# drscotthawley/signaltrain

Measured on AMD Instinct MI355X. Metric: audio-frames/sec (train step) comp_4c 8192-sample windows @ 1/2/4/8 GPUs, higher is better.
Workload: dtype f32; 1 GPU; comp_4c synthetic, 8192-sample windows, batch 256/GPU, fp32 (BASELINE configs[1]); window=8192, frames_per_window=25, global_batch=256, parallelism=dp1

## Files before the change

### include/signaltrain_hip.h

```cpp
#ifndef SIGNALTRAIN_HIP_H
#define SIGNALTRAIN_HIP_H
#include <stddef.h>
#include <stdint.h>
#ifdef __cplusplus
extern "C" {
#endif

#define ST_OK 0
#define ST_ERR_ARG (-1)
#define ST_ERR_LAUNCH (-2)
#define ST_ERR_UNSUPPORTED (-3)

#define ST_PREC_F32 0
#define ST_PREC_BF16 1
#define ST_PREC_BF16_ALL 2
#define ST_PREC_F16 3
#define ST_PREC_F16_ALL 4
#define ST_PREC_F32X3 5

typedef struct st_dims {
    int B;
    int L;
    int N;
    int H;
    int T;
    int OT;
    int F;
    int K;
    int y;
    int prec;
    float loss_scale;
    int clip_all;
} st_dims;

int st_kp(int F);

const char* st_last_error(void);
int st_version(void);

int st_set_tuning(int code);
int st_get_tuning(int* out, int n);
int st_tuning_defaults(int* out, int n);
int st_reset_tuning(void);
int st_effective_prec(const st_dims* d);
int st_set_debug(int v);

int st_profile_enable(int on);
int st_profile_report(char* buf, int buflen);

int st_geometry(double scale_factor, double shrink_factor, int legacy, int K, int B, st_dims* out);

int64_t st_param_offsets(const st_dims* d, int64_t* offs );

size_t st_workspace_bytes(const st_dims* d);
size_t st_workspace_bytes_max(const st_dims* d);

int st_analysis_fwd(const st_dims* d, const float* x, const float* Wr, const float* Wi, float in_scale,
                    float* re, float* im, float* mag, float* phs, void* stream);

int st_ae_fwd(const st_dims* d, const float* mag, const float* phs, const float* knobs,
              const float* ae_m, const float* ae_p, float* mag_hat, float* phs_hat, float* AA,
              float* reg_partial, float* ws, void* stream);
int st_ae_fwd_partials(const st_dims* d);
size_t st_ae_fwd_ws_floats(const st_dims* d);

int st_synth_fold(const st_dims* d, const float* Sr, const float* Si, float* Sfold, void* stream);

int st_synth_slabs(const st_dims* d);
int st_synth_frame_slabs(const st_dims* d);

int st_synthesis_frames(const st_dims* d, const float* AA, const float* Sfold, float* frs, void* stream);

int st_nt128_worklist(const st_dims* d, int which, int ncus, unsigned* out, int cap, int* head6);

int st_fm_div_exact(int R, int B);

int st_ola_loss(const st_dims* d, const float* frs, const float* x, const float* y_true,
                float* y_hat, float* dsyn, float* loss_partial, void* stream);
int st_ola_loss_partials(const st_dims* d);

int st_synthesis_dgrad(const st_dims* d, const float* dsyn, const float* Sfold, float* dAA, void* stream);

int st_synthesis_wgrad(const st_dims* d, const float* AA, const float* dsyn, float* ws,
                       float* gSr, float* gSi, float* norm_partial, void* stream);

int st_ae_bwd(const st_dims* d, const float* mag, const float* phs, const float* knobs,
              const float* ae_m, const float* ae_p, const float* mag_hat, const float* phs_hat,
              const float* dAA, const float* g_mag_hat , float reg_coef,
              float* dmag, float* dphs, float* ws, float* g_m, float* g_p, void* stream);
size_t st_ae_bwd_ws_floats(const st_dims* d);
size_t st_ae_kept_activation_bytes(const st_dims* d);

int st_polar_bwd(const st_dims* d, const float* re, const float* im, const float* dmag, const float* dphs,
                 const float* g_mag , float* dG, void* stream);

int st_analysis_wgrad(const st_dims* d, const float* dG, const float* x, float in_scale, float* ws,
                      float* gWr, float* gWi, float* norm_partial, void* stream);
size_t st_wgrad_ws_floats(const st_dims* d);
int st_norm_partials(const st_dims* d);

int st_finalize_scalars(const st_dims* d, const float* loss_partial, const float* reg_partial,
                        const float* norm_partial_a, const float* norm_partial_s, float inv_world,
                        float* scalars , void* stream);
int st_clip_adam(float* params, float* grads, float* m, float* v, int64_t n_total, int64_t n_stft,
                 const float* scalars, float grad_scale, float lr, float beta1, float beta2, float eps, int step,
                 void* stream);

int st_model_fwd(const st_dims* d, const float* params, const float* x, const float* knobs,
                 float* y_hat, float* mag, float* mag_hat, void* ws, int save_for_backward, void* stream);

int st_model_bwd(const st_dims* d, const float* params, float* grads, const float* x, const float* knobs,
                 const float* g_y_hat, const float* g_mag_hat, const float* g_mag, void* ws, void* stream);

int st_loss_backward(const st_dims* d, const float* params, float* grads, const float* x, const float* knobs,
                     const float* y_true, float* y_hat, float* mag, float* mag_hat, void* ws,
                     float* scalars, void* stream);

int st_eval_step(const st_dims* d, const float* params, const float* x, const float* knobs, const float* y_true,
                 float* y_hat , void* ws, double* acc , double beta, void* stream);

int st_loss_backward_p1(const st_dims* d, const float* params, float* grads, const float* x, const float* knobs,
                        const float* y_true, void* ws, void* stream);
int st_loss_backward_p2(const st_dims* d, float* grads, const float* x, void* ws, float* scalars, void* stream);
int st_loss_backward_p2_staged(const st_dims* d, float* grads, float* stage, const float* x, void* ws, float* scalars, void* stream);
int st_unstage_analysis(const st_dims* d, float* grads, const float* stage, void* stream);

int st_loss_backward_stage(const st_dims* d, const float* params, float* grads, const float* x, const float* knobs,
                           const float* y_true, void* ws, float* scalars, int stage, void* stream);

int st_train_step(const st_dims* d, float* params, float* grads, float* m, float* v, const float* x,
                  const float* knobs, const float* y_true, void* ws, float* scalars,
                  float lr, float beta1, float beta2, float eps, int step, void* stream);

#define ST_GROUP_ANALYSIS  1
#define ST_GROUP_SYNTHESIS 2
#define ST_GROUP_AE_MAG    4
#define ST_GROUP_AE_PHS    8
#define ST_GROUP_ALL      15

#define ST_STAGE_SYN_DGRAD  1
#define ST_STAGE_SYN_WGRAD  2
#define ST_STAGE_AE_BWD     4
#define ST_STAGE_AE_DINPUT  8
#define ST_STAGE_ANA_WGRAD 16

int st_step_groups_stages(int trainable);

int st_train_step_groups(const st_dims* d, float* params, float* grads, float* m, float* v,
                         const float* x, const float* knobs, const float* y_true, void* ws, float* scalars,
                         float lr, float beta1, float beta2, float eps,
                         const int step[4],
                         int trainable, void* stream);

int st_dp_clip_adam(const st_dims* d, float* params, float* grads, float* m, float* v, void* ws,
                    float* scalars, float grad_scale, float lr, float beta1, float beta2, float eps,
                    int step, void* stream);

typedef struct st_dp st_dp;
int st_dp_unique_id(void* id128);
int st_dp_init(const void* id128, int rank, int world, st_dp** out);
int st_dp_destroy(st_dp* p);
int st_dp_rank(const st_dp* p);
int st_dp_world(const st_dp* p);
int st_dp_rccl_version(const st_dp* p);
int st_dp_allreduce(st_dp* p, float* buf, int64_t n, void* stream);
int st_dp_broadcast(st_dp* p, float* buf, int64_t n, int root, void* stream);
int st_dp_sync(st_dp* p, void* stream);
int st_dp_train_step(st_dp* p, const st_dims* d, float* params, float* grads, float* m, float* v, float* stage,
                     const float* x, const float* knobs, const float* y_true, void* ws, float* scalars,
                     float lr, float beta1, float beta2, float eps, int step, int force_exchange, void* stream);

typedef struct st_graph st_graph;
int st_graph_create(const st_dims* d, float* params, float* grads, float* m, float* v, const float* x,
                    const float* knobs, const float* y_true, void* ws, float* scalars,
                    const float* lr_table, int n_lr, float beta1, float beta2, float eps, void* stream, st_graph** out);
int st_graph_launch(st_graph* g, void* stream);
int st_graph_destroy(st_graph* g);

int st_workspace_offsets(const st_dims* d, int64_t* offs8);
size_t st_ae_acts_floats(const st_dims* d);
int st_ae_acts(const st_dims* d, const float* v, const float* knobs, const float* ae, int sf, float* acts, void* stream);

int st_compressor_4c(const float* x, const float* knobs_wc, float sr, int B, int L, int ysz, float* y, void* stream);
int st_compressor(const float* x, const float* knobs_wc, float sr, int B, int L, int ysz, float* y, void* stream);
int st_lowpass(const float* x, const float* knobs_wc, float sr, int B, int L, int ysz, float* y, void* stream);
enum { ST_ECHO_MAX = 8 };
int st_echo(const float* x, const float* knobs_wc, float sr, int B, int L, int ysz, float* y, void* stream);
int st_denoise_input(unsigned seed, unsigned long long first_window, const float* x, const float* knobs_wc, int B, int L, float* x_noisy, void* stream);
size_t st_synth_comp4c_scratch_floats(int B, int L);
int st_synth_comp4c(unsigned seed, unsigned long long first_window, int B, int L, int ysz, int K, float sr,
                    const float* knob_lo, const float* knob_hi, int augment, int chooser, const float* pink_in,
                    float* x, float* y, float* knobs, float* scratch, void* stream);
enum { ST_FX_COMP4C = 0, ST_FX_COMP = 1, ST_FX_LOWPASS = 2, ST_FX_DENOISE = 3, ST_FX_ECHO = 4, ST_FX_DECOMP4C = 5 };
size_t st_synth_effect_scratch_floats(int effect, int B, int L);
int st_synth_effect(int effect, unsigned seed, unsigned long long first_window, int B, int L, int ysz, int K, float sr,
                    const float* knob_lo, const float* knob_hi, int augment, int chooser, const float* pink_in,
                    float* x, float* y, float* knobs, float* scratch, void* stream);
enum { ST_FAMILIES_COMPRESSOR = 0xD7, ST_FAMILIES_ALL = 0xFFF };
int st_synth_effect_families(int effect, unsigned family_mask, unsigned seed, unsigned long long first_window, int B, int L, int ysz, int K, float sr,
                             const float* knob_lo, const float* knob_hi, int augment, int chooser, const float* pink_in,
                             float* x, float* y, float* knobs, float* scratch, void* stream);

enum { ST_PCM_F32 = 0, ST_PCM_S16 = 1 };
int st_file_feed(unsigned seed, unsigned long long first_window, int B, int L, int ysz, int K, int fmt,
                 const void* pool_x, const void* pool_y, const long long* file_off, const long long* file_len, int nfiles,
                 long long min_len, long long pool_samples, const float* file_knobs, int augment,
                 float* x, float* y, float* knobs, long long* meta, void* stream);

size_t st_live_feed_scratch_floats(int effect, int B, int L, float synth_prob);
int st_live_feed(int effect, unsigned family_mask, float synth_prob, unsigned seed, unsigned long long first_window,
                 int B, int L, int ysz, int K, float sr, const float* knob_lo, const float* knob_hi, int augment,
                 int fmt, const void* pool_x, const long long* file_off, const long long* file_len, int nfiles,
                 long long min_len, long long pool_samples,
                 float* x, float* y, float* knobs, long long* meta ,
                 float* scratch, void* stream);

enum { ST_LIVE_PREROLL_MAX = 1 << 22 };
size_t st_live_feed_stream_scratch_floats(int effect, int B, int L, int preroll, float synth_prob);
int st_live_feed_stream(int effect, unsigned family_mask, float synth_prob, int preroll, unsigned seed, unsigned long long first_window,
                        int B, int L, int ysz, int K, float sr, const float* knob_lo, const float* knob_hi, int augment,
                        int fmt, const void* pool_x, const long long* file_off, const long long* file_len, int nfiles,
                        long long min_len, long long pool_samples,
                        float* x, float* y, float* knobs, long long* meta, float* scratch, void* stream);

size_t st_model_input_grad_ws_floats(const st_dims* d);
int st_model_input_grad(const st_dims* d, const float* params, void* ws, float* scratch, float* gxh, void* stream);
// ... 26 lines not shown
```

### signaltrain_amd/_lib.py

```python
import ctypes as C
import os

_HERE = os.path.dirname(os.path.abspath(__file__))
LIB_PATH = os.environ.get("ST_LIB_PATH") or os.path.join(_HERE, "libsignaltrain_hip.so")


class st_dims(C.Structure):
    _fields_ = [(n, C.c_int) for n in ("B", "L", "N", "H", "T", "OT", "F", "K", "y")] + \
               [("prec", C.c_int), ("loss_scale", C.c_float), ("clip_all", C.c_int)]

    def as_dict(self):
        return {n: getattr(self, n) for n, _ in self._fields_}

    def with_arith(self, prec=None, loss_scale=None, clip_all=None):
        d = st_dims(); C.memmove(C.byref(d), C.byref(self), C.sizeof(st_dims))
        if prec is not None: d.prec = int(prec)
        if loss_scale is not None: d.loss_scale = float(loss_scale)
        if clip_all is not None: d.clip_all = int(bool(clip_all))
        return d

    def with_batch(self, B):
        d = st_dims(); C.memmove(C.byref(d), C.byref(self), C.sizeof(st_dims)); d.B = int(B); return d


_p = C.c_void_p
_f = C.c_float
_i = C.c_int
_D = C.POINTER(st_dims)

SIGNATURES = {
    "st_kp": (_i, [_i]),
    "st_last_error": (C.c_char_p, []),
    "st_version": (_i, []),
    "st_set_tuning": (_i, [_i]),
    "st_get_tuning": (_i, [C.POINTER(C.c_int), _i]),
    "st_tuning_defaults": (_i, [C.POINTER(C.c_int), _i]),
    "st_reset_tuning": (_i, []),
    "st_effective_prec": (_i, [_D]),
    "st_set_debug": (_i, [_i]),
    "st_profile_enable": (_i, [_i]),
    "st_profile_report": (_i, [C.c_char_p, _i]),
    "st_geometry": (_i, [C.c_double, C.c_double, _i, _i, _i, _D]),
    "st_param_offsets": (C.c_int64, [_D, C.POINTER(C.c_int64)]),
    "st_workspace_bytes": (C.c_size_t, [_D]),
    "st_workspace_bytes_max": (C.c_size_t, [_D]),
    "st_analysis_fwd": (_i, [_D, _p, _p, _p, _f, _p, _p, _p, _p, _p]),
    "st_ae_fwd": (_i, [_D, _p, _p, _p, _p, _p, _p, _p, _p, _p, _p, _p]),
    "st_ae_fwd_ws_floats": (C.c_size_t, [_D]),
    "st_workspace_offsets": (_i, [_D, C.POINTER(C.c_int64)]),
    "st_ae_acts_floats": (C.c_size_t, [_D]),
    "st_ae_acts": (_i, [_D, _p, _p, _p, _i, _p, _p]),
    "st_compressor_4c": (_i, [_p, _p, C.c_float, C.c_int, C.c_int, C.c_int, _p, _p]),
    "st_compressor": (_i, [_p, _p, C.c_float, C.c_int, C.c_int, C.c_int, _p, _p]),
    "st_lowpass": (_i, [_p, _p, C.c_float, C.c_int, C.c_int, C.c_int, _p, _p]),
    "st_echo": (_i, [_p, _p, C.c_float, C.c_int, C.c_int, C.c_int, _p, _p]),
    "st_denoise_input": (_i, [C.c_uint, C.c_ulonglong, _p, _p, C.c_int, C.c_int, _p, _p]),
    "st_synth_comp4c_scratch_floats": (C.c_size_t, [_i, _i]),
    "st_synth_comp4c": (_i, [C.c_uint, C.c_ulonglong, C.c_int, C.c_int, C.c_int, C.c_int, C.c_float, C.POINTER(C.c_float), C.POINTER(C.c_float),
                             C.c_int, C.c_int, _p, _p, _p, _p, _p, _p]),
    "st_synth_effect_scratch_floats": (C.c_size_t, [_i, _i, _i]),
    "st_synth_effect": (_i, [_i, C.c_uint, C.c_ulonglong, C.c_int, C.c_int, C.c_int, C.c_int, C.c_float, C.POINTER(C.c_float), C.POINTER(C.c_float),
                             C.c_int, C.c_int, _p, _p, _p, _p, _p, _p]),
    "st_synth_effect_families": (_i, [_i, C.c_uint, C.c_uint, C.c_ulonglong, C.c_int, C.c_int, C.c_int, C.c_int, C.c_float, C.POINTER(C.c_float),
                                      C.POINTER(C.c_float), C.c_int, C.c_int, _p, _p, _p, _p, _p, _p]),
    "st_file_feed": (_i, [C.c_uint, C.c_ulonglong, _i, _i, _i, _i, _i, _p, _p, _p, _p, _i, C.c_longlong, C.c_longlong, _p, _i, _p, _p, _p, _p, _p]),
    "st_live_feed_scratch_floats": (C.c_size_t, [_i, _i, _i, C.c_float]),
    "st_live_feed": (_i, [_i, C.c_uint, C.c_float, C.c_uint, C.c_ulonglong, _i, _i, _i, _i, C.c_float, C.POINTER(C.c_float), C.POINTER(C.c_float), _i,
                          _i, _p, _p, _p, _i, C.c_longlong, C.c_longlong, _p, _p, _p, _p, _p, _p]),
    "st_live_feed_stream_scratch_floats": (C.c_size_t, [_i, _i, _i, _i, C.c_float]),
    "st_live_feed_stream": (_i, [_i, C.c_uint, C.c_float, _i, C.c_uint, C.c_ulonglong, _i, _i, _i, _i, C.c_float, C.POINTER(C.c_float), C.POINTER(C.c_float), _i,
                                 _i, _p, _p, _p, _i, C.c_longlong, C.c_longlong, _p, _p, _p, _p, _p, _p]),
    "st_fe_frames": (_i, [C.c_int] * 4),
    "st_fe_ws_floats": (C.c_size_t, [C.c_int] * 6),
    "st_fe_supported": (_i, [C.c_int] * 6),
    "st_fe_analysis_fwd": (_i, [_p, C.c_int, C.c_int, _p, _p, C.c_int, C.c_int, C.c_int, C.c_int, _p, _p]),
    "st_fe_synthesis_fwd": (_i, [_p, C.c_int, C.c_int, _p, C.c_int, C.c_int, C.c_int, C.c_int, _p, _p, _p]),
    "st_model_input_grad_ws_floats": (C.c_size_t, [_D]),
    "st_model_input_grad": (_i, [_D, _p, _p, _p, _p, _p]),
    "st_fe_analysis_bwd": (_i, [_p, C.c_int, C.c_int, _p, C.c_int, C.c_int, C.c_int, C.c_int, _p, _p, _p, _p, _p, _p]),
    "st_fe_synthesis_bwd": (_i, [_p, C.c_int, C.c_int, _p, C.c_int, C.c_int, C.c_int, C.c_int, _p, _p, _p, _p, _p]),
    "st_ae_fwd_partials": (_i, [_D]),
    "st_synth_slabs": (_i, [_D]),
    "st_synth_frame_slabs": (_i, [_D]),
    "st_nt128_worklist": (_i, [_D, _i, _i, C.POINTER(C.c_uint), _i, C.POINTER(C.c_int)]),
    "st_fm_div_exact": (_i, [_i, _i]),
    "st_synth_fold": (_i, [_D, _p, _p, _p, _p]),
    "st_synthesis_frames": (_i, [_D, _p, _p, _p, _p]),
    "st_ola_loss": (_i, [_D, _p, _p, _p, _p, _p, _p, _p]),
    "st_ola_loss_partials": (_i, [_D]),
    "st_synthesis_dgrad": (_i, [_D, _p, _p, _p, _p]),
    "st_synthesis_wgrad": (_i, [_D, _p, _p, _p, _p, _p, _p, _p]),
    "st_ae_bwd": (_i, [_D, _p, _p, _p, _p, _p, _p, _p, _p, _p, _f, _p, _p, _p, _p, _p, _p]),
    "st_ae_bwd_ws_floats": (C.c_size_t, [_D]),
    "st_ae_kept_activation_bytes": (C.c_size_t, [_D]),
    "st_polar_bwd": (_i, [_D, _p, _p, _p, _p, _p, _p, _p]),
    "st_analysis_wgrad": (_i, [_D, _p, _p, _f, _p, _p, _p, _p, _p]),
    "st_wgrad_ws_floats": (C.c_size_t, [_D]),
    "st_norm_partials": (_i, [_D]),
    "st_finalize_scalars": (_i, [_D, _p, _p, _p, _p, _f, _p, _p]),
    "st_clip_adam": (_i, [_p, _p, _p, _p, C.c_int64, C.c_int64, _p, _f, _f, _f, _f, _f, _i, _p]),
    "st_model_fwd": (_i, [_D, _p, _p, _p, _p, _p, _p, _p, _i, _p]),
    "st_model_bwd": (_i, [_D, _p, _p, _p, _p, _p, _p, _p, _p, _p]),
    "st_model_knob_grad": (_i, [_D, _p, _p, _p, _p, _p, _p, _p, _p, _p, _p]),
    "st_knob_grad_fused_supported": (_i, [_D]),
    "st_model_bwd_knobs_ws_floats": (C.c_size_t, [_D]),
    "st_model_bwd_knobs": (_i, [_D, _p, _p, _p, _p, _p, _p, _p, _p, _p, _p, _p]),
    "st_loss_backward": (_i, [_D, _p, _p, _p, _p, _p, _p, _p, _p, _p, _p, _p]),
    "st_eval_step": (_i, [_D, _p, _p, _p, _p, _p, _p, _p, C.c_double, _p]),
    "st_loss_backward_p1": (_i, [_D, _p, _p, _p, _p, _p, _p, _p]),
    "st_loss_backward_p2": (_i, [_D, _p, _p, _p, _p, _p]),
    "st_loss_backward_p2_staged": (_i, [_D, _p, _p, _p, _p, _p, _p]),
    "st_unstage_analysis": (_i, [_D, _p, _p, _p]),
    "st_loss_backward_stage": (_i, [_D, _p, _p, _p, _p, _p, _p, _p, _i, _p]),
    "st_train_step": (_i, [_D, _p, _p, _p, _p, _p, _p, _p, _p, _p, _f, _f, _f, _f, _i, _p]),
    "st_step_groups_stages": (_i, [_i]),
    "st_train_step_groups": (_i, [_D, _p, _p, _p, _p, _p, _p, _p, _p, _p, _f, _f, _f, _f, C.POINTER(C.c_int), _i, _p]),
    "st_dp_clip_adam": (_i, [_D, _p, _p, _p, _p, _p, _p, _f, _f, _f, _f, _f, _i, _p]),
    "st_graph_create": (_i, [_D, _p, _p, _p, _p, _p, _p, _p, _p, _p, _p, _i, _f, _f, _f, _p, C.POINTER(_p)]),
    "st_graph_launch": (_i, [_p, _p]),
    "st_graph_destroy": (_i, [_p]),
    "st_dp_unique_id": (_i, [_p]),
    "st_dp_init": (_i, [_p, _i, _i, C.POINTER(_p)]),
    "st_dp_destroy": (_i, [_p]),
    "st_dp_rank": (_i, [_p]),
    "st_dp_world": (_i, [_p]),
    "st_dp_rccl_version": (_i, [_p]),
    "st_dp_allreduce": (_i, [_p, _p, C.c_int64, _p]),
    "st_dp_broadcast": (_i, [_p, _p, C.c_int64, _i, _p]),
    "st_dp_sync": (_i, [_p, _p]),
    "st_dp_train_step": (_i, [_p, _D, _p, _p, _p, _p, _p, _p, _p, _p, _p, _p, _f, _f, _f, _f, _i, _i, _p]),
}

FX_COMP4C, FX_COMP, FX_LOWPASS, FX_DENOISE, FX_ECHO, FX_DECOMP4C = 0, 1, 2, 3, 4, 5
ECHO_MAX = 8
FAMILIES_COMPRESSOR, FAMILIES_ALL = 0xD7, 0xFFF


def family_mask(choosers):
    if choosers is None:
        return FAMILIES_COMPRESSOR
    fams = sorted({int(c) for c in choosers})
    if not fams or fams[0] < 0 or fams[-1] > 11:
        raise ValueError(f"signaltrain_amd: choosers = {list(choosers)!r}: a non-empty set of signal families out of 0..11 (the superposition, 12 and up, is not built)")
    return sum(1 << f for f in fams)
PCM_F32, PCM_S16 = 0, 1

GROUPS = {"analysis": 1, "synthesis": 2, "aenc": 4, "phs_aenc": 8}
GROUP_SETS = dict(GROUPS, frontend=3)
GROUP_ALL = 15
STAGE_SYN_DGRAD, STAGE_SYN_WGRAD, STAGE_AE_BWD, STAGE_AE_DINPUT, STAGE_ANA_WGRAD = 1, 2, 4, 8, 16

PREC = {"f32": 0, "bf16": 1, "bf16_all": 2, "f16": 3, "f16_all": 4, "f32x3": 5}

_lib = None


def load():
    global _lib
    if _lib is not None:
        return _lib
    if not os.path.isfile(LIB_PATH):
        raise RuntimeError(
            f"signaltrain_amd: {LIB_PATH} is missing. Build it with `python -c 'import __graft_entry__ as g; g.build()'` "
            "or `make -C signaltrain_amd/csrc`. There is no CPU fallback.")
    lib = C.CDLL(LIB_PATH)
    for name, (res, args) in SIGNATURES.items():
        fn = getattr(lib, name)
        fn.restype = res
        fn.argtypes = args
    _lib = lib
    return lib


def check(rc, what=""):
    if rc != 0:
        msg = load().st_last_error().decode("utf-8", "replace")
        raise RuntimeError(f"signaltrain_hip {what} failed (rc={rc}): {msg}")


def ptr(t):
    if t is None:
        return None
    assert t.is_contiguous(), "signaltrain_amd: tensor must be contiguous"
    return C.c_void_p(t.data_ptr())


def on_arg_device(fn):
    import functools
    import torch

    @functools.wraps(fn)
    def wrapped(ctx, first, *rest):
        if torch.is_tensor(first) and first.is_cuda:
            with torch.cuda.device(first.device):
                return fn(ctx, first, *rest)
        return fn(ctx, first, *rest)
    return wrapped


def geometry(scale_factor=1, shrink_factor=4, num_knobs=4, batch=1, scale_scheme="lean"):
    d = st_dims()
    check(load().st_geometry(float(scale_factor), float(shrink_factor), 0 if scale_scheme == "lean" else 1,
                             int(num_knobs), int(batch), C.byref(d)), "st_geometry")
    return d


def param_offsets(d):
    offs = (C.c_int64 * 40)()
    total = load().st_param_offsets(C.byref(d), offs)
    if total < 0:
        check(-1, "st_param_offsets")
    return list(offs), int(total)
```

### signaltrain_amd/csrc/st_api.hip

```cpp
#include <hip/hip_runtime.h>
#include <stdarg.h>
#include <stdio.h>
#include <string.h>
#include <math.h>
#include <mutex>
#include <set>
#include <type_traits>
#include <utility>
#include "st_common.h"
#include "st_gemm.h"
#include "st_gemm_planes.h"
#include "st_gemm_tn.h"
#include "st_gemm16.h"
#include "st_misc.h"
#include "st_ae.h"
#include "st_ae_wide.h"
#include "st_ae_split.h"
#include "st_ae32.h"
#include "st_dp.h"
#include "st_feed.h"
#include "st_feed_files.h"
#include "st_feed_live.h"
#include "st_feed_stream.h"

// ... 22 lines not shown
static hipEvent_t g_prof_ev[ST_PROF_MAX];
static const char* g_prof_name[ST_PROF_MAX];
static bool g_prof_init = false;
static void prof_mark(const char* name, void* stream)
{
    if (!g_prof || g_prof_n >= ST_PROF_MAX) return;
    (void)hipEventRecord(g_prof_ev[g_prof_n], st_stream(stream));
    g_prof_name[g_prof_n++] = name;
}
extern "C" int st_profile_enable(int on)
{
    if (on && !g_prof_init) {
        for (int i = 0; i < ST_PROF_MAX; ++i)
            if (hipEventCreate(&g_prof_ev[i]) != hipSuccess) return st_fail(ST_ERR_LAUNCH, "hipEventCreate");
        g_prof_init = true;
    }
    g_prof = on != 0; g_prof_n = 0;
    return ST_OK;
}
extern "C" int st_profile_report(char* buf, int buflen)
{
    if (!buf || buflen <= 0) return st_fail(ST_ERR_ARG, "st_profile_report: bad buffer");
    const char* names[64]; double tot[64]; int cnt[64]; int nn = 0;
    for (int i = 1; i < g_prof_n; ++i) {
        if (!strcmp(g_prof_name[i], "begin")) continue;
        float ms = 0.f;
        if (hipEventElapsedTime(&ms, g_prof_ev[i - 1], g_prof_ev[i]) != hipSuccess) continue;
        int k = 0; for (; k < nn; ++k) if (!strcmp(names[k], g_prof_name[i])) break;
        if (k == nn) { if (nn == 64) continue; names[nn] = g_prof_name[i]; tot[nn] = 0; cnt[nn] = 0; ++nn; }
        tot[k] += ms; cnt[k]++;
    }
    int off = 0; buf[0] = 0;
    for (int k = 0; k < nn; ++k) off += snprintf(buf + off, off < buflen ? buflen - off : 0, "%s %.6f %d\n", names[k], tot[k], cnt[k]);
    g_prof_n = 0;
    return ST_OK;
}
extern "C" int st_version(void) { return 100; }
extern "C" int st_kp(int F) { return st_kp_of(F); }

extern "C" int st_geometry(double scale_factor, double shrink_factor, int legacy, int K, int B, st_dims* o)
{
    ST_REQ(o && scale_factor > 0 && shrink_factor > 0, "st_geometry: bad arguments");
    const int chunk = (int)(8192 * scale_factor);
    const int out_chunk = (int)(chunk / shrink_factor);
    int ft = 1024, hop = 384;
    if (legacy) { ft = (int)(ft * scale_factor); hop = (int)(hop * scale_factor); }
    o->B = B; o->L = chunk; o->N = ft; o->H = hop; o->K = K;
    o->T = (int)(ceil(chunk / (double)hop) + ceil(ft / (double)hop));
    o->OT = (int)(ceil(out_chunk / (double)hop) + ceil(ft / (double)hop));
    o->y = (o->OT - 1) * hop - ft;
    o->F = ft / 2 + 1;
    return ST_OK;
}

static int check_dims(const st_dims* d)
{
    ST_REQ(d, "null dims");
    ST_REQ(d->B > 0 && d->L > 0 && d->N > 0 && d->H > 0 && d->T > 0 && d->OT > 0 && d->K >= 0, "non-positive dimension");
    ST_REQ(d->F == d->N / 2 + 1, "F must be N/2+1");
    ST_REQ(d->N % 32 == 0 && d->H % 4 == 0 && d->L % 4 == 0 && d->y % 4 == 0, "N%%32, H%%4, L%%4, y%%4 required");
    ST_REQ(d->y == (d->OT - 1) * d->H - d->N && d->y > 0 && d->y <= d->L, "y must equal (OT-1)*H-N");
    ST_REQ(d->OT <= d->T, "OT must be <= T");
    ST_REQ((long long)d->H * d->T >= (long long)d->L + d->N, "T too small: H*T >= L+N required, or a frame overlapping the signal is dropped (T=%d L=%d N=%d H=%d)",
           d->T, d->L, d->N, d->H);
    ST_REQ(d->K <= 16, "at most 16 knobs");
    ST_REQ(d->prec >= ST_PREC_F32 && d->prec <= ST_PREC_F32X3, "st_dims.prec = %d is not an ST_PREC_* level", d->prec);
    ST_REQ(d->loss_scale >= 0.f && d->loss_scale <= 3.0e38f, "st_dims.loss_scale must be 0 (none) or a positive finite scale");
    ST_REQ((size_t)d->B * d->T < ((size_t)1 << 24) && (size_t)d->B * d->T * st_kp_of(d->F) < ((size_t)1 << 30) &&
           (size_t)d->B * ((size_t)d->L + 2 * (size_t)d->N) < ((size_t)1 << 30), "batch too large for 32-bit element offsets (B=%d)", d->B);
    ST_REQ(((unsigned long long)d->B * d->T - 1) * (unsigned long long)d->T < (1ull << 32), "row split inexact: (B*T - 1)*T must stay below 2^32 (B=%d T=%d)", d->B, d->T);
    return ST_OK;
}

static void ae_shapes(const st_dims* d, int* out, int* in)
{
    const sta::AEShape sh{d->T, d->OT, d->K};
    for (int l = 0; l < sta::NL; ++l) { out[l] = sh.out(l); in[l] = sh.in(l); }
}

static int64_t param_offsets(const st_dims* d, int64_t* offs)
{
    int64_t off = 0; int n = 0;
    auto put = [&](int64_t sz) { if (offs) offs[n] = off; ++n; off += (sz + 3) / 4 * 4; };
    for (int s = 0; s < 4; ++s) put((int64_t)d->N * d->N);
    int out[9], in[9]; ae_shapes(d, out, in);
    for (int a = 0; a < 2; ++a)
        for (int l = 0; l < 9; ++l) { put((int64_t)out[l] * in[l]); put(out[l]); }
    return off;
}
extern "C" int64_t st_param_offsets(const st_dims* d, int64_t* offs) { return check_dims(d) != ST_OK ? -1 : param_offsets(d, offs); }

struct Layout {
    int64_t offs[40]; int64_t total; int64_t n_stft; int PG; sta::AEOffsets go; int KP;
};
static int make_layout(const st_dims* d, Layout* L)
{
    ST_TRY(check_dims(d));
    L->total = param_offsets(d, L->offs);
    L->n_stft = L->offs[4];
    L->PG = (int)(L->offs[22] - L->offs[4]);
    for (int l = 0; l < 9; ++l) {
        L->go.w[l] = (int)(L->offs[4 + 2 * l] - L->offs[4]);
        L->go.b[l] = (int)(L->offs[5 + 2 * l] - L->offs[4]);
    }
    L->KP = st_kp_of(d->F);
    return ST_OK;
}

static int num_cus()
{
    static int n = 0;
    if (!n) { int dev = 0; (void)hipGetDevice(&dev); hipDeviceProp_t p; if (hipGetDeviceProperties(&p, dev) == hipSuccess) n = p.multiProcessorCount; if (n <= 0) n = 256; }
    return n;
}
extern "C" int st_set_debug(int v) { return v == 0 ? ST_OK : st_fail(ST_ERR_ARG, "st_set_debug(%d): the product library has no run-time ablations (build with -DST_*_ABLATE=bits)", v); }
static int g_dp_inline = 1;
static int g_ae_save = 1;
static int g_ae_split = -1;
static int g_ae32 = 1;
static int g_pl_bf16 = 0;
static int g_wg_split = 0;
static int g_pl_dgrad = 0;
static int g_pl_shape = 3;
static int g_g16 = 1;
static int g_g16_dma = 0;
static int g_nt128 = 1;
static int g_tn128 = 1;
static int g_tn_fm = 3;
static int g_g16_crop = 15;
static int g_frs_nt = 1;
static int g_xt = 0;
static const int NORM_E_PARTIALS = 32;
static const int NORM_E_MAX = 4096;
static int g_wide_direct = 1;
static int g_an_bk = 32;
static int g_bk = 16;
static int g_wg_mode = 0;
#define ST_TUNING_LIST(X) X(g_ae_split, -1) X(g_ae_save, 1) X(g_dp_inline, 1) X(g_pl_bf16, 0) X(g_wg_split, 0) X(g_pl_dgrad, 0) X(g_pl_shape, 3) X(g_g16, 1) X(g_g16_dma, 0) \
    X(g_nt128, 1) X(g_tn128, 1) X(g_frs_nt, 1) X(g_xt, 0) X(g_an_bk, 32) X(g_bk, 16) X(g_wg_mode, 0) X(g_ae32, 1) X(g_wide_direct, 1) X(g_tn_fm, 3) X(g_g16_crop, 15)
static const struct { int first, count; int* var; int value; int* also; } k_tuning_codes[] = {
    {16, 1, &g_an_bk, 16, &g_bk}, {32, 1, &g_an_bk, 32, &g_bk},
    {100, 1, &g_wg_mode, 0, nullptr}, {102, 1, &g_wg_mode, 2, nullptr},
    {7000, 2, &g_xt, 0, nullptr},
    {8000, 2, &g_ae_split, 0, nullptr}, {8002, 1, &g_ae_split, -1, nullptr},
    {8100, 2, &g_ae32, 0, nullptr},
    {8200, 3, &g_ae_save, 0, nullptr},
    {8300, 2, &g_dp_inline, 0, nullptr},
    {9000, 2, &g_frs_nt, 0, nullptr},
    {9100, 1, &g_pl_shape, 0, nullptr}, {9103, 1, &g_pl_shape, 3, nullptr},
    {9200, 2, &g_pl_dgrad, 0, nullptr},
    {9300, 2, &g_wg_split, 0, nullptr},
    {9400, 2, &g_pl_bf16, 0, nullptr},
    {9500, 2, &g_tn128, 0, nullptr}, {9580, 1, &g_tn128, 2, nullptr}, {9581, 1, &g_tn128, 1, nullptr},
    {9540, 4, &g_tn_fm, 0, nullptr},
    {9560, 16, &g_g16_crop, 0, nullptr},
    {9600, 2, &g_g16, 0, nullptr},
    {9690, 4, &g_g16_dma, 0, nullptr},
    {9950, 2, &g_nt128, 0, nullptr},
    {9970, 2, &g_wide_direct, 0, nullptr},
};
extern "C" int st_set_tuning(int code)
{
    for (const auto& t : k_tuning_codes)
        if (code >= t.first && code < t.first + t.count) { *t.var = t.value + (code - t.first); if (t.also) *t.also = *t.var; return ST_OK; }
    return st_fail(ST_ERR_ARG, "st_set_tuning(%d): no such code", code);
}
extern "C" int st_get_tuning(int* out, int n)
{
    int i = 0;
#define X(v_, d_) if (out && i < n) out[i] = v_; ++i;
    ST_TUNING_LIST(X)
#undef X
    return i;
}
extern "C" int st_tuning_defaults(int* out, int n)
{
    int i = 0;
#define X(v_, d_) if (out && i < n) out[i] = d_; ++i;
    ST_TUNING_LIST(X)
#undef X
    return i;
}
extern "C" int st_reset_tuning(void)
{
#define X(v_, d_) v_ = d_;
    ST_TUNING_LIST(X)
#undef X
    return ST_OK;
}
static inline int gemm_ht(int prec) { return (prec == ST_PREC_BF16 || prec == ST_PREC_BF16_ALL) ? 1 : ((prec == ST_PREC_F16 || prec == ST_PREC_F16_ALL) ? 2 : (prec == ST_PREC_F32X3 ? 3 : 0)); }
static inline int ae_ht(int prec) { return prec == ST_PREC_BF16_ALL ? 1 : (prec == ST_PREC_F16_ALL ? 2 : 0); }
static inline float loss_scale_of(const st_dims* d) { return d->loss_scale > 0.f ? d->loss_scale : 1.0f; }
static inline float reg_scale_of(const st_dims* d) { return (float)(2e-5 / 10.0) / ((float)d->B * (float)d->OT * (float)d->F); }
static inline float reg_coef_of(const st_dims* d) { return loss_scale_of(d) * (float)(2e-5 / 10.0) / ((float)d->B * (float)d->OT * (float)d->F); }
static inline float expfac_of(const st_dims* d) { return (float)(7.0 / d->F); }
#define ST_GEMM_BK(BK_, W_, ...) do { const int ht_ = gemm_ht(d->prec); \
                              if (ht_ == 1) stg::launch_half<W_, 1>(__VA_ARGS__); else if (ht_ == 2) stg::launch_half<W_, 2>(__VA_ARGS__); \
                              else if (ht_ == 3) { ST_TRY((stg::launch_half<W_, 1, 3>(__VA_ARGS__))); } \
                              else if (g_xt) { if ((BK_) == 16) stg::launch<W_, 16, true>(__VA_ARGS__); else stg::launch<W_, 32, true>(__VA_ARGS__); } \
                              else if ((BK_) == 16) stg::launch<W_, 16>(__VA_ARGS__); else stg::launch<W_, 32>(__VA_ARGS__); } while (0)
#define ST_GEMM(W_, ...) ST_GEMM_BK(g_bk, W_, __VA_ARGS__)
#define ST_GEMM_AN(W_, ...) ST_GEMM_BK(g_an_bk, W_, __VA_ARGS__)
#define ST_GEMM_WG(...) do { if (g_wg_mode == 2 && gemm_ht(d->prec) == 0) stg::launch<3, 16, true>(__VA_ARGS__); \
                             else if (gemm_ht(d->prec) == 3 && !g_wg_split) stg::launch<3, 16>(__VA_ARGS__); else ST_GEMM(3, __VA_ARGS__); } while (0)
static int ensure_dyn_lds(const void* fn, const char* name)
{
    static std::mutex mu; static std::set<std::pair<int, const void*>> done;
    int dev = 0; (void)hipGetDevice(&dev);
    std::lock_guard<std::mutex> lk(mu);
    if (done.count({dev, fn})) return ST_OK;
    const hipError_t e = hipFuncSetAttribute(fn, hipFuncAttributeMaxDynamicSharedMemorySize, 160 * 1024);
    if (e != hipSuccess) return st_fail(ST_ERR_LAUNCH, "hipFuncSetAttribute(%s, 160 KB dynamic LDS): %s", name, hipGetErrorString(e));
    done.insert({dev, fn});
    return ST_OK;
}
template <class... P, class... A>
static int launch_lds(const char* name, void (*kernel)(P...), dim3 grid, dim3 block, size_t lds, hipStream_t s, A&&... args)
{
    static_assert(sizeof...(P) == sizeof...(A), "launch_lds: argument count");
    ST_TRY(ensure_dyn_lds(reinterpret_cast<const void*>(kernel), name));
    hipLaunchKernelGGL(kernel, grid, block, lds, s, static_cast<P>(args)...);
    return ST_OK;
}
template <int V> using ic = std::integral_constant<int, V>;
template <class F> static inline auto with_ht(int ht, F&& f) { return ht == 1 ? f(ic<1>{}) : ht == 2 ? f(ic<2>{}) : f(ic<0>{}); }
template <class F> static inline auto with_ht16(int ht, F&& f) { return ht == 2 ? f(ic<2>{}) : f(ic<1>{}); }
template <class F> static inline auto with_bool(bool b, F&& f) { return b ? f(std::true_type{}) : f(std::false_type{}); }
template <class F> static inline auto with_var(int var, F&& f) { return with_ht(var, f); }
template <class F> static inline auto with_slabs(int ns, F&& f) { return ns == 3 ? f(ic<3>{}) : ns == 2 ? f(ic<2>{}) : f(ic<1>{}); }
static const int AE_FWD_NW = 8, AE_BWD_NW = 4;
template <class F> static inline auto with_fwd_nw(int nw, F&& f) { return nw == 11 ? f(ic<11>{}) : f(ic<AE_FWD_NW>{}); }
template <class F> static inline auto with_inner_nw(int nw, F&& f) { return nw == 9 ? f(ic<9>{}) : nw == 12 ? f(ic<12>{}) : f(ic<AE_FWD_NW>{}); }
static int synth_live_rows(const st_dims* d);
static bool ae_is_wide(const st_dims* d);
static int ae_fwd_groups(const st_dims* d) { return d->B * (st_kp_of(d->F) / 32); }
static int ae_fwd_nw(const st_dims* d)
{
    if (ae_is_wide(d) || ae_ht(d->prec) != 0) return AE_FWD_NW;
    const int groups = ae_fwd_groups(d), c = num_cus();
    auto cost = [&](int nw) { int grid = (groups + nw - 1) / nw; if (grid > c) grid = c; const int rounds = (groups + grid * nw - 1) / (grid * nw); return rounds * nw; };
    return cost(11) < cost(AE_FWD_NW) ? 11 : AE_FWD_NW;
}
static int ae_inner_nw(const st_dims* d)
{
    const int groups = ae_fwd_groups(d), c = num_cus();
    int best = AE_FWD_NW, best_cost = 1 << 30;
    for (int nw : {8, 9, 12}) {
        int grid = (groups + nw - 1) / nw; if (grid > c) grid = c;
        const int rounds = (groups + grid * nw - 1) / (grid * nw), cost = rounds * ((nw + 3) / 4);
        if (cost < best_cost) { best_cost = cost; best = nw; }
    }
    return best;
}
static int ae_inner_grid(const st_dims* d) { const int nw = ae_inner_nw(d); int g = (ae_fwd_groups(d) + nw - 1) / nw; int c = num_cus(); return g < c ? g : c; }
static int ae_fwd_grid(const st_dims* d) { const int nw = ae_fwd_nw(d); int g = (ae_fwd_groups(d) + nw - 1) / nw; int c = num_cus(); return g < c ? g : c; }
static int ae_bwd_grid(const st_dims* d) { int groups = d->B * (st_kp_of(d->F) / 32); int g = (groups + AE_BWD_NW - 1) / AE_BWD_NW; int c = num_cus() / 2; if (c < 1) c = 1; return g < c ? g : c; }
static const int WSPLIT_ROWS = 200, WSPLIT_MAX = 16;
static int wgrad_split(int R) { int s = R / WSPLIT_ROWS; if (s < 1) s = 1; if (s > WSPLIT_MAX) s = WSPLIT_MAX; return s; }
static int wgrad_split_tiles(int R, int M, int Nc)
{
    int s = wgrad_split(R);
    const int tiles = ((M + 95) / 96) * ((Nc + 95) / 96), slots = 6 * num_cus();
    int fit = slots / (tiles > 0 ? tiles : 1); if (fit < 1) fit = 1;
    if (fit >= 2) fit &= ~1;
    return s < fit ? s : fit;
}
static int synth_split(int R) { return R >= 4096 ? 1 : 3; }
static int dgrad_slabs(int R) { return synth_split(R); }

static int ae_fwd_partials(const st_dims* d) { return ae_fwd_grid(d) * ae_fwd_nw(d); }
static int ola_loss_partials(const st_dims* d) { return d->B * ((d->y + 255) / 256); }
static int norm_partials(const st_dims* d) { return stm::norm_partial_count(d->F, d->N); }
extern "C" int st_ae_fwd_partials(const st_dims* d) { return check_dims(d) != ST_OK ? 0 : ae_fwd_partials(d); }
extern "C" int st_ola_loss_partials(const st_dims* d) { return check_dims(d) != ST_OK ? 0 : ola_loss_partials(d); }
extern "C" int st_norm_partials(const st_dims* d) { return check_dims(d) != ST_OK ? 0 : norm_partials(d); }
static int tn_split(int R, int N)
{
    const int tiles = (N / 128) * (N / 128);
    int s = num_cus() / (tiles > 0 ? tiles : 1); if (s > 16) s = 16;
    const int cap = R / 64; if (s > cap) s = cap;
    return s < 1 ? 1 : s;
}
static size_t wgrad_ws_floats(const st_dims* d)
{
    int s = wgrad_split_tiles(d->B * d->T, st_kp_of(d->F), d->N);
    const int s2 = tn_split(d->B * d->T, d->N); if (s2 > s) s = s2;
    return (size_t)s * st_kp_of(d->F) * d->N + (size_t)64 * 2 * d->N;
}
extern "C" size_t st_wgrad_ws_floats(const st_dims* d) { return check_dims(d) != ST_OK ? 0 : wgrad_ws_floats(d); }
static size_t synth_wgrad_ws_floats(const st_dims* d) { return wgrad_ws_floats(d); }
static int synth_slabs(const st_dims* d) { return dgrad_slabs(synth_live_rows(d)); }
extern "C" int st_synth_slabs(const st_dims* d) { return check_dims(d) != ST_OK ? 0 : synth_slabs(d); }
static int frames_split(int R) { return R >= 4096 ? 1 : 3; }
static int frame_slabs(const st_dims* d) { return frames_split(synth_live_rows(d)); }
extern "C" int st_synth_frame_slabs(const st_dims* d) { return check_dims(d) != ST_OK ? 0 : frame_slabs(d); }
static bool ae_is_wide(const st_dims* d) { return d->T > 32 || d->OT > 16; }
struct WideWS {
    float *W1p[2], *W5p[2], *V[2], *H[2][8], *E9[2];
    float *DA[2][9], *TL[2], *slabs, *inner_ws;
    size_t fwd_floats, floats; int Tp, nsplit; size_t R, SL; int so[10];
};
static void wide_carve(const st_dims* d, const Layout& L, float* base, WideWS* w)
{
    const int FP = st_kp_of(d->F) / 2;
    const size_t R = (size_t)d->B * FP;
    int out[9], in[9]; ae_shapes(d, out, in);
    w->R = R; w->Tp = st_round_up(d->T, 32);
    { long ns = (long)(R / 128); w->nsplit = (int)(ns < 1 ? 1 : (ns > 256 ? 256 : ns)); }
    w->so[0] = 0;
    for (int l = 0; l < 9; ++l) w->so[l + 1] = w->so[l] + st_round_up(out[l] * (in[l] + 1), 64);
    w->SL = (size_t)w->so[9];
    size_t off = 0;
    auto take = [&](size_t n) { float* p = base ? base + off : nullptr; off += (n + 63) / 64 * 64; return p; };
    for (int a = 0; a < 2; ++a) {
        w->W1p[a] = take((size_t)64 * w->Tp); w->W5p[a] = take(16 * 32);
        w->V[a] = take((size_t)(d->T + 1) * R);
        for (int j = 0; j < 8; ++j) w->H[a][j] = take((size_t)(in[j + 1] + 1) * R);
        w->E9[a] = take((size_t)d->OT * R);
    }
    w->fwd_floats = off;
    for (int a = 0; a < 2; ++a) {
        for (int l = 0; l < 9; ++l) w->DA[a][l] = take((size_t)out[l] * R);
        w->TL[a] = take((size_t)d->OT * R);
    }
    w->slabs = take((size_t)2 * w->nsplit * w->SL);
    w->inner_ws = take((size_t)ae_bwd_grid(d) * 2 * L.PG);
    w->floats = off;
}
static const int AE_SPLIT_NW = 8;
static size_t ae_h4_floats(const st_dims* d) { return (size_t)2 * ae_fwd_groups(d) * 256; }
static int ae_split_grid(const st_dims* d) { int g = (ae_fwd_groups(d) + AE_SPLIT_NW - 1) / AE_SPLIT_NW; int c = num_cus() / 2; if (c < 1) c = 1; return g < c ? g : c; }
static bool ae_use_split(const st_dims* d) { return (g_ae_split < 0 ? ae_ht(d->prec) != 0 : g_ae_split != 0) && !ae_is_wide(d); }
static size_t ae_sv_floats(const st_dims* d) { return (!ae_is_wide(d) && ae_ht(d->prec) == 0) ? (size_t)2 * ae_fwd_groups(d) * sta::AE_SV_TILES * 256 : 0; }
static int ae_parts_max(const st_dims* d) { return ae_split_grid(d) > ae_bwd_grid(d) ? ae_split_grid(d) : ae_bwd_grid(d); }
static bool ae_use_saved(const st_dims* d) { return g_ae_save && !ae_is_wide(d) && ae_ht(d->prec) == 0 && !ae_use_split(d); }
static float* ae_sv_ptr(const st_dims* d, const Layout& L, float* aews) { return aews + 2 * ae_h4_floats(d) + (size_t)ae_parts_max(d) * 2 * L.PG; }
static int ae_img_level(const st_dims* d)
{
    if (g_ae_save == 2 || ae_is_wide(d) || ae_ht(d->prec) != 0 || ae_use_split(d)) return 0;
    const int FP = st_kp_of(d->F) / 2;
    const size_t room = 2 * ae_h4_floats(d);
    if (FP > sta::CL::FWD_TOTAL || room < (size_t)sta::ae_img_fwd_floats(FP)) return 0;
    return room >= (size_t)sta::ae_img_floats(FP) ? 2 : 1;
}
static float* ae_img_ptr(float* aews) { return aews; }
static const char* ae_kg_why(const st_dims* d)
{
    if (ae_is_wide(d)) return nullptr;
    if (ae_use_split(d)) return ae_ht(d->prec) != 0 ? nullptr : "g_ae_split routes fp32 layers to the split kernels";
    if (ae_ht(d->prec) != 0) return "g_ae_split routes 16-bit layers to the single kernel";
    return ae_use_saved(d) ? nullptr : "g_ae_save is off: the recomputing fp32 kernel";
}
static bool ae_kg_route(const st_dims* d) { return ae_kg_why(d) == nullptr; }
extern "C" size_t st_ae_fwd_ws_floats(const st_dims* d)
{
    Layout L; if (make_layout(d, &L) != ST_OK) return 0;
    if (!ae_is_wide(d)) return ae_h4_floats(d);
    WideWS w; wide_carve(d, L, nullptr, &w); return w.fwd_floats;
}
extern "C" size_t st_ae_kept_activation_bytes(const st_dims* d)
{
    if (check_dims(d) != ST_OK || !ae_use_saved(d)) return 0;
    return ae_sv_floats(d) * sizeof(float);
}
static size_t ae_bwd_ws_floats(const st_dims* d, const Layout& L)
{
    if (ae_is_wide(d)) { WideWS w; wide_carve(d, L, nullptr, &w); return w.floats; }
    return 2 * ae_h4_floats(d) + (size_t)ae_parts_max(d) * 2 * L.PG + ae_sv_floats(d);
}
extern "C" size_t st_ae_bwd_ws_floats(const st_dims* d) { Layout L; return make_layout(d, &L) != ST_OK ? 0 : ae_bwd_ws_floats(d, L); }
static int ae_wide_fwd(const st_dims* d, const Layout& L, const float* mag, const float* phs, const float* knobs,
                       const float* ae_m, const float* ae_p, float* mag_hat, float* phs_hat, float* AA, float* reg_partial,
                       WideWS& w, void* stream, unsigned short* AA16 = nullptr, bool in_done = false);

struct PolarWide { float* Vm; float* Vp; int FP; unsigned RV; };
static inline void polar_wide_set(stg::PolarStore& ep, const PolarWide* pw) { if (pw && pw->Vm) { ep.Vm = pw->Vm; ep.Vp = pw->Vp; ep.FP = pw->FP; ep.RV = pw->RV; } }
static int analysis_fwd_impl(const st_dims* d, const float* sig, bool padded, const float* Wr, const float* Wi, float in_scale,
                             float* re, float* im, float* mag, float* phs, void* stream, bool dead_frames_done = false, const PolarWide* pw = nullptr)
{
    const stg::RowMap map = stg::live_frames(d->T, d->H, d->N, d->N, d->L);
    const int R = map.rows(d->B);
    stg::AnalysisW bl{Wr, Wi, d->F, d->N};
    stg::PolarStore ep{re, im, mag, phs, R, d->F, map};
    polar_wide_set(ep, pw);
    if (padded) {
        stg::FramedNT<true> al{sig, d->L, d->H, d->N, R, d->N, 1.0f, map};
        ST_GEMM_AN(4, al, bl, ep, R, 2 * d->F, d->N, 1, st_stream(stream));
    }
    else { stg::FramedNT<false> al{sig, d->L, d->H, d->N, R, d->N, in_scale, map}; ST_GEMM(4, al, bl, ep, R, 2 * d->F, d->N, 1, st_stream(stream)); }
    ST_LAUNCHED("analysis_fwd");
    if (map.Tv < d->T && !dead_frames_done) {
        hipLaunchKernelGGL(stm::zero_dead_frames_kernel, dim3(d->B * (d->T - map.Tv)), dim3(256), 0, st_stream(stream),
                           re, im, mag, phs, d->T, d->F, map.t_lo, map.Tv);
        ST_LAUNCHED("zero_dead_frames");
    }
    return ST_OK;
}
extern "C" int st_analysis_fwd(const st_dims* d, const float* x, const float* Wr, const float* Wi, float in_scale,
                               float* re, float* im, float* mag, float* phs, void* stream)
{
    ST_TRY(check_dims(d)); ST_REQ(x && Wr && Wi, "st_analysis_fwd: null input");
    return analysis_fwd_impl(d, x, false, Wr, Wi, in_scale, re, im, mag, phs, stream);
}
static int pad_scale(const float* in, float* out, int B, int Ls, int pad, float s, void* stream)
{
    hipLaunchKernelGGL(stm::pad_scale_kernel, dim3(((Ls + 2 * pad) / 4 + 255) / 256, B), dim3(256), 0, st_stream(stream), in, out, Ls, pad, s);
    ST_LAUNCHED("pad_scale");
    return ST_OK;
}

static int ae_fwd_body(const st_dims* d, const Layout& L, const float* mag, const float* phs, const float* knobs,
                       const float* ae_m, const float* ae_p, float* mag_hat, float* phs_hat, float* AA,
                       float* reg_partial, float* ws, void* stream, unsigned short* AA16 = nullptr, bool wide_in_done = false, float* sv = nullptr, const float* img = nullptr)
{
    const int aa_ht = AA16 ? gemm_ht(d->prec) : 0;
    ST_REQ(mag && phs && (knobs || d->K == 0) && ae_m && ae_p && ((mag_hat && phs_hat && AA) || (!mag_hat && !phs_hat && !AA && ws)), "st_ae_fwd: null pointer");
    if (!knobs) knobs = ae_m;
    if (ae_is_wide(d)) {
        ST_REQ(mag_hat, "st_ae_fwd: the code-only pass exists for the fused geometries only");
        ST_REQ(ws, "st_ae_fwd: this geometry (T=%d, OT=%d) needs st_ae_fwd_ws_floats() floats of workspace", d->T, d->OT);
        WideWS w; wide_carve(d, L, ws, &w);
        return ae_wide_fwd(d, L, mag, phs, knobs, ae_m, ae_p, mag_hat, phs_hat, AA, reg_partial, w, stream, AA16, wide_in_done);
    }
    ST_REQ((size_t)d->B * d->T * d->F < ((size_t)1 << 30) && (size_t)d->B * d->OT * L.KP < ((size_t)1 << 30),
           "st_ae_fwd: batch too large for the kernel's 32-bit element offsets (B=%d)", d->B);
    const size_t lds = ((size_t)2 * sta::CL::FWD_TOTAL + (size_t)(L.KP / 2)) * sizeof(float);
    const float expfac = expfac_of(d);
    const int ht = ae_ht(d->prec);
    const dim3 grid(ae_fwd_grid(d));
    hipStream_t s = st_stream(stream);
    const bool use32 = g_ae32 && ht != 0 && L.KP / 2 <= 17 * 32 && AE_FWD_NW == 8;
    if (use32)
// ... 31 lines not shown
    ST_LAUNCHED("synth_fold"); return ST_OK;
}

static stg::RowMap synth_live(const st_dims* d) { return stg::live_frames(d->OT, d->H, d->N, d->N, d->y); }
static int synth_live_rows(const st_dims* d) { return synth_live(d).rows(d->B); }

static int synthesis_frames_impl(const st_dims* d, const float* AA, const float* Sfold, const float* SfoldT, float* frs, void* stream);
extern "C" int st_synthesis_frames(const st_dims* d, const float* AA, const float* Sfold, float* frs, void* stream)
{
    ST_TRY(check_dims(d)); ST_REQ(AA && Sfold && frs, "st_synthesis_frames: null pointer");
    return synthesis_frames_impl(d, AA, Sfold, nullptr, frs, stream);
}
static double synth_crop_fraction(const st_dims* d)
{
    const stg::RowMap ms = synth_live(d);
    long live = 0;
    for (int t = ms.t_lo; t < ms.t_lo + ms.Tv; ++t) { int lo, hi; stg::ntw_live_taps(t, t, d->H, d->N, d->N, d->y, lo, hi); live += hi - lo; }
    return 1.0 - (double)live / ((double)ms.Tv * (double)d->N);
}
static inline bool fm_div_exact(int R, int B) { return R >= 0 && B >= 1 && (unsigned long long)(unsigned)R * (unsigned long long)(unsigned)B < (1ull << 32); }
extern "C" int st_fm_div_exact(int R, int B) { return fm_div_exact(R, B) ? 1 : 0; }
static bool use_nt128(const st_dims* d, int M, int Nc, int ncus = 0)
{
    if (!(g_nt128 && gemm_ht(d->prec) == 0 && d->N % 32 == 0 && (M + 127) / 128 <= 255 && fm_div_exact(M, d->B))) return false;
    if (ncus <= 0) ncus = num_cus();
    return ((M + 127) / 128) * ((Nc + 127) / 128) * 2 <= ncus || synth_crop_fraction(d) >= 0.10;
}
static int synthesis_frames_impl(const st_dims* d, const float* AA, const float* Sfold, const float* SfoldT, float* frs, void* stream)
{
    const int KP = st_kp_of(d->F);
    const stg::RowMap ms = synth_live(d);
    const int R = ms.rows(d->B);
    stg::PlainNT al{AA, R, KP, KP, ms};
    stg::PlainTN bl{Sfold, KP, d->N, d->N, stg::all_frames(1)};
    stg::StoreC ep{frs, R, d->N, d->N, (size_t)d->B * d->OT * d->N, ms};
    if (SfoldT && g_frs_nt) {
        stg::PlainNT bt{SfoldT, d->N, KP, KP, stg::all_frames(1)};
        stg::NTWork wk;
        if (use_nt128(d, R, d->N) && stg::ntw_frames(wk, ms, d->B, d->H, d->N, d->N, d->y, KP, frames_split(R), num_cus())) {
            const stg::NTRows ra = stg::ntrows_frame_major(AA, (unsigned)(d->OT * KP), (unsigned)KP, ms, d->B, R), rb{SfoldT, (unsigned)KP, 0u, 0u, 1, 0, d->N};
            const stg::StoreSlab es{frs, R, d->N, d->N, (size_t)d->B * d->OT * d->N, stg::frame_major(ms, d->B)};
            ST_TRY(stg::launch_nt128(ra, rb, es, wk, st_stream(stream)));
        }
        else if (R >= 4096) ST_GEMM(4, al, bt, ep, R, d->N, KP, 1, st_stream(stream));
        else ST_GEMM(2, al, bt, ep, R, d->N, KP, frames_split(R), st_stream(stream));
    }
    else if (R >= 4096) ST_GEMM(4, al, bl, ep, R, d->N, KP, 1, st_stream(stream));
    else ST_GEMM(2, al, bl, ep, R, d->N, KP, frames_split(R), st_stream(stream));
    ST_LAUNCHED("synthesis_frames"); return ST_OK;
}

extern "C" int st_nt128_worklist(const st_dims* d, int which, int ncus, unsigned* out, int cap, int* head6)
{
    if (check_dims(d) != ST_OK || !out || !head6 || cap < 0 || (which != 0 && which != 1)) return -1;
    const int KP = st_kp_of(d->F);
    const stg::RowMap ms = synth_live(d);
    const int R = ms.rows(d->B);
    if (ncus <= 0) ncus = num_cus();
    stg::NTWork wk; wk.n = 0;
    if (!use_nt128(d, R, which ? KP : d->N, ncus)) return 0;
    const bool ok = which ? stg::ntw_dgrad(wk, ms, d->B, d->H, d->N, d->N, d->y, d->F, KP, dgrad_slabs(R), ncus)
                          : stg::ntw_frames(wk, ms, d->B, d->H, d->N, d->N, d->y, KP, frames_split(R), ncus);
    if (!ok) return 0;
    head6[0] = wk.nslabs; head6[1] = wk.col_h; head6[2] = wk.col_stride; head6[3] = d->B; head6[4] = wk.kunit; head6[5] = wk.kt_total;
    for (int i = 0; i < wk.n && i < cap; ++i) out[i] = wk.e[i];
    return wk.n;
}

static int ola_loss_impl(const st_dims* d, const float* frs, const float* x, const float* y_true,
                         float* y_hat, float* dsyn, int dsyn_pad, float* loss_partial, void* stream, unsigned short* dsyn16 = nullptr,
                         bool with_mae = false)
{
    if (with_mae) ST_REQ(y_true && loss_partial && !dsyn, "ola_loss: the MAE partials come with a target and without d syn");
    const float inv = loss_scale_of(d) / ((float)d->B * (float)d->y);
    {
        const int ns = frame_slabs(d), nslot = (d->y + 255) / 256;
        auto al16 = [](const void* p) { return (reinterpret_cast<uintptr_t>(p) & 15) == 0; };
        const bool ok4 = d->H % 4 == 0 && d->N % 4 == 0 && d->y % 4 == 0 && d->L % 4 == 0 && dsyn_pad % 4 == 0 && ns >= 1 && ns <= 3 && (d->N + d->H - 1) / d->H <= 3 &&
                         al16(frs) && al16(x) && al16(y_true) && al16(y_hat) && al16(dsyn) && al16(dsyn16) && ((size_t)d->B * d->OT * d->N) % 4 == 0;
        if (ok4) {
            const dim3 grid((d->y / 4 + 255) / 256, d->B);
            const size_t slab = (size_t)d->B * d->OT * d->N;
            unsigned short* d16 = dsyn ? dsyn16 : nullptr; const int ht = dsyn16 ? gemm_ht(d->prec) : 0;
            with_bool(with_mae, [&](auto MAE) { with_slabs(ns, [&](auto NS) {
                hipLaunchKernelGGL((stm::ola_loss4_kernel<NS(), MAE()>), grid, dim3(256), 0, st_stream(stream), frs, x, y_true, y_hat, dsyn, loss_partial, d->L, d->N, d->H, d->OT, d->y, inv, slab, dsyn_pad, nslot, d16, ht); }); });
            ST_LAUNCHED("ola_loss");
            return ST_OK;
        }
    }
    with_bool(with_mae, [&](auto MAE) {
        hipLaunchKernelGGL(stm::ola_loss_kernel<MAE()>, dim3((d->y + 255) / 256, d->B), dim3(256), 0, st_stream(stream),
                           frs, x, y_true, y_hat, dsyn, loss_partial, d->L, d->N, d->H, d->OT, d->y, inv,
                           frame_slabs(d), (size_t)d->B * d->OT * d->N, dsyn_pad, dsyn ? dsyn16 : nullptr, dsyn16 ? gemm_ht(d->prec) : 0); });
    ST_LAUNCHED("ola_loss");
    return ST_OK;
}
extern "C" int st_ola_loss(const st_dims* d, const float* frs, const float* x, const float* y_true,
                           float* y_hat, float* dsyn, float* loss_partial, void* stream)
{
    ST_TRY(check_dims(d)); ST_REQ(frs, "st_ola_loss: null pointer");
    return ola_loss_impl(d, frs, x, y_true, y_hat, dsyn, 0, loss_partial, stream);
}

static int synthesis_dgrad_impl(const st_dims* d, const float* dsyn, bool padded, const float* Sfold, float* dAA, void* stream)
{
    const int KP = st_kp_of(d->F);
    const stg::RowMap ms = synth_live(d);
    const int R = ms.rows(d->B);
    stg::PlainNT bl{Sfold, KP, d->N, d->N, stg::all_frames(1)};
    stg::StoreC ep{dAA, R, KP, KP, (size_t)d->B * d->OT * KP, ms};
    const int ns = dgrad_slabs(R);
    if (padded) {
        stg::FramedNT<true> al{dsyn, d->y, d->H, d->N, R, d->N, 1.0f, ms};
        stg::NTWork wk;
        if (use_nt128(d, R, KP) && stg::ntw_dgrad(wk, ms, d->B, d->H, d->N, d->N, d->y, d->F, KP, ns, num_cus())) {
            const stg::NTRows ra = stg::ntrows_frame_major(dsyn, (unsigned)(d->y + 2 * d->N), (unsigned)d->H, ms, d->B, R);
            const stg::NTRows rb = wk.col_h ? stg::NTRows{Sfold, (unsigned)((KP / 2) * d->N), (unsigned)d->N, stg::rowmap_magic(d->F - 1), d->F - 1, 0, 2 * (d->F - 1)}
                                            : stg::NTRows{Sfold, (unsigned)d->N, 0u, 0u, 1, 0, KP};
            const stg::StoreSlab es{dAA, R, KP, KP, (size_t)d->B * d->OT * KP, stg::frame_major(ms, d->B)};
            ST_TRY(stg::launch_nt128(ra, rb, es, wk, st_stream(stream)));
        }
        else if (R >= 4096) ST_GEMM(4, al, bl, ep, R, KP, d->N, ns, st_stream(stream));
        else ST_GEMM(2, al, bl, ep, R, KP, d->N, ns, st_stream(stream));
    } else {
        stg::FramedNT<false> al{dsyn, d->y, d->H, d->N, R, d->N, 1.0f, ms};
        if (R >= 4096) ST_GEMM(4, al, bl, ep, R, KP, d->N, ns, st_stream(stream)); else ST_GEMM(2, al, bl, ep, R, KP, d->N, ns, st_stream(stream));
    }
    ST_LAUNCHED("synthesis_dgrad");
    return ST_OK;
}
extern "C" int st_synthesis_dgrad(const st_dims* d, const float* dsyn, const float* Sfold, float* dAA, void* stream)
{
    ST_TRY(check_dims(d)); ST_REQ(dsyn && Sfold && dAA, "st_synthesis_dgrad: null pointer");
    return synthesis_dgrad_impl(d, dsyn, false, Sfold, dAA, stream);
}

static bool use_tn128(const st_dims* d, bool padded)
{
    const int ht = gemm_ht(d->prec);
    return g_tn128 && padded && (ht == 0 || (ht == 3 && !g_wg_split)) && d->N % 256 == 0 && g_wg_mode == 0;
}
struct TNFrameMajor { stg::TNOperand a, b; stg::RowMap map; stg::FrameTrim trim; bool on; };
static TNFrameMajor tn_frame_major(const stg::TNOperand& ta, const stg::TNOperand& tb, const stg::RowMap& live, int B, int H, int Ntaps, int pad, int Ls, bool enable)
{
    TNFrameMajor f; f.on = enable && B >= 2 && fm_div_exact(live.Tv * B, B); f.a = ta; f.b = tb; f.map = live; f.trim = stg::FrameTrim{}; f.trim.on = 0;
    if (!f.on) return f;
    f.a = stg::TNOperand{ta.base + (size_t)live.t_lo * ta.S2, ta.S2, ta.S1};
    f.b = stg::TNOperand{tb.base + (size_t)live.t_lo * tb.S2, tb.S2, tb.S1};
    f.map.Tv = B; f.map.t_lo = 0; f.map.magic = stg::rowmap_magic(B); f.map.fm = 0;
    f.trim = stg::frame_trim(live, B, H, Ntaps, pad, Ls);
    return f;
}
#define ST_TN128(...) do { if (g_tn128 == 2) ST_TRY((stg::launch_tn128<32, false>(__VA_ARGS__))); else ST_TRY((stg::launch_tn128<32, true>(__VA_ARGS__))); } while (0)
static int wgrad_tn128(const st_dims* d, const stg::TNOperand& ta, const stg::TNOperand& tb, const float* zeros, const stg::RowMap& map, int R,
                       float* ws, int ns, stm::NyqJob* nyq, void* stream, const stg::FrameTrim* trim)
{
    const int KP = st_kp_of(d->F);
    const int mh = (d->N / 2) / 128;
    float* part = ws + (size_t)ns * KP * d->N;
    int P = 0;
    const unsigned c0 = (unsigned)(d->F - 1), c1 = (unsigned)(KP / 2 + d->F - 1);
    ST_TN128(ta, tb, zeros, map, R, d->N, mh, (unsigned)(KP / 2), d->N, ws, d->N, (size_t)KP * d->N, ns, st_stream(stream), part, c0, c1, &P, trim);
    nyq->part = part; nyq->P = P; nyq->on = 1;
    return ST_OK;
}
static int synthesis_wgrad_impl(const st_dims* d, const float* AA, const float* dsyn, bool padded, float* ws,
                                float* gSr, float* gSi, float* norm_partial, void* stream, int* defer_slabs = nullptr, stm::NyqJob* defer_nyq = nullptr)
{
    const int KP = st_kp_of(d->F);
    const stg::RowMap ms = synth_live(d);
    const int R = ms.rows(d->B);
    int ns = wgrad_split_tiles(R, KP, d->N);
    stm::NyqJob nyq{}; nyq.on = 0;
    const stg::TNOperand ta{AA, (unsigned)(d->OT * KP), (unsigned)KP}, tb{dsyn, (unsigned)(d->y + 2 * d->N), (unsigned)d->H};
    if (use_tn128(d, padded) && stg::tn128_fits(ta, tb, dsyn, ms, d->N, d->N, (size_t)d->B * d->OT * KP, (size_t)d->B * (d->y + 2 * d->N))) {
        ns = tn_split(R, d->N);
        const TNFrameMajor fm = tn_frame_major(ta, tb, ms, d->B, d->H, d->N, d->N, d->y, (g_tn_fm & 1) != 0);
        ST_TRY(wgrad_tn128(d, fm.a, fm.b, dsyn, fm.map, R, ws, ns, &nyq, stream, &fm.trim));
    } else {
        stg::PlainTN al{AA, R, KP, KP, ms};
        stg::StoreC ep{ws, KP, d->N, d->N, (size_t)KP * d->N, stg::all_frames(1)};
        if (padded) { stg::FramedTN<true> bl{dsyn, d->y, d->H, d->N, R, d->N, 1.0f, ms}; ST_GEMM_WG(al, bl, ep, KP, d->N, R, ns, st_stream(stream)); }
        else { stg::FramedTN<false> bl{dsyn, d->y, d->H, d->N, R, d->N, 1.0f, ms}; ST_GEMM_WG(al, bl, ep, KP, d->N, R, ns, st_stream(stream)); }
    }
    ST_LAUNCHED("synthesis_wgrad");
    if (defer_slabs) { *defer_slabs = ns; if (defer_nyq) *defer_nyq = nyq; return ST_OK; }
    hipLaunchKernelGGL(stm::wgrad_reduce_kernel, dim3(norm_partials(d)), dim3(256), 0, st_stream(stream),
                       ws, ns, gSr, gSi, norm_partial, d->N, d->F, KP, 1, 0, 2 * d->F, (float*)nullptr, nyq);
    ST_LAUNCHED("synthesis_wgrad_reduce");
    return ST_OK;
}
extern "C" int st_synthesis_wgrad(const st_dims* d, const float* AA, const float* dsyn, float* ws,
                                  float* gSr, float* gSi, float* norm_partial, void* stream)
{
    ST_TRY(check_dims(d)); ST_REQ(AA && dsyn && ws && gSr && gSi && norm_partial, "st_synthesis_wgrad: null pointer");
    return synthesis_wgrad_impl(d, AA, dsyn, false, ws, gSr, gSi, norm_partial, stream);
}


extern "C" int st_effective_prec(const st_dims* d)
{
    if (!d) return -1;
    return d->prec;
}
template <class AL, class BL, class EPI>
static void wgemm_pair(int wide_ht, const AL& a0, const BL& b0, const EPI& e0, const AL& a1, const BL& b1, const EPI& e1, int M, int Nc, int K, int ns, hipStream_t s)
{
    if (wide_ht) with_ht16(wide_ht, [&](auto HT) { stg::launch_half_pair<2, HT()>(a0, b0, e0, a1, b1, e1, M, Nc, K, ns, s); });
    else { stg::launch<2, 16>(a0, b0, e0, M, Nc, K, ns, s); stg::launch<2, 16>(a1, b1, e1, M, Nc, K, ns, s); }
}
static int fill_pad_jobs(stw::PadJobs& pj, const st_dims* d, const Layout& L, const float* ae_m, const float* ae_p, const WideWS& w)
{
    int blk = 0;
    for (int a = 0; a < 2; ++a) {
        const float* ae = a ? ae_p : ae_m;
        pj.src[2 * a] = ae + L.go.w[0]; pj.dst[2 * a] = w.W1p[a]; pj.rows[2 * a] = 64; pj.cols[2 * a] = d->T; pj.pitch[2 * a] = w.Tp;
        pj.blk0[2 * a] = blk; blk += (64 * w.Tp + 255) / 256;
        pj.src[2 * a + 1] = ae + L.go.w[4]; pj.dst[2 * a + 1] = w.W5p[a]; pj.rows[2 * a + 1] = 16; pj.cols[2 * a + 1] = 16 + d->K; pj.pitch[2 * a + 1] = 32;
        pj.blk0[2 * a + 1] = blk; blk += 2;
    }
    pj.blk0[4] = blk;
    return blk;
}
static int ae_wide_fwd(const st_dims* d, const Layout& L, const float* mag, const float* phs, const float* knobs,
                       const float* ae_m, const float* ae_p, float* mag_hat, float* phs_hat, float* AA, float* reg_partial,
                       WideWS& w, void* stream, unsigned short* AA16, bool in_done)
{
    hipStream_t s = st_stream(stream);
    const int FP = L.KP / 2, F = d->F, T = d->T, OT = d->OT, R = (int)w.R, Tp = w.Tp;
    const int wide_ht = ae_ht(d->prec);
    ST_REQ(w.R * (size_t)(T > 64 ? T : 64) < ((size_t)1 << 30), "wide autoencoder path: batch too large (B=%d)", d->B);
    const stg::RowMap id = stg::all_frames(1);
    int out[9], in[9]; ae_shapes(d, out, in);
    if (!in_done) {
        stw::PadJobs pj; const int blk = fill_pad_jobs(pj, d, L, ae_m, ae_p, w);
        ST_REQ(FP % 4 == 0 && (size_t)(T + d->K) * d->B * (FP / 4) < ((size_t)1 << 31), "wide autoencoder path: batch too large (B=%d)", d->B);
        const int n_copy = (int)(((size_t)(T + d->K) * d->B * (FP / 4) + 255) / 256);
        hipLaunchKernelGGL(stw::wide_in_kernel, dim3(n_copy + blk), dim3(256), 0, s, mag, phs, knobs, w.V[0], w.V[1], w.H[0][3], w.H[1][3],
                           d->B, T, F, FP, d->K, n_copy, pj);
        ST_LAUNCHED("ae_wide_in");
    }
    {
        stg::PlainNT al0{w.W1p[0], out[0], Tp, Tp, id}, al1{w.W1p[1], out[0], Tp, Tp, id};
        stg::PlainTN bl0{w.V[0], in[0], R, R, id}, bl1{w.V[1], in[0], R, R, id};
        stw::ActStore ep0{w.H[0][0], ae_m + L.go.b[0], out[0], R, FP, F}, ep1{w.H[1][0], ae_p + L.go.b[0], out[0], R, FP, F};
        wgemm_pair(wide_ht, al0, bl0, ep0, al1, bl1, ep1, out[0], R, Tp, 1, s);
    }
    {
        const size_t lds = (size_t)2 * sta::CL::FWD_TOTAL * sizeof(float);
        ST_TRY(with_ht(wide_ht, [&](auto HT) { return with_inner_nw(ae_inner_nw(d), [&](auto NW) {
            return launch_lds("ae_inner_fwd_kernel", sta::ae_inner_fwd_kernel<NW(), HT()>, dim3(ae_inner_grid(d)), dim3(NW() * 64), lds, s,
                              w.H[0][0], w.H[1][0], knobs, ae_m, ae_p, L.go, w.H[0][7], w.H[1][7], d->B, F, d->K, L.KP); }); }));
    }
    {
        stg::PlainNT al0{ae_m + L.go.w[8], OT, 64, 64, id}, al1{ae_p + L.go.w[8], OT, 64, 64, id};
        stg::PlainTN bl0{w.H[0][7], 64, R, R, id}, bl1{w.H[1][7], 64, R, R, id};
        stw::OutStore ep0{w.E9[0], mag_hat, w.V[0] + (size_t)(T - OT) * R, ae_m + L.go.b[8], OT, R, FP, F, 0};
        stw::OutStore ep1{w.E9[1], phs_hat, w.V[1] + (size_t)(T - OT) * R, ae_p + L.go.b[8], OT, R, FP, F, 1};
        wgemm_pair(wide_ht, al0, bl0, ep0, al1, bl1, ep1, OT, R, 64, 1, s);
    }
    ST_LAUNCHED("ae_wide_fwd");
    if (AA) {
        hipLaunchKernelGGL(stw::wide_polar_out_kernel, dim3(ae_fwd_partials(d)), dim3(256), 0, s, mag_hat, phs_hat, AA, reg_partial,
                           d->B, OT, F, FP, L.KP, expfac_of(d), AA16, AA16 ? gemm_ht(d->prec) : 0);
        ST_LAUNCHED("ae_wide_polar_out");
    }
    return ST_OK;
}

static void wide_wgrad_pair(const st_dims* d, WideWS& w, int l, const int* out, const int* in, hipStream_t s, const int wide_ht)
{
    const int R = (int)w.R;
    const stg::RowMap id = stg::all_frames(1);
    stg::PlainNT al0{w.DA[0][l], out[l], R, R, id}, al1{w.DA[1][l], out[l], R, R, id};
    stg::PlainNT bl0{l == 0 ? w.V[0] : w.H[0][l - 1], in[l] + 1, R, R, id}, bl1{l == 0 ? w.V[1] : w.H[1][l - 1], in[l] + 1, R, R, id};
    stg::StoreC ep0{w.slabs + w.so[l], out[l], in[l] + 1, in[l] + 1, w.SL, id};
    stg::StoreC ep1 = ep0;
    if (!wide_ht) ep1.out = w.slabs + (size_t)w.nsplit * w.SL + w.so[l];
    if (wide_ht && R % 32) {
        with_ht16(wide_ht, [&](auto HT) { stg::launch_half_pair<2, HT(), 1, 16>(al0, bl0, ep0, al1, bl1, ep1, out[l], in[l] + 1, R, w.nsplit, s); });
        return;
    }
    wgemm_pair(wide_ht, al0, bl0, ep0, al1, bl1, ep1, out[l], in[l] + 1, R, w.nsplit, s);
}

struct PolarSink { const float* re; const float* im; const float* g_mag; float* dG; unsigned short* dG16; };
static int ae_wide_bwd(const st_dims* d, const Layout& L, const float* mag, const float* phs, const float* knobs,
                       const float* ae_m, const float* ae_p, const float* mag_hat, const float* phs_hat, const float* dAA,
                       const float* g_mag_hat, float reg_coef, float* dmag, float* dphs, WideWS& w, float* g_m, float* g_p,
                       bool have_fwd, void* stream, const PolarSink* sink = nullptr,
                       const stw::SynReduce* syn = nullptr, float* norm_e = nullptr, int* n_norm_e = nullptr, float* kg = nullptr, bool no_dinput = false)
{
    hipStream_t s = st_stream(stream);
    const int FP = L.KP / 2, F = d->F, T = d->T, OT = d->OT, R = (int)w.R;
    const int wide_ht = ae_ht(d->prec);
    const stg::RowMap id = stg::all_frames(1);
    int out[9], in[9]; ae_shapes(d, out, in);
    if (!have_fwd) ST_TRY(ae_wide_fwd(d, L, mag, phs, knobs, ae_m, ae_p, nullptr, nullptr, nullptr, nullptr, w, stream));
    stw::OnesRows rows;
    for (int a = 0; a < 2; ++a) {
        rows.p[9 * a] = w.V[a] + (size_t)in[0] * R;
        for (int j = 0; j < 8; ++j) rows.p[9 * a + 1 + j] = w.H[a][j] + (size_t)in[j + 1] * R;
    }
    const float expfac = expfac_of(d);
    const stg::RowMap ms = synth_live(d);
    {
        const size_t n = (size_t)d->B * OT * FP;
        ST_REQ(n < ((size_t)1 << 30), "wide autoencoder path: batch too large (B=%d)", d->B);
        int grid = (int)((n + 255) / 256); if (grid > 8192) grid = 8192;
        hipLaunchKernelGGL(stw::wide_dout_kernel, dim3(grid + 18 * d->B), dim3(256), 0, s, dAA, synth_slabs(d), (size_t)d->B * OT * L.KP,
                           mag_hat, phs_hat, w.E9[0], w.E9[1], w.V[0] + (size_t)(T - OT) * R, g_mag_hat, reg_coef, expfac,
                           w.DA[0][8], w.DA[1][8], w.TL[0], w.TL[1], d->B, OT, F, FP, L.KP, ms.t_lo, ms.t_lo + ms.Tv - 1, grid, rows);
        ST_LAUNCHED("ae_wide_dout");
    }
    stw::GradTab tab;
    for (int l = 0; l < 9; ++l) { tab.so[l] = w.so[l]; tab.out[l] = out[l]; tab.in[l] = in[l]; tab.gw[l] = L.go.w[l]; tab.gb[l] = L.go.b[l]; }
    tab.so[9] = w.so[9];
    int inner_parts = 0;
    wide_wgrad_pair(d, w, 8, out, in, s, wide_ht);
    {
        stg::PlainTN al0{ae_m + L.go.w[8], out[8], in[8], in[8], id}, al1{ae_p + L.go.w[8], out[8], in[8], in[8], id};
        stg::PlainTN bl0{w.DA[0][8], out[8], R, R, id}, bl1{w.DA[1][8], out[8], R, R, id};
        stg::StoreC ep0{w.DA[0][7], in[8], R, R, 0, id}, ep1{w.DA[1][7], in[8], R, R, 0, id};
        wgemm_pair(wide_ht, al0, bl0, ep0, al1, bl1, ep1, in[8], R, out[8], 1, s);
    }
    {
        const size_t lds = (size_t)sta::ae_bwd_lds_floats(AE_BWD_NW) * sizeof(float);
        const int grid = ae_bwd_grid(d);
        ST_TRY(with_ht(wide_ht, [&](auto HT) { return with_bool(kg != nullptr, [&](auto KG) {
            return launch_lds("ae_bwd_kernel", sta::ae_bwd_kernel<AE_BWD_NW, true, HT(), 0, false, KG()>, dim3(grid, 2), dim3(AE_BWD_NW * 64), lds, s,
                              w.H[0][0], w.H[1][0], knobs, ae_m, ae_p, L.go, L.PG, w.DA[0][7], w.DA[1][7], nullptr, nullptr, 0.f, 0.f,
                              w.DA[0][0], w.DA[1][0], w.inner_ws, d->B, T, OT, F, d->K, L.KP, 0, 0, 1, (size_t)0, nullptr, kg, nullptr); }); }));
        inner_parts = grid;
    }
    for (int l = 1; l < 8; ++l) tab.out[l] = 0;
    wide_wgrad_pair(d, w, 0, out, in, s, wide_ht);
    if (norm_e && 2 * ((w.so[9] + 63) / 64 + (L.PG + 63) / 64) > NORM_E_MAX) norm_e = nullptr;
    hipLaunchKernelGGL(stw::wide_grad_finish_kernel, dim3((w.so[9] + 63) / 64 + (L.PG + 63) / 64 + (syn ? norm_partials(d) : 0), 2), dim3(256), 0, s, w.slabs, w.nsplit, w.SL, tab, g_m, g_p,
                       (w.so[9] + 63) / 64, (const float*)w.inner_ws, inner_parts, L.PG, syn ? *syn : stw::SynReduce{}, norm_e);
    if (norm_e && n_norm_e) *n_norm_e = 2 * ((w.so[9] + 63) / 64 + (L.PG + 63) / 64);
    if (no_dinput) { ST_LAUNCHED("ae_wide_bwd_noin"); return ST_OK; }
    {
        stw::DvPolarArgs q;
        q.DA1m = w.DA[0][0]; q.DA1p = w.DA[1][0]; q.TLm = w.TL[0]; q.TLp = w.TL[1]; q.W1m = ae_m + L.go.w[0]; q.W1p = ae_p + L.go.w[0];
        q.re = sink ? sink->re : nullptr; q.im = sink ? sink->im : nullptr; q.g_mag = sink ? sink->g_mag : nullptr;
        q.dG = sink ? sink->dG : nullptr; q.dG16 = sink ? sink->dG16 : nullptr;
        q.dmag = sink ? nullptr : dmag; q.dphs = sink ? nullptr : dphs;
        q.ht = gemm_ht(d->prec) <= 2 ? gemm_ht(d->prec) : 0; q.sat = gemm_ht(d->prec) == 2 ? 65504.0f : 0.0f;
        q.B = d->B; q.T = T; q.OT = OT; q.F = F; q.FP = FP; q.KP = L.KP;
        const int TP16 = (T + 15) / 16 * 16, groups = d->B * (FP / 16);
        ST_REQ(TP16 <= 192, "wide autoencoder path: T = %d frames exceeds the layer-1 data-gradient kernel's 192", T);
        const size_t lds = (size_t)2 * (wide_ht ? 32 : 64) * TP16 * sizeof(float);
        int grid = ((groups + 7) / 8) * (TP16 / 16); if (grid > num_cus()) grid = num_cus();
        ST_TRY(with_ht(wide_ht, [&](auto HT) { return launch_lds("wide_dv_polar_kernel", stw::wide_dv_polar_kernel<HT()>, dim3(grid), dim3(512), lds, s, q); }));
    }
    ST_LAUNCHED("ae_wide_bwd");
    return ST_OK;
}

static int ae_bwd_body(const st_dims* d, const Layout& L, const float* mag, const float* phs, const float* knobs,
                       const float* ae_m, const float* ae_p, const float* mag_hat, const float* phs_hat,
                       const float* dAA, const float* g_mag_hat, float reg_coef, float* dmag, float* dphs, float* ws,
                       float* g_m, float* g_p, bool have_fwd, void* stream, bool* defer_reduce = nullptr,
                       const PolarSink* sink = nullptr, const stw::SynReduce* syn = nullptr, float* norm_e = nullptr, int* n_norm_e = nullptr,
                       float* kg = nullptr, bool have_img = false, bool no_dinput = false)
{
    ST_REQ(mag && phs && (knobs || d->K == 0) && ae_m && ae_p && mag_hat && phs_hat && dAA && dmag && dphs && ws && g_m && g_p, "st_ae_bwd: null pointer");
    if (!knobs) knobs = ae_m;
    if (ae_is_wide(d)) {
        if (defer_reduce) *defer_reduce = false;
        WideWS w; wide_carve(d, L, ws, &w);
        return ae_wide_bwd(d, L, mag, phs, knobs, ae_m, ae_p, mag_hat, phs_hat, dAA, g_mag_hat, reg_coef, dmag, dphs, w, g_m, g_p, have_fwd, stream, sink, syn, norm_e, n_norm_e, kg, no_dinput);
    }
    ST_REQ(!no_dinput || (!kg && !g_mag_hat), "st_ae_bwd: the form without the input gradient takes neither an upstream d mag_hat nor the knob-gradient output");
    if (kg && !(ae_kg_route(d) && have_fwd)) return st_fail(ST_ERR_UNSUPPORTED, "st_ae_bwd: no per-group d a5 output on this autoencoder backward route (%s)", ae_kg_why(d));
    const size_t lds = (size_t)sta::ae_bwd_lds_floats(AE_BWD_NW) * sizeof(float);
    static_assert((size_t)sta::ae_bwd_lds_floats(AE_BWD_NW) * sizeof(float) <= 160 * 1024, "ae_bwd LDS budget");
    ST_REQ((size_t)synth_slabs(d) * d->B * d->OT * L.KP < ((size_t)1 << 30) && (size_t)d->B * d->T * L.KP < ((size_t)1 << 30),
           "st_ae_bwd: batch too large for the kernel's 32-bit element offsets (B=%d)", d->B);
    const float expfac = expfac_of(d);
    const stg::RowMap live = synth_live(d);
    const int t_hi = live.t_lo + live.Tv - 1, nsl = synth_slabs(d);
    const size_t slab = (size_t)d->B * d->OT * L.KP;
    hipStream_t s = st_stream(stream);
    float* h4x = ws;
    float* da4x = ws + ae_h4_floats(d);
    float* parts = ws + 2 * ae_h4_floats(d);
    int grid = ae_bwd_grid(d);
    const int ht = ae_ht(d->prec);
    if (ae_use_split(d)) {
        if (!have_fwd)
            ST_TRY(ae_fwd_body(d, L, mag, phs, knobs, ae_m, ae_p, nullptr, nullptr, nullptr, nullptr, h4x, stream));
        grid = ae_split_grid(d);
        static_assert((size_t)sta::ae_split_lds_floats<1>(AE_SPLIT_NW) * sizeof(float) <= 160 * 1024 && (size_t)sta::ae_split_lds_floats<2>(AE_SPLIT_NW) * sizeof(float) <= 160 * 1024, "split ae_bwd LDS budget");
        auto part = [&](auto PART, auto HT, auto GM, auto KG) {
            return launch_lds("ae_bwd_part_kernel", sta::ae_bwd_part_kernel<AE_SPLIT_NW, PART(), HT(), GM(), KG()>, dim3(grid, 2), dim3(AE_SPLIT_NW * 64),
                              (size_t)sta::ae_split_lds_floats<PART()>(AE_SPLIT_NW) * sizeof(float), s,
                              mag, phs, knobs, ae_m, ae_p, L.go, L.PG, mag_hat, phs_hat, dAA, g_mag_hat, reg_coef, expfac, dmag, dphs, parts,
                              h4x, da4x, d->B, d->T, d->OT, d->F, d->K, L.KP, live.t_lo, t_hi, nsl, slab, kg); };
        auto halves = [&](auto HT, auto KG) -> int {
            ST_TRY(with_bool(g_mag_hat != nullptr, [&](auto GM) { return part(ic<1>{}, HT, GM, KG); }));
            ST_LAUNCHED("ae_bwd_dec");
            ST_TRY(part(ic<2>{}, HT, std::false_type{}, std::false_type{}));
            ST_LAUNCHED("ae_bwd_enc");
            return ST_OK; };
        if (kg) ST_TRY(with_ht16(ht, [&](auto HT) { return halves(HT, std::true_type{}); }));
        else ST_TRY(with_ht(ht, [&](auto HT) { return halves(HT, std::false_type{}); }));
    } else {
        const int var = g_mag_hat ? 1 : (d->T - d->OT == 16 ? 2 : 0);
        if (no_dinput) {
            if (have_fwd && ae_use_saved(d)) {
                const float* sv = ae_sv_ptr(d, L, ws);
                const float* img = (have_img && ae_img_level(d) == 2) ? ae_img_ptr(ws) : nullptr;
                ST_TRY(with_bool(var == 2, [&](auto T16) { return with_bool(img != nullptr, [&](auto IMG) {
                    return launch_lds("ae_bwd_kernel", sta::ae_bwd_kernel<AE_BWD_NW, false, 0, T16() ? 2 : 0, true, false, IMG(), true>, dim3(grid, 2), dim3(AE_BWD_NW * 64), lds, s,
                                      mag, phs, knobs, ae_m, ae_p, L.go, L.PG, mag_hat, phs_hat, dAA, g_mag_hat, reg_coef, expfac,
                                      dmag, dphs, parts, d->B, d->T, d->OT, d->F, d->K, L.KP, live.t_lo, t_hi, nsl, slab, sv, kg, img); }); }));
            } else
                ST_TRY(with_ht(ht, [&](auto HT) { return with_bool(var == 2, [&](auto T16) {
                    return launch_lds("ae_bwd_kernel", sta::ae_bwd_kernel<AE_BWD_NW, false, HT(), T16() ? 2 : 0, false, false, false, true>, dim3(grid, 2), dim3(AE_BWD_NW * 64), lds, s,
                                      mag, phs, knobs, ae_m, ae_p, L.go, L.PG, mag_hat, phs_hat, dAA, g_mag_hat, reg_coef, expfac,
                                      dmag, dphs, parts, d->B, d->T, d->OT, d->F, d->K, L.KP, live.t_lo, t_hi, nsl, slab, nullptr, nullptr, nullptr); }); }));
        } else
        if (have_fwd && ae_use_saved(d)) {
            const float* sv = ae_sv_ptr(d, L, ws);
            const float* img = (have_img && ae_img_level(d) == 2) ? ae_img_ptr(ws) : nullptr;
            ST_TRY(with_var(var, [&](auto VAR) { return with_bool(kg != nullptr, [&](auto KG) { return with_bool(img != nullptr, [&](auto IMG) {
                return launch_lds("ae_bwd_kernel", sta::ae_bwd_kernel<AE_BWD_NW, false, 0, VAR(), true, KG(), IMG()>, dim3(grid, 2), dim3(AE_BWD_NW * 64), lds, s,
                                  mag, phs, knobs, ae_m, ae_p, L.go, L.PG, mag_hat, phs_hat, dAA, g_mag_hat, reg_coef, expfac,
                                  dmag, dphs, parts, d->B, d->T, d->OT, d->F, d->K, L.KP, live.t_lo, t_hi, nsl, slab, sv, kg, img); }); }); }));
        } else
            ST_TRY(with_ht(ht, [&](auto HT) { return with_var(var, [&](auto VAR) {
                return launch_lds("ae_bwd_kernel", sta::ae_bwd_kernel<AE_BWD_NW, false, HT(), VAR()>, dim3(grid, 2), dim3(AE_BWD_NW * 64), lds, s,
                                  mag, phs, knobs, ae_m, ae_p, L.go, L.PG, mag_hat, phs_hat, dAA, g_mag_hat, reg_coef, expfac,
                                  dmag, dphs, parts, d->B, d->T, d->OT, d->F, d->K, L.KP, live.t_lo, t_hi, nsl, slab, nullptr, nullptr, nullptr); }); }));
        ST_LAUNCHED("ae_bwd");
    }
    if (defer_reduce && *defer_reduce) return ST_OK;
    hipLaunchKernelGGL(stm::ae_grad_reduce_kernel, dim3((L.PG + 63) / 64, 2), dim3(256), 0, s, parts, grid, L.PG, g_m, g_p);
    ST_LAUNCHED("ae_grad_reduce"); return ST_OK;
}
extern "C" int st_ae_bwd(const st_dims* d, const float* mag, const float* phs, const float* knobs,
                         const float* ae_m, const float* ae_p, const float* mag_hat, const float* phs_hat,
                         const float* dAA, const float* g_mag_hat, float reg_coef, float* dmag, float* dphs, float* ws,
                         float* g_m, float* g_p, void* stream)
{
    Layout L; ST_TRY(make_layout(d, &L));
    return ae_bwd_body(d, L, mag, phs, knobs, ae_m, ae_p, mag_hat, phs_hat, dAA, g_mag_hat, reg_coef, dmag, dphs, ws, g_m, g_p, false, stream);
}

extern "C" int st_polar_bwd(const st_dims* d, const float* re, const float* im, const float* dmag, const float* dphs,
                            const float* g_mag, float* dG, void* stream)
{
    ST_TRY(check_dims(d)); ST_REQ(re && im && dmag && dphs && dG, "st_polar_bwd: null pointer");
    const int R = d->B * d->T, KP = st_kp_of(d->F);
    hipLaunchKernelGGL(stm::polar_bwd_kernel, dim3((KP / 2 + 255) / 256, R), dim3(256), 0, st_stream(stream),
                       re, im, dmag, dphs, g_mag, dG, R, d->F, KP, gemm_ht(d->prec) == 2 ? 65504.0f : 0.0f);
    ST_LAUNCHED("polar_bwd"); return ST_OK;
}

static int analysis_wgrad_impl(const st_dims* d, const float* dG, const float* sig, bool padded, float in_scale, float* ws,
                               float* gWr, float* gWi, float* norm_partial, void* stream, int half = -1, float* stage = nullptr, int stage_bf16 = 0)
{
    const int KP = st_kp_of(d->F);
    const stg::RowMap ma = stg::live_frames(d->T, d->H, d->N, d->N, d->L);
    const int R = ma.rows(d->B);
    int ns = wgrad_split_tiles(R, KP, d->N);
    if (half >= 0) {
        const int tiles = ((KP / 2 + 95) / 96) * ((d->N + 95) / 96), cus = num_cus();
        int best = ns; double bf = -1.0;
        for (int c = ns; c >= (ns + 1) / 2 && c >= 1; --c) {
            const int w = tiles * c, rounds = (w + cus - 1) / cus;
            const double f = (double)w / ((double)rounds * cus);
            if (f > bf + 1e-9) { bf = f; best = c; }
        }
        ns = best;
    }
    const int M = half < 0 ? KP : KP / 2, m0 = half > 0 ? KP / 2 : 0;
    stm::NyqJob nyq{}; nyq.on = 0;
    const stg::TNOperand ta{dG, (unsigned)(d->T * KP), (unsigned)KP}, tb{sig, (unsigned)(d->L + 2 * d->N), (unsigned)d->H};
    if (half < 0 && use_tn128(d, padded) && stg::tn128_fits(ta, tb, sig, ma, d->N, d->N, (size_t)d->B * d->T * KP, (size_t)d->B * (d->L + 2 * d->N))) {
        ns = tn_split(R, d->N);
        const TNFrameMajor fm = tn_frame_major(ta, tb, ma, d->B, d->H, d->N, d->N, d->L, (g_tn_fm & 2) != 0);
        ST_TRY(wgrad_tn128(d, fm.a, fm.b, sig, fm.map, R, ws, ns, &nyq, stream, &fm.trim));
    } else {
        stg::PlainTN al{dG + m0, R, KP, M, ma};
        stg::StoreC ep{ws + (size_t)m0 * d->N, M, d->N, d->N, (size_t)KP * d->N, stg::all_frames(1)};
        if (padded) { stg::FramedTN<true> bl{sig, d->L, d->H, d->N, R, d->N, 1.0f, ma}; ST_GEMM_WG(al, bl, ep, M, d->N, R, ns, st_stream(stream)); }
        else { stg::FramedTN<false> bl{sig, d->L, d->H, d->N, R, d->N, in_scale, ma}; ST_GEMM_WG(al, bl, ep, M, d->N, R, ns, st_stream(stream)); }
    }
    ST_LAUNCHED("analysis_wgrad");
    const int nrows = half < 0 ? 2 * d->F : d->F, extra = half == 0 ? 0 : stm::nyq_blocks(d->N);
    hipLaunchKernelGGL(stm::wgrad_reduce_kernel, dim3(nrows + extra), dim3(256), 0, st_stream(stream),
                       ws, ns, gWr, gWi, norm_partial, d->N, d->F, KP, 0, half > 0 ? d->F : 0, nrows, stage, nyq, 0, stage_bf16);
    ST_LAUNCHED("analysis_wgrad_reduce");
    return ST_OK;
}
extern "C" int st_analysis_wgrad(const st_dims* d, const float* dG, const float* x, float in_scale, float* ws,
                                 float* gWr, float* gWi, float* norm_partial, void* stream)
{
    ST_TRY(check_dims(d)); ST_REQ(dG && x && ws && gWr && gWi && norm_partial, "st_analysis_wgrad: null pointer");
    return analysis_wgrad_impl(d, dG, x, false, in_scale, ws, gWr, gWi, norm_partial, stream);
}

static stm::FinArgs fin_args(const st_dims* d, const float* loss_partial, const float* reg_partial, const float* norm_a, const float* norm_s, float norm_scale)
{
    const float inv_y = 1.0f / ((float)d->B * (float)d->y);
    return stm::FinArgs{loss_partial, ola_loss_partials(d), reg_partial, ae_fwd_partials(d),
                        norm_a, norm_partials(d), norm_s, norm_s ? norm_partials(d) : 0, inv_y, reg_scale_of(d), norm_scale, nullptr, 0};
}
static int finalize_scalars(const st_dims* d, const float* loss_partial, const float* reg_partial,
                            const float* norm_a, const float* norm_s, float inv_world, float* scalars, void* stream)
{
    ST_REQ(scalars, "st_finalize_scalars: null pointer");
    stm::FinArgs f = fin_args(d, loss_partial, reg_partial, norm_a, norm_s, inv_world);
    f.n_ns = norm_partials(d);
    hipLaunchKernelGGL(stm::finalize_kernel, dim3(1), dim3(256), 0, st_stream(stream), f, scalars);
    ST_LAUNCHED("finalize_scalars"); return ST_OK;
}
extern "C" int st_finalize_scalars(const st_dims* d, const float* loss_partial, const float* reg_partial,
                                   const float* norm_a, const float* norm_s, float inv_world, float* scalars, void* stream)
{
    ST_TRY(check_dims(d));
    return finalize_scalars(d, loss_partial, reg_partial, norm_a, norm_s, inv_world, scalars, stream);
}

static int clip_adam_impl(float* params, float* grads, float* m, float* v, int64_t n_total, int64_t n_stft ,
                          float* scalars, float grad_scale, float lr, float beta1, float beta2, float eps, int step,
                          const stm::FinArgs* fin, void* stream, bool dev_hyper = false)
{
    ST_REQ(params && grads && m && v && scalars, "st_clip_adam: null pointer");
    ST_REQ(n_total > 0, "st_clip_adam: n_total must be positive (an empty range would be a zero-block launch)");
    ST_REQ(n_stft >= 0, "st_clip_adam: n_stft must not be negative");
    ST_REQ(n_total % 4 == 0 && n_stft % 4 == 0, "st_clip_adam: n_total and n_stft must be multiples of 4");
    ST_REQ(n_stft <= n_total, "st_clip_adam: n_stft exceeds n_total");
    ST_REQ(step >= 1, "st_clip_adam: step must be at least 1");
    const double bc1 = 1.0 - pow((double)beta1, step), bc2 = 1.0 - pow((double)beta2, step);
    const float neg_step = (float)(-(double)lr / bc1);
    const float bc2s = (float)sqrt(bc2);
    const float w1 = (float)(1.0 - (double)beta1), w2 = (float)(1.0 - (double)beta2);
    int grid = (int)((n_total / 4 + 255) / 256); if (grid > 2048) grid = 2048;
    if (dev_hyper) {
        ST_REQ(fin, "device-side hyper-parameters need the fused finalize");
        hipLaunchKernelGGL((stm::clip_adam_kernel<true, true>), dim3(grid), dim3(256), 0, st_stream(stream),
                           params, grads, m, v, n_total / 4, n_stft / 4, scalars, grad_scale, 0.f, w1, beta2, w2, 1.f, eps, *fin, beta1);
    } else if (fin)
        hipLaunchKernelGGL(stm::clip_adam_kernel<true>, dim3(grid), dim3(256), 0, st_stream(stream),
                           params, grads, m, v, n_total / 4, n_stft / 4, scalars, grad_scale, neg_step, w1, beta2, w2, bc2s, eps, *fin);
    else
        hipLaunchKernelGGL(stm::clip_adam_kernel<false>, dim3(grid), dim3(256), 0, st_stream(stream),
                           params, grads, m, v, n_total / 4, n_stft / 4, scalars, grad_scale, neg_step, w1, beta2, w2, bc2s, eps, stm::FinArgs{});
    ST_LAUNCHED("clip_adam"); return ST_OK;
}
extern "C" int st_clip_adam(float* params, float* grads, float* m, float* v, int64_t n_total, int64_t n_stft,
                            const float* scalars, float grad_scale, float lr, float beta1, float beta2, float eps, int step,
                            void* stream)
{
    return clip_adam_impl(params, grads, m, v, n_total, n_stft, const_cast<float*>(scalars), grad_scale, lr, beta1, beta2, eps, step, nullptr, stream);
}

struct WS {
    float *re, *im, *mag, *phs, *mag_hat, *phs_hat, *AA, *dAA, *Sfold, *SfoldT, *frs, *y_hat, *dsyn, *dmag, *dphs, *dG, *xp;
    float *wg, *wg2, *aews, *loss_p, *reg_p, *norm_a, *norm_s, *norm_e;
    unsigned short *pl_W, *pl_Sfold, *pl_SfoldT;
    unsigned short *xp16, *W16, *Sfold16, *SfoldT16, *AA16, *dsyn16, *dG16;
    int n_norm_e;
    bool g16;
    size_t bytes;
};
static void carve(const st_dims* d, const Layout& L, void* base, WS* w)
{
    const size_t RT = (size_t)d->B * d->T, RO = (size_t)d->B * d->OT, F = d->F, KP = st_kp_of(d->F), N = d->N;
    size_t off = 0;
    auto take = [&](size_t n) { float* p = base ? reinterpret_cast<float*>(base) + off : nullptr; off += (n + 63) / 64 * 64; return p; };
    w->re = take(RT * F); w->im = take(RT * F); w->mag = take(RT * F); w->phs = take(RT * F);
    w->mag_hat = take(RO * F); w->phs_hat = take(RO * F);
    const size_t nsl = synth_slabs(d), nfs = frame_slabs(d);
    w->AA = take(RO * KP); w->dAA = take(nsl * RO * KP);
    w->Sfold = take(KP * N); w->SfoldT = take(KP * N); w->frs = take(nfs * RO * N);
    w->y_hat = take((size_t)d->B * d->y); w->dsyn = take((size_t)d->B * (d->y + 2 * d->N));
    w->xp = take((size_t)d->B * (d->L + 2 * d->N));
    w->dmag = take(RT * F); w->dphs = take(RT * F); w->dG = take(RT * KP);
    w->wg = take(wgrad_ws_floats(d)); w->aews = take(ae_bwd_ws_floats(d, L));
    w->loss_p = take(ola_loss_partials(d)); w->reg_p = take(ae_fwd_partials(d));
    w->norm_a = take(norm_partials(d)); w->norm_s = take(norm_partials(d)); w->norm_e = take(NORM_E_MAX); w->n_norm_e = 0;
    auto take16 = [&](size_t n) { return reinterpret_cast<unsigned short*>(take((n + 1) / 2)); };
    w->pl_W = take16((size_t)3 * 2 * F * N); w->pl_Sfold = take16((size_t)3 * KP * N); w->pl_SfoldT = take16((size_t)3 * KP * N);
    w->xp16 = take16((size_t)d->B * (d->L + 2 * d->N) + 256); w->W16 = take16((size_t)2 * F * N); w->Sfold16 = take16(KP * N); w->SfoldT16 = take16(KP * N);
    w->AA16 = take16(RO * KP + 256); w->dsyn16 = take16((size_t)d->B * (d->y + 2 * d->N) + 256); w->dG16 = take16(RT * KP + 256);
    w->wg2 = take(synth_wgrad_ws_floats(d));
    w->g16 = false;
    w->bytes = off * sizeof(float);
}
extern "C" int st_workspace_offsets(const st_dims* d, int64_t* offs8)
{
    Layout L; ST_TRY(make_layout(d, &L)); ST_REQ(offs8, "st_workspace_offsets: null pointer");
    WS w; carve(d, L, reinterpret_cast<void*>(sizeof(float)), &w);
    float* base = reinterpret_cast<float*>(sizeof(float));
    float* p[8] = {w.re, w.im, w.mag, w.phs, w.mag_hat, w.phs_hat, w.AA, w.y_hat};
    for (int i = 0; i < 8; ++i) offs8[i] = (int64_t)(p[i] - base);
    return ST_OK;
}
extern "C" size_t st_ae_acts_floats(const st_dims* d)
{
    if (check_dims(d) != ST_OK) return 0;
    return (size_t)d->B * d->F * (64 + 32 + 16 + 16 + 16 + d->K + 16 + 16 + 32 + 64 + d->OT);
}
extern "C" int st_ae_acts(const st_dims* d, const float* v, const float* knobs, const float* ae, int sf, float* acts, void* stream)
{
    Layout L; ST_TRY(make_layout(d, &L));
    ST_REQ(v && (knobs || d->K == 0) && ae && acts, "st_ae_acts: null pointer");
    if (!knobs) knobs = ae;
    stm::AeActsArgs a;
    a.v = v; a.knobs = knobs; a.ae = ae; a.B = d->B; a.T = d->T; a.OT = d->OT; a.F = d->F; a.K = d->K; a.sf = sf;
    for (int l = 0; l < 9; ++l) { a.w_off[l] = L.go.w[l]; a.b_off[l] = L.go.b[l]; }
    int out[9], in[9], widths[10]; ae_shapes(d, out, in);
    for (int i = 0; i < 10; ++i) widths[i] = i < 4 ? out[i] : i == 4 ? in[4] : out[i - 1];
    size_t off = 0;
    for (int i = 0; i < 10; ++i) { a.out[i] = acts + off; off += (size_t)d->B * d->F * widths[i]; }
    hipLaunchKernelGGL(stm::ae_acts_kernel, dim3((d->B * d->F + 63) / 64), dim3(64), 0, st_stream(stream), a);
    ST_LAUNCHED("ae_acts"); return ST_OK;
}
extern "C" size_t st_workspace_bytes(const st_dims* d)
{
    Layout L; if (make_layout(d, &L) != ST_OK) return 0;
    WS w; carve(d, L, nullptr, &w); return w.bytes;
}
extern "C" size_t st_workspace_bytes_max(const st_dims* d)
{
    Layout L; if (make_layout(d, &L) != ST_OK) return 0;
    size_t best = 0;
    st_dims q = *d;
    for (int b = 1; b <= d->B; ++b)
        for (int prec = ST_PREC_F32; prec <= ST_PREC_F32X3; ++prec)
            for (int ca = 0; ca < 2; ++ca) {
                q.B = b; q.prec = prec; q.clip_all = ca;
                WS w; carve(&q, L, nullptr, &w);
// ... 198 lines not shown
    const bool planes = use_planes(d) && !w.g16;
    const bool polar_rows = !(wide_direct && y_true && !mag);
    float* const pmag = polar_rows ? w.mag : nullptr; float* const pphs = polar_rows ? w.phs : nullptr;
    if (w.g16) ST_TRY(analysis_fwd16(d, w, save ? w.re : nullptr, save ? w.im : nullptr, pmag, pphs, stream, &pwide));
    else if (planes) {
        ST_TRY(planes_prepare(d, Wr, Wi, w, stream));
        ST_TRY(analysis_fwd_planes(d, w, save ? w.re : nullptr, save ? w.im : nullptr, pmag, pphs, stream, &pwide));
    } else
    ST_TRY(analysis_fwd_impl(d, w.xp, true, Wr, Wi, 1.0f, save ? w.re : nullptr, save ? w.im : nullptr, pmag, pphs, stream, true, &pwide));
    float* const sv = (save && ae_use_saved(d)) ? ae_sv_ptr(d, L, w.aews) : nullptr;
    ST_TRY(ae_fwd_body(d, L, w.mag, w.phs, knobs, ae_m, ae_p, w.mag_hat, w.phs_hat, w.AA, w.reg_p,
                       (ae_is_wide(d) || (save && ae_use_split(d))) ? w.aews : nullptr, stream, w.g16 ? w.AA16 : nullptr, wide_direct, sv,
                       ae_img_level(d) ? ae_img_ptr(w.aews) : nullptr));
    if (w.g16) ST_TRY(synthesis_frames16(d, w, stream)); else
    if (planes) ST_TRY(synthesis_frames_planes(d, w, stream)); else
    ST_TRY(synthesis_frames_impl(d, w.AA, w.Sfold, w.SfoldT, w.frs, stream));
    ST_TRY(ola_loss_impl(d, w.frs, x, y_true, y_hat ? y_hat : w.y_hat, (save && y_true) ? w.dsyn : nullptr, d->N,
                         eval_p ? eval_p : y_true ? w.loss_p : nullptr, stream, w.g16 ? w.dsyn16 : nullptr, eval_p != nullptr));
    const size_t nm = (size_t)d->B * d->T * d->F * sizeof(float), nh = (size_t)d->B * d->OT * d->F * sizeof(float);
    if (mag && hipMemcpyAsync(mag, w.mag, nm, hipMemcpyDeviceToDevice, st_stream(stream)) != hipSuccess) return st_fail(ST_ERR_LAUNCH, "copy mag");
    if (mag_hat && hipMemcpyAsync(mag_hat, w.mag_hat, nh, hipMemcpyDeviceToDevice, st_stream(stream)) != hipSuccess) return st_fail(ST_ERR_LAUNCH, "copy mag_hat");
    return ST_OK;
}

static int wgrad16_and_reduce(Call& c, float* grads, bool synth, int half, float* stage, int stage_bf16, int* defer_slabs = nullptr)
{
    const st_dims* d = c.d; const Layout& L = c.L; WS& w = c.w; void* stream = c.stream;
    const int KP = L.KP, F = d->F, N = d->N;
    const stg::RowMap map = synth ? synth_live(d) : stg::live_frames(d->T, d->H, d->N, d->N, d->L);
    const int R = map.rows(d->B);
    int ns = g16_wsplit(d, R);
    if (half >= 0) {
        const int room = (int)((wgrad_ws_floats(d) - (size_t)64 * 2 * N) / ((size_t)KP * N));
        const int tiles = ((KP / 2 + 127) / 128) * (N / 128);
        ns = (2 * num_cus()) / (tiles > 0 ? tiles : 1);
        if (ns > R / 128) ns = R / 128; if (ns > room) ns = room; if (ns < 1) ns = 1;
    }
    if (synth) ST_TRY(wgrad16(d, w.AA16, (unsigned)(d->OT * KP), w.dsyn16, (unsigned)(d->y + 2 * N), map, R, w.wg, ns, stream, 0, -1, (g_g16_crop & 4) ? d->y : 0));
    else ST_TRY(wgrad16(d, w.dG16, (unsigned)(d->T * KP), w.xp16, (unsigned)(d->L + 2 * N), map, R, w.wg, ns, stream, half > 0 ? KP / 2 : 0, half < 0 ? -1 : KP / 2, (g_g16_crop & 8) ? d->L : 0));
    ST_LAUNCHED(synth ? "synthesis_wgrad" : "analysis_wgrad");
    if (defer_slabs) { *defer_slabs = ns; return ST_OK; }
    stm::NyqJob nq{}; nq.on = 0;
    float* const g0 = grads + L.offs[synth ? 2 : 0]; float* const g1 = grads + L.offs[synth ? 3 : 1];
    const int per = stm::nyq_blocks(N) / 2;
    if (half < 0) hipLaunchKernelGGL(stm::wgrad_reduce_kernel, dim3(norm_partials(d)), dim3(256), 0, st_stream(stream),
                                     w.wg, ns, g0, g1, synth ? w.norm_s : w.norm_a, N, F, KP, synth ? 1 : 0, 0, 2 * F, stage, nq, 0, stage_bf16);
    else hipLaunchKernelGGL(stm::wgrad_reduce_kernel, dim3(F + per), dim3(256), 0, st_stream(stream),
                            w.wg, ns, g0, g1, w.norm_a, N, F, KP, 0, half * F, F, stage, nq, half * per, stage_bf16);
    ST_LAUNCHED(synth ? "synthesis_wgrad_reduce" : "analysis_wgrad_reduce");
    return ST_OK;
}
static const int ST_STAGE_EVERY = ST_STAGE_SYN_DGRAD | ST_STAGE_SYN_WGRAD | ST_STAGE_AE_BWD | ST_STAGE_AE_DINPUT | ST_STAGE_ANA_WGRAD;
static int backward_syn(Call& c, float* grads, int* defer_slabs = nullptr, stm::NyqJob* defer_nyq = nullptr, int stages = ST_STAGE_EVERY)
{
    const st_dims* d = c.d; const Layout& L = c.L; WS& w = c.w; void* stream = c.stream;
    const bool dgrad = (stages & ST_STAGE_SYN_DGRAD) != 0, wgrad = (stages & ST_STAGE_SYN_WGRAD) != 0;
    if (w.g16) {
        if (dgrad) ST_TRY(synthesis_dgrad16(d, w, stream));
        if (defer_slabs && defer_nyq) { *defer_nyq = stm::NyqJob{}; defer_nyq->on = 0; }
        return wgrad ? wgrad16_and_reduce(c, grads, true, -1, nullptr, 0, defer_slabs) : ST_OK;
    }
    if (dgrad) {
    if (use_planes(d) && g_pl_dgrad) ST_TRY(synthesis_dgrad_planes(d, w, stream)); else
    ST_TRY(synthesis_dgrad_impl(d, w.dsyn, true, w.Sfold, w.dAA, stream));
    }
    if (!wgrad) return ST_OK;
    return synthesis_wgrad_impl(d, w.AA, w.dsyn, true, w.wg, grads + L.offs[2], grads + L.offs[3], w.norm_s, stream, defer_slabs, defer_nyq);
}
static int backward_ae(Call& c, const float* params, float* grads, const float* g_mag_hat, const float* g_mag, float reg_coef, int syn_slabs = 0,
                       const stm::NyqJob* syn_nyq = nullptr, float* kg = nullptr, int stages = ST_STAGE_EVERY)
{
    const st_dims* d = c.d; const Layout& L = c.L; WS& w = c.w; void* stream = c.stream;
    const float* ae_m = params + L.offs[4]; const float* ae_p = params + L.offs[22];
    bool deferred = true;
    const PolarSink sink{w.re, w.im, g_mag, w.g16 ? nullptr : w.dG, w.g16 ? w.dG16 : nullptr};
    stw::SynReduce syn{};
    if (syn_slabs > 0 && ae_is_wide(d)) {
        syn.wg = w.wg; syn.nz = syn_slabs; syn.gSr = grads + L.offs[2]; syn.gSi = grads + L.offs[3]; syn.norm_s = w.norm_s; syn.N = d->N; syn.F = d->F; syn.KP = L.KP;
        syn.nyq = stm::NyqJob{}; syn.nyq.on = 0; if (syn_nyq) syn.nyq = *syn_nyq;
    }
    ST_TRY(ae_bwd_body(d, L, w.mag, w.phs, c.knobs, ae_m, ae_p, w.mag_hat, w.phs_hat, w.dAA, g_mag_hat, reg_coef, w.dmag, w.dphs,
                       w.aews, grads + L.offs[4], grads + L.offs[22], true, stream, &deferred, &sink, syn.wg ? &syn : nullptr,
                       (d->clip_all && ae_is_wide(d)) ? w.norm_e : nullptr, &w.n_norm_e, kg, true, !(stages & ST_STAGE_AE_DINPUT)));
    if (!deferred) return ST_OK;
    stm::PostAeArgs a;
    a.ws = w.aews + 2 * ae_h4_floats(d); a.nparts = ae_use_split(d) ? ae_split_grid(d) : ae_bwd_grid(d); a.PG = L.PG; a.g_m = grads + L.offs[4]; a.g_p = grads + L.offs[22];
    a.n_red_x = (L.PG + 63) / 64; a.n_red = 2 * a.n_red_x;
    a.re = w.re; a.im = w.im; a.dmag = w.dmag; a.dphs = w.dphs; a.g_mag = g_mag; a.dG = w.dG; a.F = d->F; a.KP = L.KP;
    a.gx = (L.KP / 2 + 255) / 256; a.sat = gemm_ht(d->prec) == 2 ? 65504.0f : 0.0f;
    a.n_polar = a.gx * d->B * d->T;
    a.polar_total = 0; a.polar_magic = 0;
    if (stm::polar_flat_ok((long long)d->B * d->T, L.KP / 2)) {
        a.polar_total = (unsigned)((long long)d->B * d->T * (L.KP / 2)); a.polar_magic = stm::polar_magic(L.KP / 2);
        a.n_polar = (int)((a.polar_total + 256 * stm::POLAR_EPT - 1) / (256 * stm::POLAR_EPT));
    }
    a.wg = w.wg; a.wg_nz = syn_slabs; a.gSr = grads + L.offs[2]; a.gSi = grads + L.offs[3]; a.norm_s = w.norm_s; a.N = d->N;
    a.nyq = stm::NyqJob{}; a.nyq.on = 0; if (syn_nyq) a.nyq = *syn_nyq;
    a.dG16 = nullptr; a.ht = 0;
    if (w.g16) { a.dG16 = w.dG16; a.ht = gemm_ht(d->prec); a.dG = nullptr; }
    a.norm_e = nullptr;
    if (d->clip_all && a.n_red <= NORM_E_MAX) { a.norm_e = w.norm_e; w.n_norm_e = a.n_red; }
    if (!(stages & ST_STAGE_AE_DINPUT)) a.n_polar = 0;
    hipLaunchKernelGGL(stm::post_ae_kernel, dim3(a.n_red + a.n_polar + (syn_slabs > 0 ? norm_partials(d) : 0)), dim3(256), 0, st_stream(stream), a);
    if (!(stages & ST_STAGE_AE_DINPUT)) { ST_LAUNCHED("post_ae_reduce"); return ST_OK; }
    ST_LAUNCHED("post_ae");
    return ST_OK;
}
static int backward_p1(Call& c, const float* params, float* grads, const float* g_mag_hat, const float* g_mag, float reg_coef, float* kg = nullptr, int stages = ST_STAGE_EVERY)
{
    if (!(stages & ST_STAGE_AE_BWD)) return backward_syn(c, grads, nullptr, nullptr, stages);
    int syn_slabs = 0; stm::NyqJob syn_nyq{}; syn_nyq.on = 0;
    ST_TRY(backward_syn(c, grads, &syn_slabs, &syn_nyq, stages));
    return backward_ae(c, params, grads, g_mag_hat, g_mag, reg_coef, syn_slabs, &syn_nyq, kg, stages);
}
static int backward_p2(Call& c, float* grads, float* stage = nullptr, int stage_bf16 = 0)
{
    if (c.w.g16) return wgrad16_and_reduce(c, grads, false, -1, stage, stage_bf16);
    return analysis_wgrad_impl(c.d, c.w.dG, c.w.xp, true, 1.0f, c.w.wg, grads + c.L.offs[0], grads + c.L.offs[1], c.w.norm_a, c.stream, -1, stage, stage_bf16);
}
static int analysis_wgrad_half(Call& c, float* grads, int half, float* stage, int stage_bf16, stm::NyqJob* nyq_io)
{
    const st_dims* d = c.d; const Layout& L = c.L; WS& w = c.w; void* stream = c.stream;
    const int KP = st_kp_of(d->F), F = d->F, N = d->N, m0 = half ? KP / 2 : 0;
    const stg::RowMap ma = stg::live_frames(d->T, d->H, d->N, d->N, d->L);
    const int R = ma.rows(d->B);
    const int room = (int)((wgrad_ws_floats(d) - (size_t)64 * 2 * N) / ((size_t)KP * N));
    const int per = stm::nyq_blocks(N) / 2;
    int ns;
    const stg::TNOperand ta{w.dG + m0, (unsigned)(d->T * KP), (unsigned)KP}, tb{w.xp, (unsigned)(d->L + 2 * d->N), (unsigned)d->H};
    if (w.g16) {
        if (!half) { *nyq_io = stm::NyqJob{}; nyq_io->on = 0; }
        return wgrad16_and_reduce(c, grads, false, half, stage, stage_bf16);
    }
    if (use_tn128(d, true) && stg::tn128_fits(ta, tb, w.xp, ma, N / 2, N, (size_t)d->B * d->T * KP, (size_t)d->B * (d->L + 2 * d->N))) {
        const int mh = (N / 2) / 128, tiles = mh * (N / 128);
        ns = num_cus() / (tiles > 0 ? tiles : 1); if (ns > 16) ns = 16; if (ns > R / 64) ns = R / 64; if (ns > room) ns = room; if (ns < 1) ns = 1;
        float* part = w.wg + (size_t)room * KP * N;
        int P = 0;
        const TNFrameMajor fm = tn_frame_major(ta, tb, ma, d->B, d->H, N, N, d->L, (g_tn_fm & 2) != 0);
        ST_TN128(fm.a, fm.b, w.xp, fm.map, R, N / 2, mh, (unsigned)(KP / 2), N, w.wg + (size_t)m0 * N, N, (size_t)KP * N, ns, st_stream(stream),
                 half ? nullptr : part, (unsigned)(F - 1), (unsigned)(KP / 2 + F - 1), &P, &fm.trim);
        if (!half) { nyq_io->part = part; nyq_io->P = P; nyq_io->on = 1; }
    } else {
        ST_LAUNCHED("analysis_wgrad");
        if (!half) { *nyq_io = stm::NyqJob{}; nyq_io->on = 0; }
        return analysis_wgrad_impl(d, w.dG, w.xp, true, 1.0f, w.wg, grads + L.offs[0], grads + L.offs[1], w.norm_a, stream, half, stage, stage_bf16);
    }
    ST_LAUNCHED("analysis_wgrad");
    hipLaunchKernelGGL(stm::wgrad_reduce_kernel, dim3(F + per), dim3(256), 0, st_stream(stream),
                       w.wg, ns, grads + L.offs[0], grads + L.offs[1], w.norm_a, N, F, KP, 0, half * F, F, stage, *nyq_io, half * per, stage_bf16);
    ST_LAUNCHED("analysis_wgrad_reduce");
    return ST_OK;
}
static int backward_impl(Call& c, const float* params, float* grads, const float* g_mag_hat, const float* g_mag, float reg_coef, float* kg = nullptr)
{
    ST_TRY(backward_p1(c, params, grads, g_mag_hat, g_mag, reg_coef, kg));
    return backward_p2(c, grads);
}

extern "C" int st_model_fwd(const st_dims* d, const float* params, const float* x, const float* knobs,
                            float* y_hat, float* mag, float* mag_hat, void* ws, int save_for_backward, void* stream)
{
    Call c; ST_TRY(call_begin(&c, d, params, knobs, ws, stream, FP32_OPERANDS));
    ST_REQ(params && x && (knobs || d->K == 0) && ws, "st_model_fwd: null pointer");
    return forward_impl(c, params, x, nullptr, y_hat, mag, mag_hat, save_for_backward != 0);
}

extern "C" int st_model_bwd(const st_dims* d, const float* params, float* grads, const float* x, const float* knobs,
                            const float* g_y_hat, const float* g_mag_hat, const float* g_mag, void* ws, void* stream)
{
    Call c; ST_TRY(call_begin(&c, d, params, knobs, ws, stream, FP32_OPERANDS));
    ST_REQ(params && grads && x && (knobs || d->K == 0) && g_y_hat && ws, "st_model_bwd: null pointer");
    ST_TRY(pad_scale(g_y_hat, c.w.dsyn, d->B, d->y, d->N, 2.0f, stream));
    return backward_impl(c, params, grads, g_mag_hat, g_mag, 0.0f);
}

__global__ void knob_grad_kernel(const float* __restrict__ Wm, const float* __restrict__ gbm, const float* __restrict__ Wp, const float* __restrict__ gbp,
                                 const int K, float* __restrict__ out, const int ng)
{
    __shared__ float gb[32];
    const int k = threadIdx.x;
    if (k < 32) {
        const float* p = (k < 16 ? gbm : gbp) + (size_t)blockIdx.x * ng * 16 + (k & 15);
        float a = p[0];
        for (int j = 1; j < ng; ++j) a += p[j * 16];
        gb[k] = a;
    }
    __syncthreads();
    if (k >= K) return;
    float s = 0.f, t = 0.f;
    for (int o = 0; o < 16; ++o) { s += Wm[o * (16 + K) + 16 + k] * gb[o]; t += Wp[o * (16 + K) + 16 + k] * gb[16 + o]; }
    out[(size_t)blockIdx.x * K + k] = s + t;
}
extern "C" int st_model_knob_grad(const st_dims* d, const float* params, float* grads_scratch, const float* x, const float* knobs,
                                  const float* g_y_hat, const float* g_mag_hat, const float* g_mag, void* ws, float* g_knobs, void* stream)
{
    Layout L; ST_TRY(make_layout(d, &L));
    ST_REQ(params && grads_scratch && x && knobs && g_y_hat && ws && g_knobs, "st_model_knob_grad: null pointer");
    ST_REQ(d->K >= 1 && d->K <= 64, "st_model_knob_grad: K = %d", d->K);
    st_dims d1 = *d; d1.B = 1;
    Layout L1; ST_TRY(make_layout(&d1, &L1));
    const size_t w5 = (size_t)L1.offs[4] + (size_t)L1.go.w[4], b5 = (size_t)L1.offs[4] + (size_t)L1.go.b[4];
    for (int b = 0; b < d->B; ++b) {
        const float* xb = x + (size_t)b * d->L; const float* kb = knobs + (size_t)b * d->K;
        ST_TRY(st_model_fwd(&d1, params, xb, kb, nullptr, nullptr, nullptr, ws, 1, stream));
        ST_TRY(st_model_bwd(&d1, params, grads_scratch, xb, kb, g_y_hat + (size_t)b * d->y, g_mag_hat ? g_mag_hat + (size_t)b * d->OT * d->F : nullptr,
                            g_mag ? g_mag + (size_t)b * d->T * d->F : nullptr, ws, stream));
        hipLaunchKernelGGL(knob_grad_kernel, dim3(1), dim3(64), 0, st_stream(stream), params + w5, grads_scratch + b5, params + w5 + L1.PG, grads_scratch + b5 + L1.PG,
                           d->K, g_knobs + (size_t)b * d->K, 1);
    }
    ST_LAUNCHED("knob_grad");
    return ST_OK;
}

extern "C" int st_knob_grad_fused_supported(const st_dims* d)
{
    if (check_dims(d) != ST_OK) return 0;
    if (d->K < 1) { (void)st_fail(ST_ERR_ARG, "st_model_bwd_knobs: K = %d (a model without knobs has no knob gradient)", d->K); return 0; }
    if (!ae_kg_route(d)) { (void)st_fail(ST_ERR_UNSUPPORTED, "st_model_bwd_knobs: no per-group d a5 output on this autoencoder backward route (%s)", ae_kg_why(d)); return 0; }
    return 1;
}
extern "C" size_t st_model_bwd_knobs_ws_floats(const st_dims* d)
{
    if (check_dims(d) != ST_OK) return 0;
    return (size_t)2 * ae_fwd_groups(d) * 16;
}
extern "C" int st_model_bwd_knobs(const st_dims* d, const float* params, float* grads, const float* x, const float* knobs,
                                  const float* g_y_hat, const float* g_mag_hat, const float* g_mag, void* ws, float* scratch, float* g_knobs, void* stream)
{
    Call c; ST_TRY(call_begin(&c, d, params, knobs, ws, stream, FP32_OPERANDS));
    const Layout& L = c.L;
    ST_REQ(params && grads && x && knobs && g_y_hat && ws && scratch && g_knobs, "st_model_bwd_knobs: null pointer");
    ST_REQ(d->K >= 1, "st_model_bwd_knobs: K = %d (a model without knobs has no knob gradient)", d->K);
    if (!ae_kg_route(d)) return st_fail(ST_ERR_UNSUPPORTED, "st_model_bwd_knobs: no per-group d a5 output on this autoencoder backward route (%s)", ae_kg_why(d));
    ST_TRY(pad_scale(g_y_hat, c.w.dsyn, d->B, d->y, d->N, 2.0f, stream));
    ST_TRY(backward_impl(c, params, grads, g_mag_hat, g_mag, 0.0f, scratch));
    const size_t w5 = (size_t)L.offs[4] + (size_t)L.go.w[4];
    const int gpw = L.KP / 32;
    hipLaunchKernelGGL(knob_grad_kernel, dim3(d->B), dim3(64), 0, st_stream(stream), params + w5, (const float*)scratch, params + w5 + L.PG,
                       (const float*)scratch + (size_t)ae_fwd_groups(d) * 16, d->K, g_knobs, gpw);
    ST_LAUNCHED("knob_grad");
    return ST_OK;
}

extern "C" int st_loss_backward(const st_dims* d, const float* params, float* grads, const float* x, const float* knobs,
                                const float* y_true, float* y_hat, float* mag, float* mag_hat, void* ws,
                                float* scalars, void* stream)
{
    Call c; ST_TRY(call_begin(&c, d, params, knobs, ws, stream, G16_PIPELINE));
    ST_REQ(params && grads && x && (knobs || d->K == 0) && y_true && ws && scalars, "st_loss_backward: null pointer");
    prof_mark("begin", stream);
    ST_TRY(forward_impl(c, params, x, y_true, y_hat, mag, mag_hat, true));
    ST_TRY(backward_impl(c, params, grads, nullptr, nullptr, reg_coef_of(d)));
    return finalize_scalars(d, c.w.loss_p, c.w.reg_p, c.w.norm_a, c.w.norm_s, 1.0f / loss_scale_of(d), scalars, stream);
}

extern "C" int st_eval_step(const st_dims* d, const float* params, const float* x, const float* knobs, const float* y_true,
                            float* y_hat, void* ws, double* acc, double beta, void* stream)
{
    Call c; ST_TRY(call_begin(&c, d, params, knobs, ws, stream, G16_PIPELINE));
    ST_REQ(params, "st_eval_step: null pointer (params)"); ST_REQ(x, "st_eval_step: null pointer (x)");
    ST_REQ(knobs || d->K == 0, "st_eval_step: null pointer (knobs, K = %d)", d->K);
    ST_REQ(y_true, "st_eval_step: null pointer (y_true)"); ST_REQ(ws, "st_eval_step: null pointer (ws)"); ST_REQ(acc, "st_eval_step: null pointer (acc)");
    prof_mark("begin", stream);
    float* const eval_p = c.w.dsyn;
    ST_TRY(forward_impl(c, params, x, y_true, y_hat, nullptr, nullptr, false, eval_p));
    const stm::FinArgs f = fin_args(d, eval_p, c.w.reg_p, nullptr, nullptr, 1.0f);
    hipLaunchKernelGGL(stm::eval_finalize_kernel, dim3(1), dim3(256), 0, st_stream(stream), f, beta, acc);
    ST_LAUNCHED("eval_finalize"); return ST_OK;
}

extern "C" int st_loss_backward_p1(const st_dims* d, const float* params, float* grads, const float* x, const float* knobs,
                                   const float* y_true, void* ws, void* stream)
{
    Call c; ST_TRY(call_begin(&c, d, params, knobs, ws, stream, G16_PIPELINE));
    ST_REQ(params && grads && x && (knobs || d->K == 0) && y_true && ws, "st_loss_backward_p1: null pointer");
    prof_mark("begin", stream);
    ST_TRY(forward_impl(c, params, x, y_true, nullptr, nullptr, nullptr, true));
    return backward_p1(c, params, grads, nullptr, nullptr, reg_coef_of(d));
}
extern "C" int st_loss_backward_p2(const st_dims* d, float* grads, const float* x, void* ws, float* scalars, void* stream)
{
    Call c; ST_TRY(call_begin(&c, d, nullptr, nullptr, ws, stream, G16_PIPELINE));
    ST_REQ(grads && x && ws && scalars, "st_loss_backward_p2: null pointer");
    ST_TRY(backward_p2(c, grads));
    return finalize_scalars(d, c.w.loss_p, c.w.reg_p, c.w.norm_a, c.w.norm_s, 1.0f / loss_scale_of(d), scalars, stream);
}

extern "C" int st_loss_backward_p2_staged(const st_dims* d, float* grads, float* stage, const float* x, void* ws, float* scalars, void* stream)
{
    Call c; ST_TRY(call_begin(&c, d, nullptr, nullptr, ws, stream, G16_PIPELINE));
    ST_REQ(grads && stage && x && ws && scalars, "st_loss_backward_p2_staged: null pointer");
    (void)scalars;
    return backward_p2(c, grads, stage);
}
extern "C" int st_unstage_analysis(const st_dims* d, float* grads, const float* stage, void* stream)
{
    Layout L; ST_TRY(make_layout(d, &L));
    ST_REQ(grads && stage, "st_unstage_analysis: null pointer");
    const size_t live = (size_t)d->F * d->N * sizeof(float);
    if (hipMemcpyAsync(grads + L.offs[0], stage, live, hipMemcpyDeviceToDevice, st_stream(stream)) != hipSuccess ||
        hipMemcpyAsync(grads + L.offs[1], stage + (size_t)d->F * d->N, live, hipMemcpyDeviceToDevice, st_stream(stream)) != hipSuccess)
        return st_fail(ST_ERR_LAUNCH, "st_unstage_analysis: copy failed");
    return ST_OK;
}

extern "C" int st_loss_backward_stage(const st_dims* d, const float* params, float* grads, const float* x, const float* knobs,
                                      const float* y_true, void* ws, float* scalars, int stage, void* stream)
// ... 894 lines not shown
```

### signaltrain_amd/csrc/st_gemm_tn.h

```cpp
#pragma once
#include "st_gemm.h"

#ifndef ST_G128_ABLATE
#define ST_G128_ABLATE 0
#endif
#define ST_G128_KEEP4(v_) asm volatile("" :: "v"((v_)[0]), "v"((v_)[1]), "v"((v_)[2]), "v"((v_)[3]))

namespace stg {

struct TNJob {
    const float* base;
    unsigned a0, b0;
    unsigned SA1, SA2, SB1, SB2;
    unsigned magic; int Tv, t_lo;
    int K;
    unsigned zero;
    int mh; unsigned mstride;
    float* nyq_out; unsigned nyq_c0, nyq_c1; int nyq_P, Nc, nsplit;
    int trim, fB; unsigned char fa[64], fb[64];
};
struct FrameTrim { int on, B; unsigned char fa[64], fb[64]; };
static inline FrameTrim frame_trim(const RowMap& live, int B, int H, int Ntaps, int pad, int Ls)
{
    FrameTrim f; f.on = (Ntaps % 128 == 0 && Ntaps / 128 <= 64 && live.Tv <= 255) ? 1 : 0; f.B = B;
    for (int j = 0; j < 64; ++j) { f.fa[j] = 0; f.fb[j] = (unsigned char)(live.Tv <= 255 ? live.Tv : 255); }
    if (!f.on) return f;
    for (int j = 0; j < Ntaps / 128; ++j) {
        const int n0 = 128 * j;
        int a = 0, b = live.Tv;
        while (a < b && H * (live.t_lo + a) + n0 + 127 < pad) ++a;
        while (b > a && H * (live.t_lo + b - 1) + n0 >= pad + Ls) --b;
        f.fa[j] = (unsigned char)a; f.fb[j] = (unsigned char)b;
    }
    return f;
}

__device__ __forceinline__ void nyq_partial(const TNJob& j, const int p)
{
    if (p >= j.nyq_P) return;
    const int per = (j.K + j.nyq_P - 1) / j.nyq_P, k0 = p * per, k1 = (k0 + per < j.K) ? k0 + per : j.K;
    for (int n4 = threadIdx.x; n4 < j.Nc / 4; n4 += 256) {
        float4 s0 = make_float4(0.f, 0.f, 0.f, 0.f), s1 = s0;
        for (int kb = k0; kb < k1; kb += 8) {
            float a0[8], a1[8]; float4 x[8];
#pragma unroll
            for (int u = 0; u < 8; ++u) {
                const int k = kb + u < k1 ? kb + u : k1 - 1;
                const unsigned w = __umulhi((unsigned)k, j.magic), t = (unsigned)j.t_lo + ((unsigned)k - w * (unsigned)j.Tv);
                const float* arow = j.base + j.a0 + (size_t)w * j.SA1 + (size_t)t * j.SA2;
                a0[u] = kb + u < k1 ? arow[j.nyq_c0] : 0.f; a1[u] = kb + u < k1 ? arow[j.nyq_c1] : 0.f;
                x[u] = *reinterpret_cast<const float4*>(j.base + j.b0 + (size_t)w * j.SB1 + (size_t)t * j.SB2 + 4 * n4);
            }
#pragma unroll
            for (int u = 0; u < 8; ++u) {
                s0.x = __builtin_fmaf(a0[u], x[u].x, s0.x); s0.y = __builtin_fmaf(a0[u], x[u].y, s0.y); s0.z = __builtin_fmaf(a0[u], x[u].z, s0.z); s0.w = __builtin_fmaf(a0[u], x[u].w, s0.w);
                s1.x = __builtin_fmaf(a1[u], x[u].x, s1.x); s1.y = __builtin_fmaf(a1[u], x[u].y, s1.y); s1.z = __builtin_fmaf(a1[u], x[u].z, s1.z); s1.w = __builtin_fmaf(a1[u], x[u].w, s1.w);
            }
        }
        float* o = j.nyq_out + (size_t)p * 2 * j.Nc + 4 * n4;
        *reinterpret_cast<float4*>(o) = s0;
        *reinterpret_cast<float4*>(o + j.Nc) = s1;
    }
}

template <int BKT, bool PIPE = false, bool UNI = false>
__global__ void __launch_bounds__(256) __attribute__((amdgpu_waves_per_eu(1, 2)))
gemm_tn128_kernel(const TNJob j, float* __restrict__ out, const int ldo, const size_t slab, const int ksplit)
{
    constexpr int TS = BKT * 128;
    constexpr int NP = BKT / 8;
    constexpr int KS = BKT / 2;
    extern __shared__ __attribute__((aligned(16))) float tn_lds[];
    float* const As = tn_lds;
    float* const Bs = tn_lds + 2 * TS;

    const int tid = threadIdx.x, lane = tid & 63, wave = tid >> 6, wm = wave >> 1, wn = wave & 1;
    if ((int)blockIdx.z >= j.nsplit) { nyq_partial(j, (int)(blockIdx.y * gridDim.x + blockIdx.x)); return; }
    int tbx, tby, tbz; xcd_tile(tbx, tby, tbz, j.nsplit);
    const unsigned rowA = (unsigned)(tby % j.mh) * 128u + (unsigned)(tby / j.mh) * j.mstride;
    const unsigned colB = (unsigned)tbx * 128u;
    int k_begin = tbz * ksplit;
    int k_end = (k_begin + ksplit < j.K) ? k_begin + ksplit : j.K;
    if (j.trim) {
        const int lo = (int)j.fa[tbx] * j.fB, hi = (int)j.fb[tbx] * j.fB;
        const int per = ((hi - lo + j.nsplit - 1) / j.nsplit + BKT - 1) / BKT * BKT;
        k_begin = lo + tbz * per;
        k_end = (k_begin + per < hi) ? k_begin + per : hi;
    }

    const int c4 = tid & 31, kr = tid >> 5;
    const unsigned la = 4u * (j.a0 + rowA + 4u * (unsigned)c4), lb = 4u * (j.b0 + colB + 4u * (unsigned)c4), lz = 4u * (j.zero + 4u * (unsigned)c4);
    const unsigned sa1 = 4u * j.SA1, sa2 = 4u * j.SA2, sb1 = 4u * j.SB1, sb2 = 4u * j.SB2;
    float4 ra[NP], rb[NP];
    auto ld = [&](const unsigned byte_off) { return *reinterpret_cast<const float4*>(reinterpret_cast<const char*>(j.base) + byte_off); };
    auto gload_pass = [&](const int kt, const int p) {
        const int k = kt + kr + 8 * p;
        const unsigned kc = (unsigned)(k < j.K ? k : j.K - 1);
        const unsigned b = __umulhi(kc, j.magic);
        const unsigned t = (unsigned)j.t_lo + kc - __umul24(b, (unsigned)j.Tv);
        const unsigned oa = __umul24(b, sa1) + __umul24(t, sa2) + la;
        const unsigned ob = __umul24(b, sb1) + __umul24(t, sb2) + lb;
        const unsigned live = (unsigned)((k - j.K) >> 31);
        ra[p] = ld((oa & live) | (lz & ~live));
        rb[p] = ld(ob);
    };
    auto gload = [&](const int kt) {
#pragma unroll
        for (int p = 0; p < NP; ++p) gload_pass(kt, p);
    };
    auto lstore_pass = [&](const int buf, const int p) {
        float* as = As + buf * TS + kr * 128 + 4 * c4;
        float* bs = Bs + buf * TS + kr * 128 + 4 * c4;
        *reinterpret_cast<float4*>(as + p * 8 * 128) = ra[p];
        *reinterpret_cast<float4*>(bs + p * 8 * 128) = rb[p];
    };
    auto lstore = [&](const int buf) {
#pragma unroll
        for (int p = 0; p < NP; ++p) lstore_pass(buf, p);
    };

    f32x16 acc[2][2];
#pragma unroll
    for (int mi = 0; mi < 2; ++mi)
#pragma unroll
        for (int nj = 0; nj < 2; ++nj)
#pragma unroll
            for (int i = 0; i < 16; ++i) acc[mi][nj][i] = 0.f;

    const int h = lane >> 5, l31 = lane & 31;
    if constexpr (PIPE) {
        constexpr int PAIRS = KS / 2;
        static_assert(PAIRS % 2 == 0 && NP + 1 <= PAIRS - 1, "fragment buffers alternate by pair; stores and loads sit before the barrier");
        const int ntiles = (k_end - k_begin + BKT - 1) / BKT;
        if (ntiles > 0) {
            const int k_last = k_begin + (ntiles - 1) * BKT;
            unsigned ua[UNI ? NP : 1], ub[UNI ? NP : 1];
            if constexpr (UNI) {
#pragma unroll
                for (int p = 0; p < NP; ++p) { ua[p] = la + (unsigned)(kr + 8 * p) * sa2; ub[p] = lb + (unsigned)(kr + 8 * p) * sb2; }
            }
            auto gl = [&](const int kt, const int p) {
                if constexpr (UNI) {
                    const unsigned b = __umulhi((unsigned)kt, j.magic), t0 = (unsigned)j.t_lo + (unsigned)kt - b * (unsigned)j.Tv;
                    ra[p] = ld(b * sa1 + t0 * sa2 + ua[p]);
                    rb[p] = ld(b * sb1 + t0 * sb2 + ub[p]);
                } else gload_pass(kt, p);
            };
            const int a_off = h * 128 + wm * 64 + 2 * l31;
            const int b_off = h * 128 + wn * 64 + 2 * l31;
            float2 fa[2][2], fb[2][2];
            auto frag = [&](const int stage, const int pr, const int buf) {
                const float* as = As + stage * TS + a_off;
                const float* bs = Bs + stage * TS + b_off;
#pragma unroll
                for (int u = 0; u < 2; ++u) {
                    fa[buf][u] = *reinterpret_cast<const float2*>(as + (2 * pr + u) * 256);
                    fb[buf][u] = *reinterpret_cast<const float2*>(bs + (2 * pr + u) * 256);
                }
            };
            auto mfma8 = [&](const int buf) {
#pragma unroll
                for (int u = 0; u < 2; ++u) {
                    const float2 a = fa[buf][u], b = fb[buf][u];
                    acc[0][0] = __builtin_amdgcn_mfma_f32_32x32x2f32(a.x, b.x, acc[0][0], 0, 0, 0);
                    acc[0][1] = __builtin_amdgcn_mfma_f32_32x32x2f32(a.x, b.y, acc[0][1], 0, 0, 0);
                    acc[1][0] = __builtin_amdgcn_mfma_f32_32x32x2f32(a.y, b.x, acc[1][0], 0, 0, 0);
                    acc[1][1] = __builtin_amdgcn_mfma_f32_32x32x2f32(a.y, b.y, acc[1][1], 0, 0, 0);
                }
            };
#pragma unroll
            for (int p = 0; p < NP; ++p) gl(k_begin, p);
            lstore(0);
#pragma unroll
            for (int p = 0; p < NP; ++p) gl(ntiles > 1 ? k_begin + BKT : k_begin, p);
            __syncthreads();
            frag(0, 0, 0);
            int cur = 0;
            for (int i = 0; i < ntiles; ++i) {
                const int k2 = k_begin + (i + 2) * BKT, kn = k2 < k_last ? k2 : k_last;
                __builtin_amdgcn_sched_barrier(0);
#pragma unroll
                for (int pr = 0; pr < PAIRS - 1; ++pr) {
                    frag(cur, pr + 1, (pr + 1) & 1);
                    if (pr < NP) lstore_pass(cur ^ 1, pr);
                    if (pr >= 1 && pr <= NP) gl(kn, pr - 1);
                    mfma8(pr & 1);
                    __builtin_amdgcn_sched_barrier(0);
                }
                __syncthreads();
                frag(cur ^ 1, 0, 0);
                mfma8(1);
                __builtin_amdgcn_sched_barrier(0);
                cur ^= 1;
            }
        }
    } else if (k_begin < k_end) {
        gload(k_begin);
        lstore(0);
        __syncthreads();
        int cur = 0;
        const int a_off = h * 128 + wm * 64 + 2 * l31;
        const int b_off = h * 128 + wn * 64 + 2 * l31;
        float2 abl_f[4];
#pragma unroll
        for (int u = 0; u < 4; ++u) abl_f[u] = (ST_G128_ABLATE & 2) ? *reinterpret_cast<const float2*>(As + a_off + u * 256) : make_float2(0.f, 0.f);
        for (int kt = k_begin; kt < k_end; kt += BKT) {
            const bool more = kt + BKT < k_end;
            if (!(ST_G128_ABLATE & 8)) gload(more ? kt + BKT : kt);
            __builtin_amdgcn_sched_barrier(0);
            const float* as = As + cur * TS + a_off;
            const float* bs = Bs + cur * TS + b_off;
            float2 fa[2][2], fb[2][2];
            auto frag = [&](const int pr, const int buf) {
#pragma unroll
                for (int u = 0; u < 2; ++u) {
                    if (ST_G128_ABLATE & 2) { fa[buf][u] = abl_f[(2 * buf + u) & 3]; fb[buf][u] = abl_f[(2 * buf + u + 1) & 3]; continue; }
                    fa[buf][u] = *reinterpret_cast<const float2*>(as + (2 * pr + u) * 256);
                    fb[buf][u] = *reinterpret_cast<const float2*>(bs + (2 * pr + u) * 256);
                }
            };
            frag(0, 0);
#pragma unroll
            for (int pr = 0; pr < KS / 2; ++pr) {
                if (pr + 1 < KS / 2) frag(pr + 1, (pr + 1) & 1);
#pragma unroll
                for (int u = 0; u < 2; ++u) {
                    const float2 a = fa[pr & 1][u], b = fb[pr & 1][u];
                    acc[0][0] = __builtin_amdgcn_mfma_f32_32x32x2f32(a.x, b.x, acc[0][0], 0, 0, 0);
                    acc[0][1] = __builtin_amdgcn_mfma_f32_32x32x2f32(a.x, b.y, acc[0][1], 0, 0, 0);
                    acc[1][0] = __builtin_amdgcn_mfma_f32_32x32x2f32(a.y, b.x, acc[1][0], 0, 0, 0);
                    acc[1][1] = __builtin_amdgcn_mfma_f32_32x32x2f32(a.y, b.y, acc[1][1], 0, 0, 0);
                }
            }
            __builtin_amdgcn_sched_group_barrier(0x100, 2, 0);
#pragma unroll
            for (int pr = 0; pr < KS / 2; ++pr) {
                if (pr + 1 < KS / 2) __builtin_amdgcn_sched_group_barrier(0x100, 2, 0);
                __builtin_amdgcn_sched_group_barrier(0x008, 8, 0);
            }
            __builtin_amdgcn_sched_barrier(0);
            if (!(ST_G128_ABLATE & 4)) lstore(cur ^ 1);
            else {
#pragma unroll
                for (int p = 0; p < NP; ++p) { asm volatile("" :: "v"(ra[p].x), "v"(ra[p].y), "v"(ra[p].z), "v"(ra[p].w)); asm volatile("" :: "v"(rb[p].x), "v"(rb[p].y), "v"(rb[p].z), "v"(rb[p].w)); }
            }
            if (!(ST_G128_ABLATE & 1)) __syncthreads();
            cur ^= 1;
        }
    }
    float* o = out + (size_t)tbz * slab + (size_t)(rowA + wm * 64) * ldo + colB + wn * 64 + 2 * l31;
#pragma unroll
    for (int i = 0; i < 16; ++i) {
        const int r = 2 * d_row(i, lane);
#pragma unroll
        for (int mi = 0; mi < 2; ++mi)
            *reinterpret_cast<float2*>(o + (size_t)(r + mi) * ldo) = make_float2(acc[mi][0][i], acc[mi][1][i]);
    }
}

struct TNOperand { const float* base; unsigned S1, S2; };
static inline bool tn128_fits(const TNOperand& A, const TNOperand& B, const float* zeros, const RowMap& map, int M, int Nc, size_t extentA, size_t extentB)
{
    if (M % 128 || Nc % 128 || map.Tv < 2) return false;
    const unsigned lim24 = 1u << 22;
    if (A.S1 >= lim24 || A.S2 >= lim24 || B.S1 >= lim24 || B.S2 >= lim24) return false;
    const float* lo = A.base < B.base ? A.base : B.base; if (zeros < lo) lo = zeros;
    const size_t lim = (size_t)1 << 30;
    return (size_t)(A.base - lo) + extentA < lim && (size_t)(B.base - lo) + extentB < lim && (size_t)(zeros - lo) + 128 < lim;
}
static inline bool tn128_uniform(const RowMap& map, int K, int bkt, const FrameTrim* trim)
{
    if (map.Tv % bkt || K % bkt) return false;
    return !(trim && trim->on) || trim->B % bkt == 0;
}
template <int BKT, bool PIPE = false>
static inline int launch_tn128(const TNOperand& A, const TNOperand& B, const float* zeros, const RowMap& map, int K,
                               int M, int mh, unsigned mstride, int Nc, float* out, int ldo, size_t slab, int nsplit, hipStream_t s,
                               float* nyq_out = nullptr, unsigned nyq_c0 = 0, unsigned nyq_c1 = 0, int* nyq_P = nullptr, const FrameTrim* trim = nullptr)
{
    const float* lo = A.base < B.base ? A.base : B.base; if (zeros < lo) lo = zeros;
    TNJob j;
    j.base = lo; j.a0 = (unsigned)(A.base - lo); j.b0 = (unsigned)(B.base - lo); j.zero = (unsigned)(zeros - lo);
    j.SA1 = A.S1; j.SA2 = A.S2; j.SB1 = B.S1; j.SB2 = B.S2;
    j.magic = map.magic; j.Tv = map.Tv; j.t_lo = map.t_lo; j.K = K; j.mh = mh; j.mstride = mstride;
    j.trim = (trim && trim->on) ? 1 : 0; j.fB = trim ? trim->B : 0;
    for (int i = 0; i < 64; ++i) { j.fa[i] = trim ? trim->fa[i] : 0; j.fb[i] = trim ? trim->fb[i] : 0; }
    int ksplit = K;
    if (nsplit > 1) ksplit = st_round_up((K + nsplit - 1) / nsplit, BKT);
    constexpr size_t lds = (size_t)4 * BKT * 128 * sizeof(float);
    static_assert(lds <= 65536, "the Nyquist side workgroups share a CU with a GEMM workgroup: 2 x 64 KB of the 160");
    const int nz = nsplit > 1 ? nsplit : 1, tiles = (Nc / 128) * (M / 128);
    j.nsplit = nz; j.Nc = Nc; j.nyq_out = nyq_out; j.nyq_c0 = nyq_c0; j.nyq_c1 = nyq_c1;
    j.nyq_P = tiles < 64 ? tiles : 64; { const int W = K / 8 > 0 ? K / 8 : 1; if (j.nyq_P > W) j.nyq_P = W; }
    if (nyq_P) *nyq_P = j.nyq_P;
    const dim3 grid(Nc / 128, M / 128, nz + (nyq_out ? 1 : 0));
    if (!PIPE) hipLaunchKernelGGL((gemm_tn128_kernel<BKT>), grid, dim3(256), lds, s, j, out, ldo, slab, ksplit);
    else if (tn128_uniform(map, K, BKT, trim)) hipLaunchKernelGGL((gemm_tn128_kernel<BKT, PIPE, PIPE>), grid, dim3(256), lds, s, j, out, ldo, slab, ksplit);
    else hipLaunchKernelGGL((gemm_tn128_kernel<BKT, PIPE, false>), grid, dim3(256), lds, s, j, out, ldo, slab, ksplit);
    return 0;
}

}

namespace stg {

struct NTRows { const float* base; unsigned S1, S2, magic; int Tv, t_lo, R; };
__device__ __forceinline__ unsigned ntrows_off(const NTRows& o, const int r)
{
    const unsigned rc = (unsigned)(r < o.R ? r : o.R - 1);
    const unsigned b = o.magic ? __umulhi(rc, o.magic) : rc;
    const unsigned t = o.magic ? (unsigned)o.t_lo + (rc - b * (unsigned)o.Tv) : 0u;
    return b * o.S1 + t * o.S2;
}
static inline NTRows ntrows_frame_major(const float* base, unsigned s_window, unsigned s_frame, const RowMap& live, int B, int R)
{
    return NTRows{base + (size_t)live.t_lo * s_frame, s_frame, s_window, B > 1 ? rowmap_magic(B) : 0u, B, 0, R};
}

constexpr int NTW_MAX = 768;
struct NTWork {
    int n, nslabs;
    int col_h, col_stride;
    int kunit, kt_total;
    unsigned nyq_b[2], nyq_col[2];
    unsigned e[NTW_MAX];
};
static inline unsigned ntw_pack(int mt, int nt, int z, int zf, int kind, int k0, int kl)
{
    return (unsigned)mt | (unsigned)nt << 8 | (unsigned)z << 14 | (unsigned)zf << 16 | (unsigned)kind << 18 | (unsigned)k0 << 19 | (unsigned)kl << 25;
}

struct StoreSlab {
    float* out; int M, Nc, ld; size_t slab; RowMap map;
    __device__ void operator()(const int z, const int m0, const int n0, const f32x16 (&acc)[2]) const {
        const int lane = threadIdx.x & 63;
        float* o = out + (size_t)z * slab;
#pragma unroll
        for (int i = 0; i < 16; ++i) {
            const int row = m0 + d_row(i, lane);
            if (row < M) {
                float* orow = o + (size_t)map.full(row) * ld;
#pragma unroll
                for (int j = 0; j < 2; ++j) {
                    const int col = n0 + 32 * j + (lane & 31);
                    if (col < Nc) orow[col] = acc[j][i];
                }
            }
        }
    }
};

__device__ __forceinline__ void nt128_nyquist(const NTRows& ra, const NTRows& rb, const StoreSlab& epi, const NTWork& wk, const int m_blk, const int k_begin, const int k_end)
{
    const int lane = threadIdx.x & 63, wave = threadIdx.x >> 6;
    const float* b0 = rb.base + wk.nyq_b[0];
    const float* b1 = rb.base + wk.nyq_b[1];
    for (int r0 = wave; r0 < 128; r0 += 16) {
        float s0[4], s1[4];
        const float* a[4];
#pragma unroll
        for (int u = 0; u < 4; ++u) { s0[u] = 0.f; s1[u] = 0.f; a[u] = ra.base + ntrows_off(ra, m_blk + r0 + 4 * u); }
        for (int k = k_begin + 4 * lane; k < k_end; k += 256) {
            const f32x4 vb0 = *reinterpret_cast<const f32x4*>(b0 + k), vb1 = *reinterpret_cast<const f32x4*>(b1 + k);
            f32x4 va[4];
#pragma unroll
            for (int u = 0; u < 4; ++u) va[u] = *reinterpret_cast<const f32x4*>(a[u] + k);
#pragma unroll
            for (int u = 0; u < 4; ++u) {
                s0[u] += (va[u][0] * vb0[0] + va[u][1] * vb0[1]) + (va[u][2] * vb0[2] + va[u][3] * vb0[3]);
                s1[u] += (va[u][0] * vb1[0] + va[u][1] * vb1[1]) + (va[u][2] * vb1[2] + va[u][3] * vb1[3]);
            }
        }
#pragma unroll
        for (int u = 0; u < 4; ++u) {
#pragma unroll
            for (int m = 32; m >= 1; m >>= 1) { s0[u] += __shfl_xor(s0[u], m); s1[u] += __shfl_xor(s1[u], m); }
            const int row = m_blk + r0 + 4 * u;
            if (lane < 2 && row < epi.M) {
                float* o = epi.out + (size_t)epi.map.full(row) * epi.ld + wk.nyq_col[lane];
                o[0] = lane ? s1[u] : s0[u];
                for (int z = 1; z < wk.nslabs; ++z) o[(size_t)z * epi.slab] = 0.f;
            }
        }
    }
}

__global__ void __launch_bounds__(256)
gemm_nt128_kernel(const NTRows ra, const NTRows rb, const StoreSlab epi, const NTWork wk)
{
    constexpr int BKT = 32, LD = BKT + 4, TS = 128 * LD;
    constexpr int NP = 4;
    extern __shared__ __attribute__((aligned(16))) float nt_lds[];
    float* const As = nt_lds;
    float* const Bs = nt_lds + 2 * TS;
    const int tid = threadIdx.x, lane = tid & 63, wave = tid >> 6, wm = wave >> 1, wn = wave & 1;
    const unsigned ent = wk.e[blockIdx.x];
    const int m_blk = (int)(ent & 255u) * 128, n_blk = (int)((ent >> 8) & 63u) * 128, tbz = (int)((ent >> 14) & 3u), zf = (int)((ent >> 16) & 3u);
    const int k_begin = (int)((ent >> 19) & 63u) * wk.kunit * BKT;
    int k_end = k_begin + (int)(ent >> 25) * wk.kunit * BKT;
    if (k_end > wk.kt_total * BKT) k_end = wk.kt_total * BKT;
    if ((ent >> 18) & 1u) { nt128_nyquist(ra, rb, epi, wk, m_blk, k_begin, k_end); return; }

    const int lr = tid >> 3, lk = (tid & 7) * 4;
    unsigned ao[NP], bo[NP];
#pragma unroll
    for (int p = 0; p < NP; ++p) {
        ao[p] = 4u * (ntrows_off(ra, m_blk + lr + 32 * p) + (unsigned)lk);
        bo[p] = 4u * (ntrows_off(rb, n_blk + lr + 32 * p) + (unsigned)lk);
    }
    f32x4 va[NP], vb[NP];
    auto gload = [&](const int kt) {
        const char* pa = reinterpret_cast<const char*>(ra.base) + 4 * (size_t)kt;
        const char* pb = reinterpret_cast<const char*>(rb.base) + 4 * (size_t)kt;
#pragma unroll
        for (int p = 0; p < NP; ++p) {
            va[p] = *reinterpret_cast<const f32x4*>(pa + ao[p]);
            vb[p] = *reinterpret_cast<const f32x4*>(pb + bo[p]);
        }
    };
    auto lstore = [&](const int buf) {
        float* as = As + buf * TS + lr * LD + lk;
        float* bs = Bs + buf * TS + lr * LD + lk;
#pragma unroll
        for (int p = 0; p < NP; ++p) {
            *reinterpret_cast<f32x4*>(as + p * 32 * LD) = va[p];
            *reinterpret_cast<f32x4*>(bs + p * 32 * LD) = vb[p];
        }
    };
    f32x16 acc[2][2];
#pragma unroll
    for (int mi = 0; mi < 2; ++mi)
#pragma unroll
        for (int nj = 0; nj < 2; ++nj)
#pragma unroll
            for (int i = 0; i < 16; ++i) acc[mi][nj][i] = 0.f;

    if (k_begin < k_end) {
        gload(k_begin);
        lstore(0);
        __syncthreads();
        int cur = 0;
        const int h = lane >> 5, l31 = lane & 31;
        const int a_off = (wm * 64 + l31) * LD + 16 * h, b_off = (wn * 64 + l31) * LD + 16 * h;
        f32x4 abl_f[4];
#pragma unroll
        for (int u = 0; u < 4; ++u) abl_f[u] = (ST_G128_ABLATE & 2) ? *reinterpret_cast<const f32x4*>(As + a_off + 4 * u) : f32x4{0.f, 0.f, 0.f, 0.f};
        for (int kt = k_begin; kt < k_end; kt += BKT) {
            const bool more = kt + BKT < k_end;
            if (!(ST_G128_ABLATE & 8)) gload(more ? kt + BKT : kt);
            __builtin_amdgcn_sched_barrier(0);
            const float* as = As + cur * TS + a_off;
// ... 165 lines not shown
```

### signaltrain_amd/csrc/st_misc.h

```cpp
#pragma once
#include "st_common.h"
#include "st_ae.h"

namespace stm {

__device__ __forceinline__ void fold_row(const float* __restrict__ Sr, const float* __restrict__ Si, float* __restrict__ Sfold,
                                         const int N, const int F, const int KP, const int row)
{
    const int half = KP / 2;
    const bool is_im = row >= half;
    const int k = is_im ? row - half : row;
    const float* S = is_im ? Si : Sr;
    const bool valid = k < F;
    const bool paired = valid && k >= 1 && k <= F - 2;
    const float sgn = is_im ? -1.f : 1.f;
    for (int n4 = threadIdx.x; n4 < N / 4; n4 += blockDim.x) {
        float4 v = make_float4(0.f, 0.f, 0.f, 0.f);
        if (valid) {
            v = reinterpret_cast<const float4*>(S + (size_t)k * N)[n4];
            if (paired) {
                const float4 u = reinterpret_cast<const float4*>(S + (size_t)(N - k) * N)[n4];
                v.x += sgn * u.x; v.y += sgn * u.y; v.z += sgn * u.z; v.w += sgn * u.w;
            }
        }
// ... 337 lines not shown
        gim = dm * bb * inv + dp * rp / den;
        if (sat > 0.f) { gre = __builtin_amdgcn_fmed3f(gre, -sat, sat); gim = __builtin_amdgcn_fmed3f(gim, -sat, sat); }
    }
    if (dG16) { dG16[(size_t)r * KP + c] = st_to_h16(gre, ht); dG16[(size_t)r * KP + half + c] = st_to_h16(gim, ht); }
    if (dG) { dG[(size_t)r * KP + c] = gre; dG[(size_t)r * KP + half + c] = gim; }
}
constexpr int POLAR_EPT = 4;
__host__ __device__ static inline unsigned polar_magic(int half) { return (unsigned)((0x100000000ull + (unsigned)half - 1) / (unsigned)half); }
__host__ static inline bool polar_flat_ok(long long R, int half)
{
    const unsigned long long M = polar_magic(half), slack = M * (unsigned)half - 0x100000000ull;
    const unsigned long long total = (unsigned long long)R * (unsigned)half;
    return total < 0x7fffffffull && (slack == 0 || total < 0x100000000ull / slack);
}
__device__ __forceinline__ void polar_bwd_flat(const float* __restrict__ re, const float* __restrict__ im, const float* __restrict__ dmag,
                 const float* __restrict__ dphs, const float* __restrict__ g_mag, float* __restrict__ dG, const int F, const int KP, const float sat,
                 const unsigned bx, const unsigned total, const unsigned magic, unsigned short* __restrict__ dG16, const int ht)
{
    const unsigned half = (unsigned)KP / 2;
    unsigned r[POLAR_EPT], c[POLAR_EPT]; bool on[POLAR_EPT], live[POLAR_EPT];
    float a[POLAR_EPT], bb[POLAR_EPT], dm[POLAR_EPT], dp[POLAR_EPT];
#pragma unroll
    for (int u = 0; u < POLAR_EPT; ++u) {
        const unsigned e = (bx * POLAR_EPT + u) * 256 + threadIdx.x;
        on[u] = e < total;
        r[u] = __umulhi(on[u] ? e : 0u, magic); c[u] = (on[u] ? e : 0u) - r[u] * half;
        live[u] = on[u] && c[u] < (unsigned)F;
        const size_t i = live[u] ? (size_t)r[u] * F + c[u] : 0;
        a[u] = re[i]; bb[u] = im[i]; dm[u] = dmag[i] + (g_mag ? g_mag[i] : 0.f); dp[u] = dphs[i];
    }
#pragma unroll
    for (int u = 0; u < POLAR_EPT; ++u) {
        float gre = 0.f, gim = 0.f;
        if (live[u]) {
            const float mg = sqrtf(a[u] * a[u] + bb[u] * bb[u]);
            const float inv = mg > 0.f ? 1.0f / mg : 0.f;
            const float rp = a[u] + 1e-7f;
            const float den = rp * rp + bb[u] * bb[u];
            gre = dm[u] * a[u] * inv - dp[u] * bb[u] / den;
            gim = dm[u] * bb[u] * inv + dp[u] * rp / den;
            if (sat > 0.f) { gre = __builtin_amdgcn_fmed3f(gre, -sat, sat); gim = __builtin_amdgcn_fmed3f(gim, -sat, sat); }
        }
        if (on[u]) {
            const size_t o = (size_t)r[u] * KP + c[u];
            if (dG16) { dG16[o] = st_to_h16(gre, ht); dG16[o + half] = st_to_h16(gim, ht); }
            if (dG) { dG[o] = gre; dG[o + half] = gim; }
        }
    }
}
__global__ void __launch_bounds__(256)
polar_bwd_kernel(const float* __restrict__ re, const float* __restrict__ im, const float* __restrict__ dmag,
                 const float* __restrict__ dphs, const float* __restrict__ g_mag, float* __restrict__ dG, int R, int F, int KP, const float sat,
                 unsigned short* __restrict__ dG16 = nullptr, const int ht = 0)
{
    polar_bwd_block(re, im, dmag, dphs, g_mag, dG, F, KP, sat, blockIdx.x, blockIdx.y, dG16, ht);
}

struct NyqJob {
    const float* part; int P;
    int on;
};
__device__ __forceinline__ void stage_store4(float* __restrict__ stage, const size_t elem, const float4 v, const int bf16)
{
    if (bf16) {
        typedef __bf16 bf16x2_t __attribute__((ext_vector_type(2)));
        typedef float f32x2_t __attribute__((ext_vector_type(2)));
        union { bf16x2_t h; unsigned u; } lo, hi;
        lo.h = __builtin_convertvector((f32x2_t){v.x, v.y}, bf16x2_t); hi.h = __builtin_convertvector((f32x2_t){v.z, v.w}, bf16x2_t);
        *reinterpret_cast<uint2*>(reinterpret_cast<unsigned short*>(stage) + elem) = make_uint2(lo.u, hi.u);
    } else *reinterpret_cast<float4*>(stage + elem) = v;
}
constexpr int NYQ_CW = 256;
__host__ __device__ static inline int nyq_blocks(int N) { return 2 * ((N + NYQ_CW - 1) / NYQ_CW); }
__host__ __device__ static inline int norm_partial_count(int F, int N) { return 2 * F + nyq_blocks(N); }
__device__ __forceinline__ void
nyquist_chunk(const NyqJob& q, float* __restrict__ gRe, float* __restrict__ gIm, float* __restrict__ norm_partial,
              const int N, const int F, const int blk, const int slot, float* __restrict__ stage, const int stage_bf16 = 0)
{
    __shared__ float4 part[4][64];
    __shared__ float red[4];
    const int per = (N + NYQ_CW - 1) / NYQ_CW;
    const bool is_im = blk >= per;
    const int n4 = (is_im ? blk - per : blk) * (NYQ_CW / 4) + (threadIdx.x & 63), grp = threadIdx.x >> 6;
    float4 v = make_float4(0.f, 0.f, 0.f, 0.f);
    if (4 * n4 < N)
        for (int p0 = grp; p0 < q.P; p0 += 32) {
            float4 u[8];
#pragma unroll
            for (int j = 0; j < 8; ++j) { const int p = p0 + 4 * j < q.P ? p0 + 4 * j : grp; u[j] = *reinterpret_cast<const float4*>(q.part + ((size_t)p * 2 + (is_im ? 1 : 0)) * N + 4 * n4); }
#pragma unroll
            for (int j = 0; j < 8; ++j) if (p0 + 4 * j < q.P) { v.x += u[j].x; v.y += u[j].y; v.z += u[j].z; v.w += u[j].w; }
        }
    part[grp][threadIdx.x & 63] = v;
    __syncthreads();
    float na = 0.f;
    if (threadIdx.x < 64 && 4 * n4 < N) {
        const float4 a = part[0][threadIdx.x], b = part[1][threadIdx.x], c = part[2][threadIdx.x], d = part[3][threadIdx.x];
        v = make_float4((a.x + b.x) + (c.x + d.x), (a.y + b.y) + (c.y + d.y), (a.z + b.z) + (c.z + d.z), (a.w + b.w) + (c.w + d.w));
        *reinterpret_cast<float4*>((is_im ? gIm : gRe) + (size_t)(F - 1) * N + 4 * n4) = v;
        if (stage) stage_store4(stage, (size_t)((is_im ? F : 0) + F - 1) * N + 4 * n4, v, stage_bf16);
        na = fabsf(v.x) + fabsf(v.y) + fabsf(v.z) + fabsf(v.w);
    }
    const float tot = block_sum<4>(na, red);
    if (threadIdx.x == 0) norm_partial[slot] = tot;
}
__device__ __forceinline__ void
wgrad_reduce_block(const float* __restrict__ ws, int nz, float* __restrict__ gRe, float* __restrict__ gIm,
                   float* __restrict__ norm_partial, int N, int F, int KP, int mode, const int row, float* __restrict__ stage, const NyqJob& nyq,
                   const int stage_bf16 = 0)
{
    __shared__ float red[4];
    if (row >= 2 * F) {
        if (nyq.on) nyquist_chunk(nyq, gRe, gIm, norm_partial, N, F, row - 2 * F, row, stage, stage_bf16);
        else if (threadIdx.x == 0) norm_partial[row] = 0.f;
        return;
    }
    const bool is_im = row >= F;
    const int k = is_im ? row - F : row;
    if (nyq.on && k == F - 1) { if (threadIdx.x == 0) norm_partial[row] = 0.f; return; }
    const int src = is_im ? KP / 2 + k : k;
    float* g = is_im ? gIm : gRe;
    const bool mirror = mode == 1 && k >= 1 && k <= F - 2;
    const float sgn = is_im ? -1.f : 1.f;
    const size_t slab = (size_t)KP * N;
    float na = 0.f;
    for (int n4 = threadIdx.x; n4 < N / 4; n4 += blockDim.x) {
        float4 v = make_float4(0.f, 0.f, 0.f, 0.f);
        for (int z0 = 0; z0 < nz; z0 += 8) {
            float4 u[8];
#pragma unroll
            for (int j = 0; j < 8; ++j) { const int z = z0 + j < nz ? z0 + j : nz - 1; u[j] = reinterpret_cast<const float4*>(ws + z * slab + (size_t)src * N)[n4]; }
#pragma unroll
            for (int j = 0; j < 8; ++j) if (z0 + j < nz) { v.x += u[j].x; v.y += u[j].y; v.z += u[j].z; v.w += u[j].w; }
        }
        reinterpret_cast<float4*>(g + (size_t)k * N)[n4] = v;
        if (stage) stage_store4(stage, (size_t)row * N + 4 * n4, v, stage_bf16);
        float a = fabsf(v.x) + fabsf(v.y) + fabsf(v.z) + fabsf(v.w);
        if (mirror) {
            reinterpret_cast<float4*>(g + (size_t)(N - k) * N)[n4] = make_float4(sgn * v.x, sgn * v.y, sgn * v.z, sgn * v.w);
            a *= 2.f;
        }
        na += a;
    }
    const float tot = block_sum<4>(na, red);
    if (threadIdx.x == 0) norm_partial[row] = tot;
}
__global__ void __launch_bounds__(256)
wgrad_reduce_kernel(const float* __restrict__ ws, int nz, float* __restrict__ gRe, float* __restrict__ gIm,
                    float* __restrict__ norm_partial, int N, int F, int KP, int mode, int row0, int nrows, float* __restrict__ stage, const NyqJob nyq,
                    const int extra0 = 0, const int stage_bf16 = 0)
{
    const int row = (int)blockIdx.x < nrows ? (int)blockIdx.x + row0 : 2 * F + extra0 + ((int)blockIdx.x - nrows);
    wgrad_reduce_block(ws, nz, gRe, gIm, norm_partial, N, F, KP, mode, row, stage, nyq, stage_bf16);
}

__global__ void __launch_bounds__(256)
l1_partial_kernel(const float* __restrict__ g, int64_t n, float scale, float* __restrict__ partial)
{
    __shared__ float red[4];
    float a = 0.f;
    const int64_t n4 = n / 4;
    for (int64_t i = (int64_t)blockIdx.x * 256 + threadIdx.x; i < n4; i += (int64_t)gridDim.x * 256) {
        const float4 v = reinterpret_cast<const float4*>(g)[i];
        a += fabsf(v.x * scale) + fabsf(v.y * scale) + fabsf(v.z * scale) + fabsf(v.w * scale);
    }
    const float tot = block_sum<4>(a, red);
    if (threadIdx.x == 0) partial[blockIdx.x] = tot;
}

__global__ void __launch_bounds__(256)
unstage_l1_kernel(const float* __restrict__ stage, float* __restrict__ gRe, float* __restrict__ gIm, const int F, const int N, const float scale,
                  float* __restrict__ partial, const int n_partial, const int stage_bf16 = 0)
{
    __shared__ float red[4];
    const int row = blockIdx.x;
    const bool is_im = row >= F;
    float* dst = (is_im ? gIm : gRe) + (size_t)(is_im ? row - F : row) * N;
    const float* src = stage + (size_t)row * N;
    float a = 0.f;
    for (int i = threadIdx.x; i < N / 4; i += 256) {
        float4 v;
        if (stage_bf16) {
            const uint2 u = *reinterpret_cast<const uint2*>(reinterpret_cast<const unsigned short*>(stage) + (size_t)row * N + 4 * i);
            v = make_float4(__uint_as_float(u.x << 16), __uint_as_float(u.x & 0xffff0000u), __uint_as_float(u.y << 16), __uint_as_float(u.y & 0xffff0000u));
        } else v = reinterpret_cast<const float4*>(src)[i];
        reinterpret_cast<float4*>(dst)[i] = v;
        a += fabsf(v.x * scale) + fabsf(v.y * scale) + fabsf(v.z * scale) + fabsf(v.w * scale);
    }
    const float tot = block_sum<4>(a, red);
    if (threadIdx.x == 0) partial[row] = tot;
    if (row == 2 * F - 1) for (int j = 2 * F + threadIdx.x; j < n_partial; j += 256) partial[j] = 0.f;
}

__device__ __forceinline__ void ae_grad_reduce_block(const float* __restrict__ ws, const int nparts, const int PG,
                                                     float* __restrict__ g_m, float* __restrict__ g_p, const int bx, const int ae,
                                                     float* __restrict__ norm_out = nullptr, const int slot = 0)
{
    __shared__ float red[4][64];
    const int col = threadIdx.x & 63, pl = threadIdx.x >> 6;
    const int i = bx * 64 + col;
    float s = 0.f;
    if (i < PG) {
        const float* base = ws + (size_t)ae * PG + i;
        const size_t stride = (size_t)2 * PG;
        for (int p0 = pl; p0 < nparts; p0 += 32) {
            float v[8];
#pragma unroll
            for (int u = 0; u < 8; ++u) { const int p = p0 + 4 * u; v[u] = p < nparts ? base[(size_t)p * stride] : 0.f; }
#pragma unroll
            for (int u = 0; u < 8; ++u) s += v[u];
        }
    }
    red[pl][col] = s;
    __syncthreads();
    if (pl != 0) return;
    const float r = i < PG ? (red[0][col] + red[1][col]) + (red[2][col] + red[3][col]) : 0.f;
    if (i < PG) (ae ? g_p : g_m)[i] = r;
    if (norm_out) { const float t = wave_sum(fabsf(r)); if (col == 0) norm_out[slot] = t; }
}
__global__ void __launch_bounds__(256)
ae_grad_reduce_kernel(const float* __restrict__ ws, int nparts, int PG, float* __restrict__ g_m, float* __restrict__ g_p)
{
    ae_grad_reduce_block(ws, nparts, PG, g_m, g_p, blockIdx.x, blockIdx.y);
}
struct PostAeArgs {
    const float* ws; int nparts, PG; float* g_m; float* g_p; int n_red_x, n_red;
    const float* re; const float* im; const float* dmag; const float* dphs; const float* g_mag; float* dG; int F, KP, gx; float sat;
    int n_polar; const float* wg; int wg_nz; float* gSr; float* gSi; float* norm_s; int N; NyqJob nyq;
    unsigned short* dG16; int ht;
    unsigned polar_total, polar_magic;
    float* norm_e;
};
__global__ void __launch_bounds__(256)
post_ae_kernel(const PostAeArgs a)
{
    const int blk = blockIdx.x;
    if (blk < a.n_red) { const int ae = blk / a.n_red_x; ae_grad_reduce_block(a.ws, a.nparts, a.PG, a.g_m, a.g_p, blk - ae * a.n_red_x, ae, a.norm_e, blk); }
    else if (blk < a.n_red + a.n_polar && a.polar_total) polar_bwd_flat(a.re, a.im, a.dmag, a.dphs, a.g_mag, a.dG, a.F, a.KP, a.sat, (unsigned)(blk - a.n_red), a.polar_total, a.polar_magic, a.dG16, a.ht);
    else if (blk < a.n_red + a.n_polar) { const int q = blk - a.n_red, r = q / a.gx; polar_bwd_block(a.re, a.im, a.dmag, a.dphs, a.g_mag, a.dG, a.F, a.KP, a.sat, q - r * a.gx, r, a.dG16, a.ht); }
    else wgrad_reduce_block(a.wg, a.wg_nz, a.gSr, a.gSi, a.norm_s, a.N, a.F, a.KP, 1, blk - a.n_red - a.n_polar, nullptr, a.nyq);
}

struct FinArgs {
    const float* loss_partial; int n_loss; const float* reg_partial; int n_reg;
    const float* norm_a; int n_na; const float* norm_s; int n_ns;
    float inv_ycount, reg_scale, norm_scale;
    const float* norm_e; int n_ne;
};
__device__ __forceinline__ float finalize_block(const FinArgs& f, const bool want_loss, float* red, float& lc, float& rg, float& nrm)
{
    auto psum = [](const float* __restrict__ p, const int n) {
        float s0 = 0.f, s1 = 0.f, s2 = 0.f, s3 = 0.f;
        if ((reinterpret_cast<uintptr_t>(p) & 15) == 0) {
            const int n4 = n >> 2;
            const float4* p4 = reinterpret_cast<const float4*>(p);
            int i = threadIdx.x;
            for (; i + 768 < n4; i += 1024) {
                const float4 u0 = p4[i], u1 = p4[i + 256], u2 = p4[i + 512], u3 = p4[i + 768];
                s0 += (u0.x + u0.y) + (u0.z + u0.w); s1 += (u1.x + u1.y) + (u1.z + u1.w);
                s2 += (u2.x + u2.y) + (u2.z + u2.w); s3 += (u3.x + u3.y) + (u3.z + u3.w);
            }
            for (; i < n4; i += 256) { const float4 u = p4[i]; s0 += (u.x + u.y) + (u.z + u.w); }
            for (int j = 4 * n4 + threadIdx.x; j < n; j += 256) s1 += p[j];
        } else for (int j = threadIdx.x; j < n; j += 256) s0 += p[j];
        return (s0 + s1) + (s2 + s3);
    };
    float a = 0.f, b = 0.f, c = 0.f;
    if (want_loss && f.loss_partial) a = psum(f.loss_partial, f.n_loss);
    if (want_loss && f.reg_partial) b = psum(f.reg_partial, f.n_reg);
    if (f.norm_a) c += psum(f.norm_a, f.n_na);
    if (f.norm_s) c += psum(f.norm_s, f.n_ns);
    if (f.norm_e) c += psum(f.norm_e, f.n_ne);
    if (want_loss) { a = block_sum<4>(a, red); b = block_sum<4>(b, red); }
    c = block_sum<4>(c, red);
    __shared__ float bc;
    if (threadIdx.x == 0) bc = c;
    __syncthreads();
    lc = a * f.inv_ycount; rg = b * f.reg_scale; nrm = bc * f.norm_scale;
    const float coef = 1.0f / (nrm + 1e-6f);
    return coef < 1.0f ? coef : 1.0f;
}
__global__ void __launch_bounds__(256)
finalize_kernel(const FinArgs f, float* __restrict__ scalars)
{
    __shared__ float red[4];
    float lc, rg, nrm;
    const float coef = finalize_block(f, true, red, lc, rg, nrm);
    if (threadIdx.x == 0) {
        if (f.loss_partial) { scalars[1] = lc; scalars[2] = rg; scalars[0] = lc + rg; }
        if (f.norm_a || f.norm_s || f.norm_e) { scalars[3] = nrm; scalars[4] = coef; }
    }
}

__global__ void __launch_bounds__(256)
eval_finalize_kernel(const FinArgs f, const double beta, double* __restrict__ acc)
{
    __shared__ float red[4];
    float lc, rg, nrm, ma, t0, t1;
    finalize_block(f, true, red, lc, rg, nrm);
    FinArgs g = f; g.loss_partial = f.loss_partial + mae_partial_offset(f.n_loss); g.reg_partial = nullptr;
    finalize_block(g, true, red, ma, t0, t1);
    if (threadIdx.x == 0) {
#pragma clang fp contract(off)
        const double loss = (double)(lc + rg), mae = (double)ma;
        acc[0] = beta * acc[0] + (1.0 - beta) * loss;
        acc[1] = loss; acc[2] = (double)lc; acc[3] = (double)rg; acc[4] = mae;
// ... 395 lines not shown
```

Before: 11.21 million frames/s.

## Fuse analysis and synthesis weight-gradient GEMMs into one paired TN128 launch

Adds a paired TN128 kernel that computes the analysis and synthesis weight-gradient GEMMs in one launch. Each workgroup processes one tile from each problem, with column permutations chosen so a heavy K-range from one is paired with a light one from the other. The second job's prologue loads are issued before the first job's results are stored. A single fused reduce kernel then replaces the two separate reduce launches, removing launch overhead and tail imbalance between the two stages. The cost is more code complexity and a larger per-workgroup workload, which may reduce parallelism.

```diff
diff --git a/include/signaltrain_hip.h b/include/signaltrain_hip.h
--- a/include/signaltrain_hip.h
+++ b/include/signaltrain_hip.h
@@ -72,6 +72,8 @@
 int st_synthesis_frames(const st_dims* d, const float* AA, const float* Sfold, float* frs, void* stream);
 
 int st_nt128_worklist(const st_dims* d, int which, int ncus, unsigned* out, int cap, int* head6);
+
+int st_wgrad_pair_plan(const st_dims* d, int ncus, int* out, int cap);
 
 int st_fm_div_exact(int R, int B);
 
diff --git a/signaltrain_amd/_lib.py b/signaltrain_amd/_lib.py
--- a/signaltrain_amd/_lib.py
+++ b/signaltrain_amd/_lib.py
@@ -83,6 +83,7 @@
     "st_synth_slabs": (_i, [_D]),
     "st_synth_frame_slabs": (_i, [_D]),
     "st_nt128_worklist": (_i, [_D, _i, _i, C.POINTER(C.c_uint), _i, C.POINTER(C.c_int)]),
+    "st_wgrad_pair_plan": (_i, [_D, _i, C.POINTER(C.c_int), _i]),
     "st_fm_div_exact": (_i, [_i, _i]),
     "st_synth_fold": (_i, [_D, _p, _p, _p, _p]),
     "st_synthesis_frames": (_i, [_D, _p, _p, _p, _p]),
diff --git a/signaltrain_amd/csrc/st_api.hip b/signaltrain_amd/csrc/st_api.hip
--- a/signaltrain_amd/csrc/st_api.hip
+++ b/signaltrain_amd/csrc/st_api.hip
@@ -198,6 +198,7 @@
     {9300, 2, &g_wg_split, 0, nullptr},
     {9400, 2, &g_pl_bf16, 0, nullptr},
     {9500, 2, &g_tn128, 0, nullptr}, {9580, 1, &g_tn128, 2, nullptr}, {9581, 1, &g_tn128, 1, nullptr},
+    {9582, 1, &g_tn128, 3, nullptr},
     {9540, 4, &g_tn_fm, 0, nullptr},
     {9560, 16, &g_g16_crop, 0, nullptr},
     {9600, 2, &g_g16, 0, nullptr},
@@ -320,10 +321,10 @@
 extern "C" int st_ae_fwd_partials(const st_dims* d) { return check_dims(d) != ST_OK ? 0 : ae_fwd_partials(d); }
 extern "C" int st_ola_loss_partials(const st_dims* d) { return check_dims(d) != ST_OK ? 0 : ola_loss_partials(d); }
 extern "C" int st_norm_partials(const st_dims* d) { return check_dims(d) != ST_OK ? 0 : norm_partials(d); }
-static int tn_split(int R, int N)
+static int tn_split(int R, int N, int ncus = 0)
 {
     const int tiles = (N / 128) * (N / 128);
-    int s = num_cus() / (tiles > 0 ? tiles : 1); if (s > 16) s = 16;
+    int s = (ncus > 0 ? ncus : num_cus()) / (tiles > 0 ? tiles : 1); if (s > 16) s = 16;
     const int cap = R / 64; if (s > cap) s = cap;
     return s < 1 ? 1 : s;
 }
@@ -661,6 +662,28 @@
     return f;
 }
 #define ST_TN128(...) do { if (g_tn128 == 2) ST_TRY((stg::launch_tn128<32, false>(__VA_ARGS__))); else ST_TRY((stg::launch_tn128<32, true>(__VA_ARGS__))); } while (0)
+struct TNProblem { stg::TNOperand a, b; const float* zeros; stg::RowMap map; stg::FrameTrim trim; int R, ns; bool fits; };
+static TNProblem tn_problem(const st_dims* d, const stg::TNOperand& ta, const stg::TNOperand& tb, const stg::RowMap& live, size_t extentA, int Ls, int fm_bit, bool padded, int ncus)
+{
+    TNProblem p; p.zeros = tb.base; p.R = live.rows(d->B);
+    p.fits = use_tn128(d, padded) && stg::tn128_fits(ta, tb, tb.base, live, d->N, d->N, extentA, (size_t)d->B * (Ls + 2 * d->N));
+    p.ns = tn_split(p.R, d->N, ncus);
+    const TNFrameMajor fm = tn_frame_major(ta, tb, live, d->B, d->H, d->N, d->N, Ls, (g_tn_fm & fm_bit) != 0);
+    p.a = fm.a; p.b = fm.b; p.map = fm.map; p.trim = fm.trim;
+    return p;
+}
+static TNProblem synthesis_tn_problem(const st_dims* d, const float* AA, const float* dsyn, bool padded, int ncus = 0)
+{
+    const int KP = st_kp_of(d->F);
+    const stg::TNOperand ta{AA, (unsigned)(d->OT * KP), (unsigned)KP}, tb{dsyn, (unsigned)(d->y + 2 * d->N), (unsigned)d->H};
+    return tn_problem(d, ta, tb, synth_live(d), (size_t)d->B * d->OT * KP, d->y, 1, padded, ncus);
+}
+static TNProblem analysis_tn_problem(const st_dims* d, const float* dG, const float* sig, bool padded, int ncus = 0)
+{
+    const int KP = st_kp_of(d->F);
+    const stg::TNOperand ta{dG, (unsigned)(d->T * KP), (unsigned)KP}, tb{sig, (unsigned)(d->L + 2 * d->N), (unsigned)d->H};
+    return tn_problem(d, ta, tb, stg::live_frames(d->T, d->H, d->N, d->N, d->L), (size_t)d->B * d->T * KP, d->L, 2, padded, ncus);
+}
 static int wgrad_tn128(const st_dims* d, const stg::TNOperand& ta, const stg::TNOperand& tb, const float* zeros, const stg::RowMap& map, int R,
                        float* ws, int ns, stm::NyqJob* nyq, void* stream, const stg::FrameTrim* trim)
 {
@@ -681,11 +704,10 @@
     const int R = ms.rows(d->B);
     int ns = wgrad_split_tiles(R, KP, d->N);
     stm::NyqJob nyq{}; nyq.on = 0;
-    const stg::TNOperand ta{AA, (unsigned)(d->OT * KP), (unsigned)KP}, tb{dsyn, (unsigned)(d->y + 2 * d->N), (unsigned)d->H};
-    if (use_tn128(d, padded) && stg::tn128_fits(ta, tb, dsyn, ms, d->N, d->N, (size_t)d->B * d->OT * KP, (size_t)d->B * (d->y + 2 * d->N))) {
-        ns = tn_split(R, d->N);
-        const TNFrameMajor fm = tn_frame_major(ta, tb, ms, d->B, d->H, d->N, d->N, d->y, (g_tn_fm & 1) != 0);
-        ST_TRY(wgrad_tn128(d, fm.a, fm.b, dsyn, fm.map, R, ws, ns, &nyq, stream, &fm.trim));
+    const TNProblem tp = synthesis_tn_problem(d, AA, dsyn, padded);
+    if (tp.fits) {
+        ns = tp.ns;
+        ST_TRY(wgrad_tn128(d, tp.a, tp.b, tp.zeros, tp.map, R, ws, ns, &nyq, stream, &tp.trim));
     } else {
         stg::PlainTN al{AA, R, KP, KP, ms};
         stg::StoreC ep{ws, KP, d->N, d->N, (size_t)KP * d->N, stg::all_frames(1)};
@@ -987,11 +1009,10 @@
     }
     const int M = half < 0 ? KP : KP / 2, m0 = half > 0 ? KP / 2 : 0;
     stm::NyqJob nyq{}; nyq.on = 0;
-    const stg::TNOperand ta{dG, (unsigned)(d->T * KP), (unsigned)KP}, tb{sig, (unsigned)(d->L + 2 * d->N), (unsigned)d->H};
-    if (half < 0 && use_tn128(d, padded) && stg::tn128_fits(ta, tb, sig, ma, d->N, d->N, (size_t)d->B * d->T * KP, (size_t)d->B * (d->L + 2 * d->N))) {
-        ns = tn_split(R, d->N);
-        const TNFrameMajor fm = tn_frame_major(ta, tb, ma, d->B, d->H, d->N, d->N, d->L, (g_tn_fm & 2) != 0);
-        ST_TRY(wgrad_tn128(d, fm.a, fm.b, sig, fm.map, R, ws, ns, &nyq, stream, &fm.trim));
+    const TNProblem tp = analysis_tn_problem(d, dG, sig, padded);
+    if (half < 0 && tp.fits) {
+        ns = tp.ns;
+        ST_TRY(wgrad_tn128(d, tp.a, tp.b, tp.zeros, tp.map, R, ws, ns, &nyq, stream, &tp.trim));
     } else {
         stg::PlainTN al{dG + m0, R, KP, M, ma};
         stg::StoreC ep{ws + (size_t)m0 * d->N, M, d->N, d->N, (size_t)KP * d->N, stg::all_frames(1)};
@@ -1496,8 +1517,52 @@
     ST_LAUNCHED("analysis_wgrad_reduce");
     return ST_OK;
 }
+struct WgradPair { TNProblem pa, ps; stg::TNLaunch la, ls; stg::TNPair pair; bool on; };
+static void wgrad_pair_make(WgradPair& q, const st_dims* d, const WS& w, int ncus = 0)
+{
+    const int KP = st_kp_of(d->F), N = d->N, mh = (N / 2) / 128;
+    q.on = false;
+    if (g_tn128 != 1 || w.g16 || gemm_ht(d->prec) != 0 || ae_is_wide(d)) return;
+    q.pa = analysis_tn_problem(d, w.dG, w.xp, true, ncus); q.ps = synthesis_tn_problem(d, w.AA, w.dsyn, true, ncus);
+    if (!q.pa.fits || !q.ps.fits) return;
+    const unsigned c0 = (unsigned)(d->F - 1), c1 = (unsigned)(KP / 2 + d->F - 1);
+    const size_t slab = (size_t)KP * N;
+    q.la = stg::tn128_job(32, q.pa.a, q.pa.b, q.pa.zeros, q.pa.map, q.pa.R, N, mh, (unsigned)(KP / 2), N, w.wg, N, slab, q.pa.ns, w.wg + (size_t)q.pa.ns * slab, c0, c1, nullptr, &q.pa.trim);
+    q.ls = stg::tn128_job(32, q.ps.a, q.ps.b, q.ps.zeros, q.ps.map, q.ps.R, N, mh, (unsigned)(KP / 2), N, w.wg2, N, slab, q.ps.ns, w.wg2 + (size_t)q.ps.ns * slab, c0, c1, nullptr, &q.ps.trim);
+    q.on = stg::tn128_pair_make(q.pair, q.la, q.ls, 32);
+}
+static int wgrad_pair(Call& c, const WgradPair& q, float* grads)
+{
+    const st_dims* d = c.d; const Layout& L = c.L; void* stream = c.stream;
+    ST_TRY(stg::launch_tn128_pair<32>(q.pair, q.la, q.ls, st_stream(stream)));
+    ST_LAUNCHED("wgrad_pair");
+    stm::WgradPairArgs a;
+    const stg::TNLaunch* l[2] = {&q.la, &q.ls};
+    for (int i = 0; i < 2; ++i) {
+        a.ws[i] = l[i]->out; a.nz[i] = l[i]->j.nsplit; a.gRe[i] = grads + L.offs[2 * i]; a.gIm[i] = grads + L.offs[2 * i + 1]; a.norm[i] = i ? c.w.norm_s : c.w.norm_a;
+        a.nyq[i].part = l[i]->j.nyq_out; a.nyq[i].P = l[i]->j.nyq_P; a.nyq[i].on = 1;
+    }
+    a.N = d->N; a.F = d->F; a.KP = L.KP;
+    hipLaunchKernelGGL(stm::wgrad_pair_reduce_kernel, dim3(2 * norm_partials(d)), dim3(256), 0, st_stream(stream), a);
+    ST_LAUNCHED("wgrad_pair_reduce");
+    return ST_OK;
+}
+extern "C" int st_wgrad_pair_plan(const st_dims* d, int ncus, int* out, int cap)
+{
+    Layout L;
+    if (make_layout(d, &L) != ST_OK || cap < 0 || (cap > 0 && !out)) return -1;
+    WS w; carve(d, L, reinterpret_cast<void*>(sizeof(float)), &w);
+    WgradPair q; wgrad_pair_make(q, d, w, ncus);
+    if (!q.on) return 0;
+    return stg::tn128_pair_describe(q.pair, d->N / 128, d->N / 128, 32, out, cap);
+}
 static int backward_impl(Call& c, const float* params, float* grads, const float* g_mag_hat, const float* g_mag, float reg_coef, float* kg = nullptr)
 {
+    WgradPair q; wgrad_pair_make(q, c.d, c.w);
+    if (q.on) {
+        ST_TRY(backward_p1(c, params, grads, g_mag_hat, g_mag, reg_coef, kg, ST_STAGE_EVERY & ~ST_STAGE_SYN_WGRAD));
+        return wgrad_pair(c, q, grads);
+    }
     ST_TRY(backward_p1(c, params, grads, g_mag_hat, g_mag, reg_coef, kg));
     return backward_p2(c, grads);
 }
diff --git a/signaltrain_amd/csrc/st_gemm_tn.h b/signaltrain_amd/csrc/st_gemm_tn.h
--- a/signaltrain_amd/csrc/st_gemm_tn.h
+++ b/signaltrain_amd/csrc/st_gemm_tn.h
@@ -35,6 +35,18 @@
     return f;
 }
 
+__host__ __device__ static inline void tn128_krange(const TNJob& j, const int tx, const int z, const int ksplit, const int bkt, int& k_begin, int& k_end)
+{
+    k_begin = z * ksplit;
+    k_end = (k_begin + ksplit < j.K) ? k_begin + ksplit : j.K;
+    if (j.trim) {
+        const int lo = (int)j.fa[tx] * j.fB, hi = (int)j.fb[tx] * j.fB;
+        const int per = ((hi - lo + j.nsplit - 1) / j.nsplit + bkt - 1) / bkt * bkt;
+        k_begin = lo + z * per;
+        k_end = (k_begin + per < hi) ? k_begin + per : hi;
+    }
+}
+
 __device__ __forceinline__ void nyq_partial(const TNJob& j, const int p)
 {
     if (p >= j.nyq_P) return;
@@ -63,62 +75,161 @@
     }
 }
 
+template <int BKT, bool UNI> struct TNTile {
+    static constexpr int TS = BKT * 128;
+    static constexpr int NP = BKT / 8;
+    static constexpr int KS = BKT / 2;
+    static constexpr int PAIRS = KS / 2;
+    static_assert(PAIRS % 2 == 0 && NP + 1 <= PAIRS - 1, "fragment buffers alternate by pair; stores and loads sit before the barrier");
+    float* As; float* Bs;
+    int c4, kr, a_off, b_off;
+    const char* base; unsigned la, lb, lz, sa1, sa2, sb1, sb2, magic; int Tv, t_lo, K;
+    unsigned ua[UNI ? NP : 1], ub[UNI ? NP : 1];
+    int k_begin, ntiles, k_last;
+    float4 ra[NP], rb[NP];
+    float2 fa[2][2], fb[2][2];
+
+    __device__ __forceinline__ void init(float* lds)
+    {
+        const int tid = threadIdx.x, lane = tid & 63, wave = tid >> 6, wm = wave >> 1, wn = wave & 1, h = lane >> 5, l31 = lane & 31;
+        As = lds; Bs = lds + 2 * TS;
+        c4 = tid & 31; kr = tid >> 5;
+        a_off = h * 128 + wm * 64 + 2 * l31;
+        b_off = h * 128 + wn * 64 + 2 * l31;
+    }
+    __device__ __forceinline__ void job(const TNJob& j, const unsigned rowA, const unsigned colB)
+    {
+        base = reinterpret_cast<const char*>(j.base);
+        la = 4u * (j.a0 + rowA + 4u * (unsigned)c4); lb = 4u * (j.b0 + colB + 4u * (unsigned)c4); lz = 4u * (j.zero + 4u * (unsigned)c4);
+        sa1 = 4u * j.SA1; sa2 = 4u * j.SA2; sb1 = 4u * j.SB1; sb2 = 4u * j.SB2;
+        magic = j.magic; Tv = j.Tv; t_lo = j.t_lo; K = j.K;
+        if constexpr (UNI) {
+#pragma unroll
+            for (int p = 0; p < NP; ++p) { ua[p] = la + (unsigned)(kr + 8 * p) * sa2; ub[p] = lb + (unsigned)(kr + 8 * p) * sb2; }
+        }
+    }
+    __device__ __forceinline__ float4 ld(const unsigned byte_off) const { return *reinterpret_cast<const float4*>(base + byte_off); }
+    __device__ __forceinline__ void gl(const int kt, const int p)
+    {
+        if constexpr (UNI) {
+            const unsigned b = __umulhi((unsigned)kt, magic), t0 = (unsigned)t_lo + (unsigned)kt - b * (unsigned)Tv;
+            ra[p] = ld(b * sa1 + t0 * sa2 + ua[p]);
+            rb[p] = ld(b * sb1 + t0 * sb2 + ub[p]);
+        } else {
+            const int k = kt + kr + 8 * p;
+            const unsigned kc = (unsigned)(k < K ? k : K - 1);
+            const unsigned b = __umulhi(kc, magic);
+            const unsigned t = (unsigned)t_lo + kc - __umul24(b, (unsigned)Tv);
+            const unsigned oa = __umul24(b, sa1) + __umul24(t, sa2) + la;
+            const unsigned ob = __umul24(b, sb1) + __umul24(t, sb2) + lb;
+            const unsigned live = (unsigned)((k - K) >> 31);
+            ra[p] = ld((oa & live) | (lz & ~live));
+            rb[p] = ld(ob);
+        }
+    }
+    __device__ __forceinline__ void gload(const int kt)
+    {
+#pragma unroll
+        for (int p = 0; p < NP; ++p) gl(kt, p);
+    }
+    __device__ __forceinline__ void lstore_pass(const int buf, const int p)
+    {
+        float* as = As + buf * TS + kr * 128 + 4 * c4;
+        float* bs = Bs + buf * TS + kr * 128 + 4 * c4;
+        *reinterpret_cast<float4*>(as + p * 8 * 128) = ra[p];
+        *reinterpret_cast<float4*>(bs + p * 8 * 128) = rb[p];
+    }
+    __device__ __forceinline__ void lstore(const int buf)
+    {
+#pragma unroll
+        for (int p = 0; p < NP; ++p) lstore_pass(buf, p);
+    }
+    __device__ __forceinline__ void frag(const int stage, const int pr, const int buf)
+    {
+        const float* as = As + stage * TS + a_off;
+        const float* bs = Bs + stage * TS + b_off;
+#pragma unroll
+        for (int u = 0; u < 2; ++u) {
+            fa[buf][u] = *reinterpret_cast<const float2*>(as + (2 * pr + u) * 256);
+            fb[buf][u] = *reinterpret_cast<const float2*>(bs + (2 * pr + u) * 256);
+        }
+    }
+    __device__ __forceinline__ void mfma8(f32x16 (&acc)[2][2], const int buf) const
+    {
+#pragma unroll
+        for (int u = 0; u < 2; ++u) {
+            const float2 a = fa[buf][u], b = fb[buf][u];
+            acc[0][0] = __builtin_amdgcn_mfma_f32_32x32x2f32(a.x, b.x, acc[0][0], 0, 0, 0);
+            acc[0][1] = __builtin_amdgcn_mfma_f32_32x32x2f32(a.x, b.y, acc[0][1], 0, 0, 0);
+            acc[1][0] = __builtin_amdgcn_mfma_f32_32x32x2f32(a.y, b.x, acc[1][0], 0, 0, 0);
+            acc[1][1] = __builtin_amdgcn_mfma_f32_32x32x2f32(a.y, b.y, acc[1][1], 0, 0, 0);
+        }
+    }
+    __device__ __forceinline__ void prologue(const int kb, const int ke)
+    {
+        k_begin = kb; ntiles = (ke - kb + BKT - 1) / BKT;
+        if (ntiles > 0) {
+            k_last = k_begin + (ntiles - 1) * BKT;
+            gload(k_begin);
+            lstore(0);
+            gload(ntiles > 1 ? k_begin + BKT : k_begin);
+        }
+    }
+    __device__ __forceinline__ void tile(f32x16 (&acc)[2][2], const int i, int& cur)
+    {
+        const int k2 = k_begin + (i + 2) * BKT, kn = k2 < k_last ? k2 : k_last;
+        __builtin_amdgcn_sched_barrier(0);
+#pragma unroll
+        for (int pr = 0; pr < PAIRS - 1; ++pr) {
+            frag(cur, pr + 1, (pr + 1) & 1);
+            if (pr < NP) lstore_pass(cur ^ 1, pr);
+            if (pr >= 1 && pr <= NP) gl(kn, pr - 1);
+            mfma8(acc, pr & 1);
+            __builtin_amdgcn_sched_barrier(0);
+        }
+        __syncthreads();
+        frag(cur ^ 1, 0, 0);
+        mfma8(acc, 1);
+        __builtin_amdgcn_sched_barrier(0);
+        cur ^= 1;
+    }
+    template <bool PEEL> __device__ __forceinline__ void loop(f32x16 (&acc)[2][2])
+    {
+        if (ntiles > 0) {
+            __syncthreads();
+            frag(0, 0, 0);
+            int cur = 0, i = 0;
+            if constexpr (PEEL) { tile(acc, 0, cur); i = 1; }
+            for (; i < ntiles; ++i) tile(acc, i, cur);
+        }
+    }
+};
+__device__ __forceinline__ void tn128_store(const f32x16 (&acc)[2][2], float* __restrict__ o, const int ldo, const int lane)
+{
+#pragma unroll
+    for (int i = 0; i < 16; ++i) {
+        const int r = 2 * d_row(i, lane);
+#pragma unroll
+        for (int mi = 0; mi < 2; ++mi)
+            *reinterpret_cast<float2*>(o + (size_t)(r + mi) * ldo) = make_float2(acc[mi][0][i], acc[mi][1][i]);
+    }
+}
+
 template <int BKT, bool PIPE = false, bool UNI = false>
 __global__ void __launch_bounds__(256) __attribute__((amdgpu_waves_per_eu(1, 2)))
 gemm_tn128_kernel(const TNJob j, float* __restrict__ out, const int ldo, const size_t slab, const int ksplit)
 {
-    constexpr int TS = BKT * 128;
-    constexpr int NP = BKT / 8;
-    constexpr int KS = BKT / 2;
+    constexpr int TS = BKT * 128, NP = BKT / 8, KS = BKT / 2;
     extern __shared__ __attribute__((aligned(16))) float tn_lds[];
-    float* const As = tn_lds;
-    float* const Bs = tn_lds + 2 * TS;
 
     const int tid = threadIdx.x, lane = tid & 63, wave = tid >> 6, wm = wave >> 1, wn = wave & 1;
     if ((int)blockIdx.z >= j.nsplit) { nyq_partial(j, (int)(blockIdx.y * gridDim.x + blockIdx.x)); return; }
     int tbx, tby, tbz; xcd_tile(tbx, tby, tbz, j.nsplit);
     const unsigned rowA = (unsigned)(tby % j.mh) * 128u + (unsigned)(tby / j.mh) * j.mstride;
     const unsigned colB = (unsigned)tbx * 128u;
-    int k_begin = tbz * ksplit;
-    int k_end = (k_begin + ksplit < j.K) ? k_begin + ksplit : j.K;
-    if (j.trim) {
-        const int lo = (int)j.fa[tbx] * j.fB, hi = (int)j.fb[tbx] * j.fB;
-        const int per = ((hi - lo + j.nsplit - 1) / j.nsplit + BKT - 1) / BKT * BKT;
-        k_begin = lo + tbz * per;
-        k_end = (k_begin + per < hi) ? k_begin + per : hi;
-    }
-
-    const int c4 = tid & 31, kr = tid >> 5;
-    const unsigned la = 4u * (j.a0 + rowA + 4u * (unsigned)c4), lb = 4u * (j.b0 + colB + 4u * (unsigned)c4), lz = 4u * (j.zero + 4u * (unsigned)c4);
-    const unsigned sa1 = 4u * j.SA1, sa2 = 4u * j.SA2, sb1 = 4u * j.SB1, sb2 = 4u * j.SB2;
-    float4 ra[NP], rb[NP];
-    auto ld = [&](const unsigned byte_off) { return *reinterpret_cast<const float4*>(reinterpret_cast<const char*>(j.base) + byte_off); };
-    auto gload_pass = [&](const int kt, const int p) {
-        const int k = kt + kr + 8 * p;
-        const unsigned kc = (unsigned)(k < j.K ? k : j.K - 1);
-        const unsigned b = __umulhi(kc, j.magic);
-        const unsigned t = (unsigned)j.t_lo + kc - __umul24(b, (unsigned)j.Tv);
-        const unsigned oa = __umul24(b, sa1) + __umul24(t, sa2) + la;
-        const unsigned ob = __umul24(b, sb1) + __umul24(t, sb2) + lb;
-        const unsigned live = (unsigned)((k - j.K) >> 31);
-        ra[p] = ld((oa & live) | (lz & ~live));
-        rb[p] = ld(ob);
-    };
-    auto gload = [&](const int kt) {
-#pragma unroll
-        for (int p = 0; p < NP; ++p) gload_pass(kt, p);
-    };
-    auto lstore_pass = [&](const int buf, const int p) {
-        float* as = As + buf * TS + kr * 128 + 4 * c4;
-        float* bs = Bs + buf * TS + kr * 128 + 4 * c4;
-        *reinterpret_cast<float4*>(as + p * 8 * 128) = ra[p];
-        *reinterpret_cast<float4*>(bs + p * 8 * 128) = rb[p];
-    };
-    auto lstore = [&](const int buf) {
-#pragma unroll
-        for (int p = 0; p < NP; ++p) lstore_pass(buf, p);
-    };
-
+    int k_begin, k_end; tn128_krange(j, tbx, tbz, ksplit, BKT, k_begin, k_end);
+
+    TNTile<BKT, UNI> t; t.init(tn_lds); t.job(j, rowA, colB);
     f32x16 acc[2][2];
 #pragma unroll
     for (int mi = 0; mi < 2; ++mi)
@@ -127,86 +238,23 @@
 #pragma unroll
             for (int i = 0; i < 16; ++i) acc[mi][nj][i] = 0.f;
 
-    const int h = lane >> 5, l31 = lane & 31;
+    const int l31 = lane & 31;
     if constexpr (PIPE) {
-        constexpr int PAIRS = KS / 2;
-        static_assert(PAIRS % 2 == 0 && NP + 1 <= PAIRS - 1, "fragment buffers alternate by pair; stores and loads sit before the barrier");
-        const int ntiles = (k_end - k_begin + BKT - 1) / BKT;
-        if (ntiles > 0) {
-            const int k_last = k_begin + (ntiles - 1) * BKT;
-            unsigned ua[UNI ? NP : 1], ub[UNI ? NP : 1];
-            if constexpr (UNI) {
-#pragma unroll
-                for (int p = 0; p < NP; ++p) { ua[p] = la + (unsigned)(kr + 8 * p) * sa2; ub[p] = lb + (unsigned)(kr + 8 * p) * sb2; }
-            }
-            auto gl = [&](const int kt, const int p) {
-                if constexpr (UNI) {
-                    const unsigned b = __umulhi((unsigned)kt, j.magic), t0 = (unsigned)j.t_lo + (unsigned)kt - b * (unsigned)j.Tv;
-                    ra[p] = ld(b * sa1 + t0 * sa2 + ua[p]);
-                    rb[p] = ld(b * sb1 + t0 * sb2 + ub[p]);
-                } else gload_pass(kt, p);
-            };
-            const int a_off = h * 128 + wm * 64 + 2 * l31;
-            const int b_off = h * 128 + wn * 64 + 2 * l31;
-            float2 fa[2][2], fb[2][2];
-            auto frag = [&](const int stage, const int pr, const int buf) {
-                const float* as = As + stage * TS + a_off;
-                const float* bs = Bs + stage * TS + b_off;
-#pragma unroll
-                for (int u = 0; u < 2; ++u) {
-                    fa[buf][u] = *reinterpret_cast<const float2*>(as + (2 * pr + u) * 256);
-                    fb[buf][u] = *reinterpret_cast<const float2*>(bs + (2 * pr + u) * 256);
-                }
-            };
-            auto mfma8 = [&](const int buf) {
-#pragma unroll
-                for (int u = 0; u < 2; ++u) {
-                    const float2 a = fa[buf][u], b = fb[buf][u];
-                    acc[0][0] = __builtin_amdgcn_mfma_f32_32x32x2f32(a.x, b.x, acc[0][0], 0, 0, 0);
-                    acc[0][1] = __builtin_amdgcn_mfma_f32_32x32x2f32(a.x, b.y, acc[0][1], 0, 0, 0);
-                    acc[1][0] = __builtin_amdgcn_mfma_f32_32x32x2f32(a.y, b.x, acc[1][0], 0, 0, 0);
-                    acc[1][1] = __builtin_amdgcn_mfma_f32_32x32x2f32(a.y, b.y, acc[1][1], 0, 0, 0);
-                }
-            };
-#pragma unroll
-            for (int p = 0; p < NP; ++p) gl(k_begin, p);
-            lstore(0);
-#pragma unroll
-            for (int p = 0; p < NP; ++p) gl(ntiles > 1 ? k_begin + BKT : k_begin, p);
-            __syncthreads();
-            frag(0, 0, 0);
-            int cur = 0;
-            for (int i = 0; i < ntiles; ++i) {
-                const int k2 = k_begin + (i + 2) * BKT, kn = k2 < k_last ? k2 : k_last;
-                __builtin_amdgcn_sched_barrier(0);
-#pragma unroll
-                for (int pr = 0; pr < PAIRS - 1; ++pr) {
-                    frag(cur, pr + 1, (pr + 1) & 1);
-                    if (pr < NP) lstore_pass(cur ^ 1, pr);
-                    if (pr >= 1 && pr <= NP) gl(kn, pr - 1);
-                    mfma8(pr & 1);
-                    __builtin_amdgcn_sched_barrier(0);
-                }
-                __syncthreads();
-                frag(cur ^ 1, 0, 0);
-                mfma8(1);
-                __builtin_amdgcn_sched_barrier(0);
-                cur ^= 1;
-            }
-        }
+        t.prologue(k_begin, k_end);
+        t.template loop<false>(acc);
     } else if (k_begin < k_end) {
-        gload(k_begin);
-        lstore(0);
+        float* const As = t.As; float* const Bs = t.Bs;
+        t.gload(k_begin);
+        t.lstore(0);
         __syncthreads();
         int cur = 0;
-        const int a_off = h * 128 + wm * 64 + 2 * l31;
-        const int b_off = h * 128 + wn * 64 + 2 * l31;
+        const int a_off = t.a_off, b_off = t.b_off;
         float2 abl_f[4];
 #pragma unroll
         for (int u = 0; u < 4; ++u) abl_f[u] = (ST_G128_ABLATE & 2) ? *reinterpret_cast<const float2*>(As + a_off + u * 256) : make_float2(0.f, 0.f);
         for (int kt = k_begin; kt < k_end; kt += BKT) {
             const bool more = kt + BKT < k_end;
-            if (!(ST_G128_ABLATE & 8)) gload(more ? kt + BKT : kt);
+            if (!(ST_G128_ABLATE & 8)) t.gload(more ? kt + BKT : kt);
             __builtin_amdgcn_sched_barrier(0);
             const float* as = As + cur * TS + a_off;
             const float* bs = Bs + cur * TS + b_off;
@@ -239,22 +287,79 @@
                 __builtin_amdgcn_sched_group_barrier(0x008, 8, 0);
             }
             __builtin_amdgcn_sched_barrier(0);
-            if (!(ST_G128_ABLATE & 4)) lstore(cur ^ 1);
+            if (!(ST_G128_ABLATE & 4)) t.lstore(cur ^ 1);
             else {
 #pragma unroll
-                for (int p = 0; p < NP; ++p) { asm volatile("" :: "v"(ra[p].x), "v"(ra[p].y), "v"(ra[p].z), "v"(ra[p].w)); asm volatile("" :: "v"(rb[p].x), "v"(rb[p].y), "v"(rb[p].z), "v"(rb[p].w)); }
+                for (int p = 0; p < NP; ++p) { asm volatile("" :: "v"(t.ra[p].x), "v"(t.ra[p].y), "v"(t.ra[p].z), "v"(t.ra[p].w)); asm volatile("" :: "v"(t.rb[p].x), "v"(t.rb[p].y), "v"(t.rb[p].z), "v"(t.rb[p].w)); }
             }
             if (!(ST_G128_ABLATE & 1)) __syncthreads();
             cur ^= 1;
         }
     }
-    float* o = out + (size_t)tbz * slab + (size_t)(rowA + wm * 64) * ldo + colB + wn * 64 + 2 * l31;
-#pragma unroll
-    for (int i = 0; i < 16; ++i) {
-        const int r = 2 * d_row(i, lane);
+    tn128_store(acc, out + (size_t)tbz * slab + (size_t)(rowA + wm * 64) * ldo + colB + wn * 64 + 2 * l31, ldo, lane);
+}
+
+struct TNPair {
+    TNJob j[2]; float* out[2]; int ldo[2]; size_t slab[2]; int ksplit[2];
+    int nz;
+    unsigned char perm[64];
+};
+__host__ __device__ static inline bool tn128_pair_entry(const TNPair& p, const int job, const int sx, const int sz, const int bkt, int& tx, int& k_begin, int& k_end)
+{
+    if (sz >= p.j[job].nsplit) return false;
+    tx = job ? (int)p.perm[sx] : sx;
+    tn128_krange(p.j[job], tx, sz, p.ksplit[job], bkt, k_begin, k_end);
+    return true;
+}
+template <int BKT, bool UNI>
+__global__ void __launch_bounds__(256) __attribute__((amdgpu_waves_per_eu(1, 2)))
+gemm_tn128_pair_kernel(const TNPair p)
+{
+    extern __shared__ __attribute__((aligned(16))) float tn_pair_lds[];
+    const int tid = threadIdx.x, lane = tid & 63, wave = tid >> 6, wm = wave >> 1, wn = wave & 1, l31 = lane & 31;
+    if ((int)blockIdx.z >= p.nz) {
+        const int part = (int)(blockIdx.y * gridDim.x + blockIdx.x);
+        if ((int)blockIdx.z == p.nz) nyq_partial(p.j[0], part); else nyq_partial(p.j[1], part);
+        return;
+    }
+    int sx, sy, sz; xcd_tile(sx, sy, sz, p.nz);
+    int tx0 = 0, tx1 = 0, kb0 = 0, ke0 = 0, kb1 = 0, ke1 = 0;
+    const bool on0 = tn128_pair_entry(p, 0, sx, sz, BKT, tx0, kb0, ke0), on1 = tn128_pair_entry(p, 1, sx, sz, BKT, tx1, kb1, ke1);
+
+    TNTile<BKT, UNI> t; t.init(tn_pair_lds);
+    f32x16 acc[2][2];
+    auto clear = [&]() {
 #pragma unroll
         for (int mi = 0; mi < 2; ++mi)
-            *reinterpret_cast<float2*>(o + (size_t)(r + mi) * ldo) = make_float2(acc[mi][0][i], acc[mi][1][i]);
+#pragma unroll
+            for (int nj = 0; nj < 2; ++nj)
+#pragma unroll
+                for (int i = 0; i < 16; ++i) acc[mi][nj][i] = 0.f;
+    };
+    auto row_of = [&](const TNJob& j) { return (unsigned)(sy % j.mh) * 128u + (unsigned)(sy / j.mh) * j.mstride; };
+    auto tile_out = [&](const int job, const unsigned rowA, const unsigned colB) {
+        return p.out[job] + (size_t)sz * p.slab[job] + (size_t)(rowA + wm * 64) * p.ldo[job] + colB + wn * 64 + 2 * l31;
+    };
+    clear();
+    if (on0) {
+        t.job(p.j[0], row_of(p.j[0]), (unsigned)tx0 * 128u);
+        t.prologue(kb0, ke0);
+        t.template loop<false>(acc);
+    }
+    if (on1) {
+        t.job(p.j[1], row_of(p.j[1]), (unsigned)tx1 * 128u);
+        t.prologue(kb1, ke1);
+    }
+    if (on0) {
+        tn128_store(acc, tile_out(0, row_of(p.j[0]), (unsigned)tx0 * 128u), p.ldo[0], lane);
+        clear();
+        if (on1) {
+            t.template loop<true>(acc);
+            tn128_store(acc, tile_out(1, row_of(p.j[1]), (unsigned)tx1 * 128u), p.ldo[1], lane);
+        }
+    } else if (on1) {
+        t.template loop<false>(acc);
+        tn128_store(acc, tile_out(1, row_of(p.j[1]), (unsigned)tx1 * 128u), p.ldo[1], lane);
     }
 }
 
@@ -273,30 +378,88 @@
     if (map.Tv % bkt || K % bkt) return false;
     return !(trim && trim->on) || trim->B % bkt == 0;
 }
-template <int BKT, bool PIPE = false>
-static inline int launch_tn128(const TNOperand& A, const TNOperand& B, const float* zeros, const RowMap& map, int K,
-                               int M, int mh, unsigned mstride, int Nc, float* out, int ldo, size_t slab, int nsplit, hipStream_t s,
-                               float* nyq_out = nullptr, unsigned nyq_c0 = 0, unsigned nyq_c1 = 0, int* nyq_P = nullptr, const FrameTrim* trim = nullptr)
+struct TNLaunch { TNJob j; float* out; int ldo; size_t slab; int ksplit, M, Nc; bool nyq, uniform; };
+static inline TNLaunch tn128_job(const int BKT, const TNOperand& A, const TNOperand& B, const float* zeros, const RowMap& map, int K,
+                                 int M, int mh, unsigned mstride, int Nc, float* out, int ldo, size_t slab, int nsplit,
+                                 float* nyq_out = nullptr, unsigned nyq_c0 = 0, unsigned nyq_c1 = 0, int* nyq_P = nullptr, const FrameTrim* trim = nullptr)
 {
     const float* lo = A.base < B.base ? A.base : B.base; if (zeros < lo) lo = zeros;
-    TNJob j;
+    TNLaunch l; TNJob& j = l.j;
     j.base = lo; j.a0 = (unsigned)(A.base - lo); j.b0 = (unsigned)(B.base - lo); j.zero = (unsigned)(zeros - lo);
     j.SA1 = A.S1; j.SA2 = A.S2; j.SB1 = B.S1; j.SB2 = B.S2;
     j.magic = map.magic; j.Tv = map.Tv; j.t_lo = map.t_lo; j.K = K; j.mh = mh; j.mstride = mstride;
     j.trim = (trim && trim->on) ? 1 : 0; j.fB = trim ? trim->B : 0;
     for (int i = 0; i < 64; ++i) { j.fa[i] = trim ? trim->fa[i] : 0; j.fb[i] = trim ? trim->fb[i] : 0; }
-    int ksplit = K;
-    if (nsplit > 1) ksplit = st_round_up((K + nsplit - 1) / nsplit, BKT);
-    constexpr size_t lds = (size_t)4 * BKT * 128 * sizeof(float);
-    static_assert(lds <= 65536, "the Nyquist side workgroups share a CU with a GEMM workgroup: 2 x 64 KB of the 160");
+    l.ksplit = K;
+    if (nsplit > 1) l.ksplit = st_round_up((K + nsplit - 1) / nsplit, BKT);
     const int nz = nsplit > 1 ? nsplit : 1, tiles = (Nc / 128) * (M / 128);
     j.nsplit = nz; j.Nc = Nc; j.nyq_out = nyq_out; j.nyq_c0 = nyq_c0; j.nyq_c1 = nyq_c1;
     j.nyq_P = tiles < 64 ? tiles : 64; { const int W = K / 8 > 0 ? K / 8 : 1; if (j.nyq_P > W) j.nyq_P = W; }
     if (nyq_P) *nyq_P = j.nyq_P;
-    const dim3 grid(Nc / 128, M / 128, nz + (nyq_out ? 1 : 0));
+    l.out = out; l.ldo = ldo; l.slab = slab; l.M = M; l.Nc = Nc; l.nyq = nyq_out != nullptr; l.uniform = tn128_uniform(map, K, BKT, trim);
+    return l;
+}
+template <int BKT, bool PIPE = false>
+static inline int launch_tn128(const TNOperand& A, const TNOperand& B, const float* zeros, const RowMap& map, int K,
+                               int M, int mh, unsigned mstride, int Nc, float* out, int ldo, size_t slab, int nsplit, hipStream_t s,
+                               float* nyq_out = nullptr, unsigned nyq_c0 = 0, unsigned nyq_c1 = 0, int* nyq_P = nullptr, const FrameTrim* trim = nullptr)
+{
+    const TNLaunch l = tn128_job(BKT, A, B, zeros, map, K, M, mh, mstride, Nc, out, ldo, slab, nsplit, nyq_out, nyq_c0, nyq_c1, nyq_P, trim);
+    const TNJob& j = l.j; const int ksplit = l.ksplit;
+    constexpr size_t lds = (size_t)4 * BKT * 128 * sizeof(float);
+    static_assert(lds <= 65536, "the Nyquist side workgroups share a CU with a GEMM workgroup: 2 x 64 KB of the 160");
+    const dim3 grid(Nc / 128, M / 128, j.nsplit + (nyq_out ? 1 : 0));
     if (!PIPE) hipLaunchKernelGGL((gemm_tn128_kernel<BKT>), grid, dim3(256), lds, s, j, out, ldo, slab, ksplit);
-    else if (tn128_uniform(map, K, BKT, trim)) hipLaunchKernelGGL((gemm_tn128_kernel<BKT, PIPE, PIPE>), grid, dim3(256), lds, s, j, out, ldo, slab, ksplit);
+    else if (l.uniform) hipLaunchKernelGGL((gemm_tn128_kernel<BKT, PIPE, PIPE>), grid, dim3(256), lds, s, j, out, ldo, slab, ksplit);
     else hipLaunchKernelGGL((gemm_tn128_kernel<BKT, PIPE, false>), grid, dim3(256), lds, s, j, out, ldo, slab, ksplit);
+    return 0;
+}
+
+static inline int tn128_col_tiles(const TNLaunch& l, int tx, int bkt)
+{
+    int k0, k1; tn128_krange(l.j, tx, 0, l.ksplit, bkt, k0, k1);
+    return k1 > k0 ? (k1 - k0 + bkt - 1) / bkt : 0;
+}
+static inline bool tn128_pair_make(TNPair& p, const TNLaunch& a, const TNLaunch& b, int bkt)
+{
+    if (a.M != b.M || a.Nc != b.Nc || a.Nc / 128 > 64 || !a.nyq || !b.nyq) return false;
+    const TNLaunch* l[2] = {&a, &b};
+    for (int q = 0; q < 2; ++q) { p.j[q] = l[q]->j; p.out[q] = l[q]->out; p.ldo[q] = l[q]->ldo; p.slab[q] = l[q]->slab; p.ksplit[q] = l[q]->ksplit; }
+    p.nz = a.j.nsplit > b.j.nsplit ? a.j.nsplit : b.j.nsplit;
+    const int nx = a.Nc / 128;
+    int ia[64], ib[64];
+    for (int c = 0; c < nx; ++c) {
+        const int ta = tn128_col_tiles(a, c, bkt), tb = tn128_col_tiles(b, c, bkt);
+        int i = c; while (i > 0 && tn128_col_tiles(a, ia[i - 1], bkt) < ta) { ia[i] = ia[i - 1]; --i; } ia[i] = c;
+        i = c; while (i > 0 && tn128_col_tiles(b, ib[i - 1], bkt) > tb) { ib[i] = ib[i - 1]; --i; } ib[i] = c;
+    }
+    for (int c = 0; c < 64; ++c) p.perm[c] = (unsigned char)c;
+    for (int i = 0; i < nx; ++i) p.perm[ia[i]] = (unsigned char)ib[i];
+    return true;
+}
+static inline int tn128_pair_describe(const TNPair& p, int ny, int nx, int bkt, int* out, int cap)
+{
+    int n = 0;
+    for (int sz = 0; sz < p.nz; ++sz)
+        for (int sy = 0; sy < ny; ++sy)
+            for (int sx = 0; sx < nx; ++sx, ++n) {
+                if (!out || n >= cap) continue;
+                for (int q = 0; q < 2; ++q) {
+                    int tx, k0, k1, *o = out + (size_t)n * 10 + 5 * q;
+                    if (tn128_pair_entry(p, q, sx, sz, bkt, tx, k0, k1)) { o[0] = sy; o[1] = tx; o[2] = sz; o[3] = k0; o[4] = k1; }
+                    else for (int i = 0; i < 5; ++i) o[i] = -1;
+                }
+            }
+    return n;
+}
+template <int BKT>
+static inline int launch_tn128_pair(const TNPair& p, const TNLaunch& a, const TNLaunch& b, hipStream_t s)
+{
+    constexpr size_t lds = (size_t)4 * BKT * 128 * sizeof(float);
+    static_assert(lds <= 65536, "the Nyquist side workgroups share a CU with a GEMM workgroup: 2 x 64 KB of the 160");
+    const dim3 grid(a.Nc / 128, a.M / 128, p.nz + 2);
+    if (a.uniform && b.uniform) hipLaunchKernelGGL((gemm_tn128_pair_kernel<BKT, true>), grid, dim3(256), lds, s, p);
+    else hipLaunchKernelGGL((gemm_tn128_pair_kernel<BKT, false>), grid, dim3(256), lds, s, p);
     return 0;
 }
 
diff --git a/signaltrain_amd/csrc/st_misc.h b/signaltrain_amd/csrc/st_misc.h
--- a/signaltrain_amd/csrc/st_misc.h
+++ b/signaltrain_amd/csrc/st_misc.h
@@ -513,6 +513,14 @@
 {
     const int row = (int)blockIdx.x < nrows ? (int)blockIdx.x + row0 : 2 * F + extra0 + ((int)blockIdx.x - nrows);
     wgrad_reduce_block(ws, nz, gRe, gIm, norm_partial, N, F, KP, mode, row, stage, nyq, stage_bf16);
+}
+struct WgradPairArgs { const float* ws[2]; int nz[2]; float* gRe[2]; float* gIm[2]; float* norm[2]; NyqJob nyq[2]; int N, F, KP; };
+__global__ void __launch_bounds__(256)
+wgrad_pair_reduce_kernel(const WgradPairArgs a)
+{
+    const int n = norm_partial_count(a.F, a.N);
+    if ((int)blockIdx.x < n) wgrad_reduce_block(a.ws[0], a.nz[0], a.gRe[0], a.gIm[0], a.norm[0], a.N, a.F, a.KP, 0, (int)blockIdx.x, nullptr, a.nyq[0]);
+    else wgrad_reduce_block(a.ws[1], a.nz[1], a.gRe[1], a.gIm[1], a.norm[1], a.N, a.F, a.KP, 1, (int)blockIdx.x - n, nullptr, a.nyq[1]);
 }
 
 __global__ void __launch_bounds__(256)
```

New measurement: 11.35 million frames/s (median of 6 runs). 1.3% higher.
